# NilanEkanayake/TiTok-Video

Measured on AMD Instinct MI355X. Metric: video clips/sec encode+decode (whole node), higher is better.
Workload: dtype bf16

## Files before the change

include/titok_hip.h:

```cpp
#ifndef TITOK_HIP_H
#define TITOK_HIP_H

#include <stdint.h>

#ifdef __cplusplus
extern "C" {
#endif

#define TTV_OK 0
#define TTV_ERR_INVALID 1
#define TTV_ERR_LAUNCH 2
#define TTV_ERR_UNSUPPORTED 3

#define TTV_BF16 0
#define TTV_F32 1

#define TTV_ENCODER 0
#define TTV_DECODER 1

#define TTV_MAX_FSQ 8
#define TTV_MAX_TOKEN 64
#define TTV_MAX_CLIPS_PER_LAUNCH 64

const char* ttv_error_string(void);
int ttv_version(void);

typedef struct ttv_fsq_params {
  int32_t n;
  int32_t levels[TTV_MAX_FSQ];
  int32_t basis[TTV_MAX_FSQ];
  float half_l[TTV_MAX_FSQ];
  float offset[TTV_MAX_FSQ];
  float shift[TTV_MAX_FSQ];
  float half_width[TTV_MAX_FSQ];
} ttv_fsq_params;

int ttv_fsq_forward(const ttv_fsq_params* p, const void* z, int z_dtype, int rows, void* codes, int codes_dtype,
                    int32_t* indices, float* bounded, void* stream);
int ttv_fsq_indices_to_codes(const ttv_fsq_params* p, const int32_t* indices, int rows, void* codes, int codes_dtype,
                             void* stream);

int ttv_vq_codebook_norms(const void* codebook, int dtype, int ld, int N, int C, float* cnorm, void* stream);
int64_t ttv_vq_workspace_bytes(int rows);
int ttv_vq_l2_argmin(const void* z, int dtype, int ldz, const void* codebook, int ldc, const float* cnorm, int rows, int N, int C,
                     int32_t* indices, float* best_dist, void* workspace, int64_t workspace_bytes, void* stream);
int ttv_vq_lookup(const void* codebook, int dtype, int ldc, const int32_t* indices, int rows, int C, void* codes, int ldo, void* stream);
int ttv_vq_lookup_backward(const void* dcodes, int dtype, int ld, const int32_t* indices, int rows, int C, float* dcodebook, int ldc, void* stream);

int64_t ttv_vq_train_workspace_bytes(int rows, int N);
int ttv_vq_commit_forward(const void* z, int dtype, int ldz, const void* codebook, int ldc, const int32_t* indices, int rows, int N, int C,
                          float* loss, void* workspace, int64_t workspace_bytes, void* stream);
int ttv_vq_commit_backward(const void* grad, int ldg, const void* z, int ldz, const void* e, int lde, int dtype, int rows, int C, double scale,
                           void* dz, int ldd, void* stream);
int ttv_vq_ema_stats(const void* z, int dtype, int ldz, const int32_t* indices, int rows, int N, int C, const float* cluster_size,
                     float dead_threshold, uint64_t seed, const int64_t* ema_step, int rank, int world_size, float* stats, void* workspace,
                     int64_t workspace_bytes, void* stream);
int ttv_vq_ema_update(const float* stats, float* cluster_size, float* embed_avg, float* codebook, void* codebook_copy, int copy_dtype,
                      float* cnorm, int64_t* ema_step, int N, int C, float decay, float one_minus_decay, float eps, float dead_threshold,
                      void* workspace, int64_t workspace_bytes, void* stream);

int ttv_quant_rows_fp8(const void* in, int dtype, int ld_in, const float* gain, float eps, void* out, int ld_out, float* scales, int rows,
                       int width, void* stream);
int ttv_linear_fp8(const void* xq, int ldx, const float* x_scale, const void* wq, int ldw, const float* w_scale, void* y, int ldy, int M, int N,
                   int K, int epilogue, const float* rope_cs, int d_model, int gqa_dim, void* stream);

int ttv_split3_pack(const float* w, int ldw, void* out, int ldo, int rows, int K, void* stream);
int ttv_linear_split3(const float* x, int ldx, const void* w_image, int ldw, const float* bias, float* y, int ldy, int M, int N, int K, void* stream);

int64_t ttv_mx_scale_bytes_per_row(int width);
int ttv_quant_mx_fp8(const void* in, int dtype, int ld_in, void* out, int ld_out, void* mx, float* row_scales, int rows, int width, void* stream);
int ttv_linear_fp8_mx(const void* xq, int ldx, const void* x_mx, const float* x_row_scale, const void* wq, int ldw, const void* w_mx,
                      const float* w_row_scale, void* y, int ldy, int M, int N, int K, int epilogue, const float* rope_cs, int d_model,
                      int gqa_dim, const void* resid, int ldr, float alpha, void* stream);


int ttv_rmsnorm(const void* in, int in_dtype, int ld_in, const int32_t* src_rows, void* out, int out_dtype, int ld_out,
                const int32_t* dst_rows, const float* gain, int rows, int width, float eps, void* stream);

int ttv_rope_apply(void* x, int dtype, int ld, int rows, int heads, const float* rope_cs, void* stream);

int ttv_linear(const void* x, int ldx, const void* w, int ldw, const void* bias, const float* add_scalar, void* y, int ldy,
               int M, int N, int K, int dtype, void* stream);

int ttv_linear_qkv_rope(const void* x, int ldx, const void* w, int ldw, void* y, int ldy, int M, int d_model, int gqa_dim,
                        const float* rope_cs, int dtype, void* stream);
int ttv_linear_geglu(const void* x, int ldx, const void* w, int ldw, void* y, int ldy, int M, int I, int K, int dtype,
                     void* stream);
int ttv_linear_residual(const void* x, int ldx, const void* w, int ldw, const void* resid, int ldr, float alpha, void* y,
                        int ldy, int y_f32, int M, int N, int K, int dtype, void* stream);

int ttv_linear_residual_norm(const void* x, int ldx, const void* w, int ldw, const void* resid, int ldr, float alpha,
                             const float* gain, float eps, void* y, int ldy, int M, int N, int K, int dtype, void* stream);

int64_t ttv_mlp_pack_bytes(int inner, int next_qkv_rows);
int ttv_mlp_pack(const void* w12_folded, const void* w3, const void* out_proj, const void* next_qkv_folded, int next_qkv_rows, int inner,
                 int width, int dtype, void* mlp_packed, void* stream);
int ttv_mlp_fused(const void* x, int ldx, const void* mlp_packed, int inner, void* y, int ldy, const float* post_gain, float alpha,
                  float eps, int M, int width, int dtype, void* stream);
typedef struct ttv_next_qkv {
  void* qkv; int32_t ld;
  const float* rope_cs;
  int32_t rows;
  int32_t rope_q_end, rope_k_begin, rope_k_end;
} ttv_next_qkv;
int ttv_layer_tail_fused(const void* ao, int ldao, const float* attn_post_gain, float attn_alpha, const void* x, int ldx,
                         const void* mlp_packed, int inner, void* y, int ldy, const float* ffd_post_gain, float ffd_alpha, float eps,
                         int M, int width, int dtype, const ttv_next_qkv* next, void* stream);

int ttv_fill_const_rows(void* x, int dtype, int ld, const int32_t* rows_map, int rows, int width, const float* mask_token,
                        const float* gain, float eps, void* stream);
int ttv_decoder_embed(const void* codes, int token_size, const void* w, const void* bias, const float* mask_token, const float* gain,
                      void* x, int dtype, int ld, const int32_t* rows_map, int rows, int width, float eps, void* stream);

#define TTV_ATTN_GATE 1
#define TTV_ATTN_PAIRED 2
#define TTV_ATTN_QSCALED 4
#define TTV_ATTN_ALLFULL 8
#define TTV_ATTN_PIPE 16
#define TTV_ATTN_SPLIT3 32
#define TTV_ATTN_SPLIT_OUT 64
#define TTV_ATTN_SPLIT_IN 128
int ttv_attention(const void* qkvg, int ld, void* out, int ldo, const int32_t* cu_seqlens, const int32_t* qblocks,
                  int n_qblocks, int q_heads, int kv_heads, int head_dim, int flags, int dtype, void* stream);
int ttv_attention64(const void* qkvg, int ld, void* out, int ldo, const int32_t* cu_seqlens, const int32_t* items, int n_items,
                    int q_heads, int kv_heads, int head_dim, int flags, int dtype, void* stream);

int ttv_rmsnorm_mx(const void* in, int in_dtype, int ld_in, void* out, int out_dtype, int ld_out, const float* gain, int rows, int width,
                   float eps, float* next_rstd, void* mx_q, void* mx_s, void* stream);
int ttv_attention_mxout(const void* qkvg, int ld, void* out_q, void* out_mx, int ld_mx, const int32_t* cu_seqlens, const int32_t* qblocks,
                        int n_qblocks, int q_heads, int kv_heads, void* stream);
int ttv_linear_fp8_mx_geglu_q(const void* xq, int ldx, const void* x_mx, const float* x_row_scale, const void* wq, int ldw, const void* w_mx,
                              const float* w_row_scale, void* hq, void* hq_mx, int M, int N, int K, void* stream);

int ttv_row_rstd(const void* x, int dtype, int ldx, float* rstd, int rows, int width, float eps, void* stream);
int ttv_linear_rowscale(const void* x, int ldx, const void* w, int ldw, const float* row_scale, int epilogue, const float* rope_cs, int d_model,
                        int gqa_dim, void* y, int ldy, int M, int N, int K, int dtype, void* stream);

int ttv_patch_gather(const void* const* clips, const int32_t* clip_desc, int clip0, int n_clips, int patch_t, int patch_h,
                     int patch_w, int channels, void* patches, int ld, int dtype, int max_patches_per_clip, void* stream);
int ttv_patch_embed_norm(const void* const* clips, const int32_t* clip_desc, const int32_t* patch_rows, const int32_t* row_seq, int n_clips,
                         int patch_t, int patch_h, int patch_w, int channels, const void* w, int ldw, const void* bias,
                         const float* mask_token, const float* gain, float eps, void* x, int ldx, int rows, int width, int dtype,
                         void* stream);
int ttv_patch_scatter(const void* patches, int ld, const int32_t* clip_desc, int clip0, int n_clips, int patch_t, int patch_h,
                      int patch_w, int channels, void* const* clips, int dtype, int max_patches_per_clip, void* stream);

typedef struct ttv_tower_dims {
  int32_t kind;
  int32_t dtype;
  int32_t width;
  int32_t layers;
  int32_t q_heads, kv_heads, head_dim;
  int32_t inner;
  int32_t patch_t, patch_h, patch_w;
  int32_t pix_channels;
  int32_t token_size;
  float eps;
  float alpha;
} ttv_tower_dims;

typedef struct ttv_layer_weights {
  const float* pre_ln;
  const void* to_qkv;
  const void* out_proj;
  const float* ffd_norm;
  const void* w12;
  const void* w3;
  const float* attn_post_ln;
  const float* ffd_post_ln;
  const void* to_qkv_pn;
  const void* w12_pn;
  const void* mlp_pack;
  int32_t mlp_pack_qkv_rows;
  int32_t qkv_q_prescaled;
  const void* to_qkv_qs;
  const void* to_qkv_f8; const float* to_qkv_f8_scale;
  const void* w12_f8; const float* w12_f8_scale;
  const void* to_qkv_mx; const void* w12_mx;
  const void* out_proj_f8; const float* out_proj_f8_scale; const void* out_proj_mx;
  const void* w3_f8; const float* w3_f8_scale; const void* w3_mx;
} ttv_layer_weights;

typedef struct ttv_tower_weights {
  const void* proj_in_w;
  const void* proj_in_b;
  const float* mask_token;
  const float* ln_pre_t;
  const float* ln_pre_p;
  const float* ln_post;
  const void* proj_out_w;
  const void* proj_out_b;
  const ttv_layer_weights* layers;
  const void* proj_out_pn;
  int32_t f32_split3;
} ttv_tower_weights;

typedef struct ttv_batch {
  int32_t n_clips;
  int32_t total_rows;
  int32_t sum_tokens;
  int32_t sum_patches;
  int32_t max_patches_per_clip;
  int32_t n_qblocks;
  const int32_t* cu_seqlens;
  const int32_t* latent_rows;
  const int32_t* patch_rows;
  const int32_t* clip_desc;
  const int32_t* qblocks;
  const float* rope_cs;
  const int32_t* blocks64;
  const int32_t* row_seq;
  int32_t n_blocks64;
  int32_t qblocks_paired;
  int32_t qblocks_all_full;
  const int32_t* items64;
  int32_t n_items64;
  const int32_t* rope_ids;
  const float* rope_base;
  const int32_t* qblocks_latent;
  int32_t n_qblocks_latent;
  const int32_t* qblocks_patch;
  int32_t n_qblocks_patch;
  int32_t tokens_per_clip;
} ttv_batch;

int ttv_rope_table_build(const float* base_cos, const float* base_sin, int n_ids, int n_freqs, const int32_t* clip_desc,
                         const int32_t* cu_seqlens, const int32_t* row_seq, float* rope_cs, int total_rows, void* stream);

typedef struct ttv_plan_sizes {
  int32_t n_clips, total_rows, sum_tokens, sum_patches, max_patches_per_clip, max_seqlen, n_rope_ids, n_blocks64;
  int64_t host_words;
  int64_t off_cu_seqlens, off_clip_desc, off_blocks64;
  int64_t dev_words;
  int64_t off_latent_rows, off_patch_rows, off_row_seq, off_rope_ids;
} ttv_plan_sizes;

int ttv_plan_rows_sizes(const int32_t* pixel_dims, const int32_t* token_counts, int n_clips, const int32_t* patch, ttv_plan_sizes* sizes);
int ttv_plan_rows_fill(const int32_t* pixel_dims, const int32_t* token_counts, int n_clips, const int32_t* patch, int bwd_xcd,
                       int32_t* host_segment, int64_t host_words);

int ttv_plan_rows_build(const ttv_plan_sizes* sizes, const int32_t* host_segment, int32_t* dev_segment, const float* base_cos,
                        const float* base_sin, int n_freqs, float* rope_cs, const float* rope_base, ttv_batch* batch, void* stream);

typedef struct ttv_plan_attn {
  int32_t n_qblocks, qblocks_all_full, n_qblocks_latent, n_qblocks_patch, n_qblocks_l0;
  int32_t tokens_per_clip;
  int64_t words;
  int64_t off_qblocks, off_qblocks_latent, off_qblocks_patch, off_qblocks_l0;
} ttv_plan_attn;

int ttv_plan_attn_sizes(const int32_t* cu_seqlens, const int32_t* token_counts, int n_clips, int q_heads, int kv_heads, int split,
                        int tail_div, ttv_plan_attn* sizes);
int ttv_plan_attn_fill(const int32_t* cu_seqlens, const int32_t* token_counts, int n_clips, int q_heads, int kv_heads, int split,
                       int tail_div, int32_t* host_tables, int64_t host_words);
int ttv_plan_attn_set(const ttv_plan_attn* sizes, const int32_t* host_tables, int32_t* dev_tables, ttv_batch* batch, void* stream);

int ttv_rope_base_table(int head_dim, int nd, int n_ids, double theta, float* base_cos, float* base_sin);

int64_t ttv_tower_workspace_bytes(const ttv_tower_dims* dims, const ttv_batch* batch);

// ... 123 lines not shown
int ttv_l1_loss(void* const* recon, void* const* target, void* const* grad, const int32_t* sizes, int n_clips, int dtype, float* loss,
                void* stream);

int ttv_clip_from_u8(const void* frames_thwc, int T, int H, int W, void* clip_cthw, int dtype, void* stream);

int ttv_clip_resample_u8(void* const* frames_thwc, void* const* clips_cthw, const int32_t* geom, int n_clips, int dtype, void* stream);

int ttv_recon_panels_u8(void* const* target, void* const* recon, const int32_t* dims, int n_clips, int dtype, void* const* panels,
                        void* stream);

int ttv_sq_err_accumulate(void* const* recon, void* const* target, const int32_t* sizes, int n_clips, int dtype, int clamp, double* acc,
                          void* stream);

int64_t ttv_ssim_workspace_bytes(const int32_t* dims, int n_clips);
int ttv_ssim_accumulate(void* const* recon, void* const* target, const int32_t* dims, int n_clips, int dtype, int clamp, double* acc,
                        void* workspace, int64_t workspace_bytes, void* stream);

typedef struct {
  const void* w[13];
  const void* wd[13];
  const float* b[13];
  const float* lin[5];
} ttv_lpips_weights;

int64_t ttv_lpips_tape_bytes(int n, int H, int W, int dtype);
int64_t ttv_lpips_workspace_bytes(int n, int H, int W, int dtype);

int ttv_lpips_forward(const ttv_lpips_weights* w, const void* recon, const void* target, int n, int H, int W, int dtype, float* lpips,
                      float* gram, void* tape, void* workspace, int64_t workspace_bytes, void* stream);

int ttv_lpips_backward(const ttv_lpips_weights* w, const void* tape, int n, int H, int W, int dtype, const float* glpips,
                       const float* ggram, void* drecon, void* workspace, int64_t workspace_bytes, void* stream);

int64_t ttv_lpips_eval_workspace_bytes(int frames, int H, int W, int dtype);
int ttv_lpips_eval_accumulate(const ttv_lpips_weights* w, void* const* recon_clips, void* const* target_clips, const int32_t* frames,
                              int n_clips, int H, int W, int dtype, int clamp_recon, float* per_frame, double* acc, void* workspace,
                              int64_t workspace_bytes, void* stream);

int ttv_lpips_crops_forward(void* const* recon_clips, void* const* target_clips, const int32_t* clip_dims, int n_clips, const int32_t* crops,
                            int n_crops, int size, void* recon_crops, void* target_crops, int dtype, void* stream);
int ttv_lpips_crops_backward(void* const* recon_clips, void* const* grad_clips, const int32_t* clip_dims, int n_clips, const int32_t* crops,
                             int n_crops, int size, const void* g, int dtype, void* stream);

int ttv_gp_noise_add(const void* table, int n_clips, const int32_t* chunks, int n_chunks, int generate, uint64_t seed, uint64_t draw,
                     float gp_noise, int dtype, void* stream);

#define TTV_DISC_HEAD_GENERATOR 0
#define TTV_DISC_HEAD_DISCRIMINATOR 1
int ttv_disc_head(const void* per_token_a, const void* per_token_b, int mode, int groups, int n_clips, int tokens_per_clip, int dtype,
                  float gp_scale, float centering_weight, float* terms, float* grad, void* stream);

int64_t ttv_lpips_conv_workspace_bytes(int N, int H, int W, int Cin, int Cout, int dtype);
int ttv_lpips_conv3x3(const void* x, int N, int H, int W, int Cin, int Cout, const void* w, const float* bias, int mode, const void* h,
                      void* y, int dtype, void* workspace, int64_t workspace_bytes, void* stream);
int ttv_lpips_maxpool(const void* x, int N, int H, int W, int C, void* y, int dtype, void* stream);
int ttv_lpips_maxpool_backward(const void* dy, const float* add, const void* h, int N, int H, int W, int C, void* dx, int dtype,
                               void* stream);

#define TTV_I3D_CONVS 58
#define TTV_I3D_FEATURES 400
typedef struct {
  const float* w[TTV_I3D_CONVS];
  const float* scale[TTV_I3D_CONVS];
  const float* shift[TTV_I3D_CONVS];
} ttv_i3d_weights;

int64_t ttv_i3d_workspace_bytes(int n);

int ttv_fvd_preprocess(void* const* clips, const int32_t* dims, int n_clips, int dtype, int clamp, float* out, void* stream);

int ttv_i3d_features(const ttv_i3d_weights* w, const float* x, int n, float* feats, void* workspace, int64_t workspace_bytes,
                     void* stream);

int ttv_i3d_conv3d(const float* x, int N, int T, int H, int W, int Cin, int k, int stride, const float* w, const float* scale,
                   const float* shift, int Cout, int relu, float* y, int ldc, int c_off, void* stream);
int ttv_i3d_maxpool3d(const float* x, int N, int T, int H, int W, int C, int kt, int kh, int kw, int st, int sh, int sw, float* y,
                      void* stream);

#define TTV_VJEPA_WIDTH 1024
#define TTV_VJEPA_TOKENS 1568
#define TTV_VJEPA_PATCH_K 1536
typedef struct ttv_vjepa_layer {
  const float* norm1_w; const float* norm1_b;
  const void* qkv_w; const void* qkv_b;
  const void* proj_w; const void* proj_b;
  const float* norm2_w; const float* norm2_b;
  const void* fc1_w; const void* fc1_b;
  const void* fc2_w; const void* fc2_b;
} ttv_vjepa_layer;
typedef struct ttv_vjepa_weights {
  int32_t width, heads, depth;
  const void* patch_w; const void* patch_b; const float* pos_embed;
  const ttv_vjepa_layer* layers;
  const float* norm_w; const float* norm_b;
  const float* query_tokens; const void* pool_q;
  const float* pool_norm1_w; const float* pool_norm1_b;
  const void* pool_kv_w; const void* pool_kv_b;
  const void* pool_proj_w; const void* pool_proj_b;
  const float* pool_norm2_w; const float* pool_norm2_b;
  const void* pool_fc1_w; const void* pool_fc1_b;
  const void* pool_fc2_w; const void* pool_fc2_b;
} ttv_vjepa_weights;

int ttv_jedi_preprocess(void* const* clips, const int32_t* dims, int n_clips, int dtype, void* out, void* stream);
int64_t ttv_vjepa_workspace_bytes(int n);
int ttv_vjepa_features(const ttv_vjepa_weights* w, const void* x, int n, float* feats, int finetuned, void* workspace,
                       int64_t workspace_bytes, void* stream);

#define TTV_VJEPA_EPI_STORE 0
#define TTV_VJEPA_EPI_GELU 1
#define TTV_VJEPA_EPI_RESID 2
int ttv_vjepa_layernorm(const float* x, int ldx, int rows, int width, const float* w1, const float* b1, float eps1, const float* w2,
                        const float* b2, float eps2, float* y32, int ld32, void* y16, int ld16, void* stream);
int ttv_vjepa_linear(const void* x, int ldx, const void* w, int ldw, const void* bias, int M, int N, int K, int epilogue,
                     const float* resid, int ldr, int resid_rows, void* y, int ldy, void* stream);
int ttv_vjepa_pool_attention(const void* q, const void* kv, int n, int rows, void* out, void* stream);

#define TTV_KC_ATTENTION 1
#define TTV_KC_GEMM_QKV 2
#define TTV_KC_GEMM_GEGLU 3
#define TTV_KC_GEMM_RESID 4
#define TTV_KC_GEMM_STORE 5
#define TTV_KC_RMSNORM 6
#define TTV_KC_PATCH 7
#define TTV_KC_ROWS 8
int ttv_prof_begin(int kernel_class, int max_records);
enum {
  TTV_DBG_NO_STORES = 1,
  TTV_DBG_K256_NO_PANEL_DMA = 2,
  TTV_DBG_MLP_NO_WEIGHT_DMA = 2,
  TTV_DBG_K256_NO_TILE_RELOAD = 4,
  TTV_DBG_MLP_NO_GEGLU = 4,
  TTV_DBG_K256_NO_EPILOGUE_MATH = 8,
  TTV_DBG_MLP_TILES8 = 8,
  TTV_DBG_MLP_NO_P2 = 16,
  TTV_DBG_MLP_PAIRS_ONLY = 32,
  TTV_DBG_MLP_TILES4 = 64,
  TTV_DBG_GEMM_TILE160 = 128,
  TTV_DBG_GEMM_TILE128 = 256,
  TTV_DBG_GEMM_T256 = 512,
  TTV_DBG_MLP_TILES9 = 512,
  TTV_DBG_GEMM_NO_T256 = 1024,
  TTV_DBG_MX_UNFUSED_QUANT = 2048,
  TTV_DBG_SPLIT3_NO_IMAGES = 4096,
  TTV_DBG_SPLIT3_NO_DMA = 8192,
  TTV_DBG_K256_GENERAL = 16384,
  TTV_DBG_QKV256_OFF = 32768,
  TTV_DBG_QKV256_WS = 131072,
  TTV_DBG_ENC_ALL_ROWS = 524288,
  TTV_DBG_ATTN_NO_SWP = 1048576,
  TTV_DBG_DEC_ALL_BLOCKS = 2097152,
  TTV_DBG_DEC_L0_NO_CONST = 4194304,
  TTV_DBG_ENC_LAST_QKV_ALL = 8388608,
  TTV_DBG_PATCH_EMBED_UNFUSED = 16777216
};
int ttv_debug_set(int flags);
int ttv_debug_stamps(void* device_buffer);
int ttv_prof_end(double* total_ms, int* count);

#ifdef __cplusplus
}
#endif
#endif
```

titok_video_amd/_lib.py:

```python
from __future__ import annotations

import ctypes as C
import os
import threading

import torch

from . import switches

TTV_BF16, TTV_F32 = 0, 1
TTV_ENCODER, TTV_DECODER = 0, 1
TTV_MAX_FSQ = 8
TTV_MAX_TOKEN = 64
TTV_MAX_CLIPS_PER_LAUNCH = 64
TTV_DISC_HEAD_GENERATOR, TTV_DISC_HEAD_DISCRIMINATOR = 0, 1
TTV_TAPE_STORED, TTV_TAPE_RECOMPUTE = 0, 1

DBG_NO_STORES = 1
DBG_K256_NO_PANEL_DMA = 2
DBG_MLP_NO_WEIGHT_DMA = 2
DBG_K256_NO_TILE_RELOAD = 4
DBG_MLP_NO_GEGLU = 4
DBG_K256_NO_EPILOGUE_MATH = 8
DBG_MLP_TILES8 = 8
DBG_MLP_NO_P2 = 16
DBG_MLP_PAIRS_ONLY = 32
DBG_MLP_TILES4 = 64
DBG_GEMM_TILE160 = 128
DBG_GEMM_TILE128 = 256
DBG_GEMM_T256 = 512
DBG_MLP_TILES9 = 512
DBG_GEMM_NO_T256 = 1024
DBG_MX_UNFUSED_QUANT = 2048
DBG_SPLIT3_NO_IMAGES = 4096
DBG_SPLIT3_NO_DMA = 8192
DBG_K256_GENERAL = 16384
DBG_QKV256_OFF = 32768
DBG_QKV256_WS = 131072
DBG_ENC_ALL_ROWS = 524288
DBG_ATTN_NO_SWP = 1048576
DBG_DEC_ALL_BLOCKS = 2097152
DBG_DEC_L0_NO_CONST = 4194304
DBG_ENC_LAST_QKV_ALL = 8388608
DBG_PATCH_EMBED_UNFUSED = 16777216

_HERE = os.path.dirname(os.path.abspath(__file__))
LIB_PATH = switches.text("TTV_LIB_PATH") or os.path.join(_HERE, "libtitok_hip.so")

i32, i64, f32, vp = C.c_int32, C.c_int64, C.c_float, C.c_void_p


class FsqParams(C.Structure):
    _fields_ = [("n", i32), ("levels", i32 * TTV_MAX_FSQ), ("basis", i32 * TTV_MAX_FSQ),
                ("half_l", f32 * TTV_MAX_FSQ), ("offset", f32 * TTV_MAX_FSQ), ("shift", f32 * TTV_MAX_FSQ),
                ("half_width", f32 * TTV_MAX_FSQ)]


class TowerDims(C.Structure):
    _fields_ = [("kind", i32), ("dtype", i32), ("width", i32), ("layers", i32), ("q_heads", i32), ("kv_heads", i32),
                ("head_dim", i32), ("inner", i32), ("patch_t", i32), ("patch_h", i32), ("patch_w", i32),
                ("pix_channels", i32), ("token_size", i32), ("eps", f32), ("alpha", f32)]


class NextQkv(C.Structure):
    _fields_ = [("qkv", vp), ("ld", i32), ("rope_cs", vp), ("rows", i32), ("rope_q_end", i32), ("rope_k_begin", i32), ("rope_k_end", i32)]


class LayerWeights(C.Structure):
    _fields_ = [("pre_ln", vp), ("to_qkv", vp), ("out_proj", vp), ("ffd_norm", vp), ("w12", vp), ("w3", vp),
                ("attn_post_ln", vp), ("ffd_post_ln", vp), ("to_qkv_pn", vp), ("w12_pn", vp), ("mlp_pack", vp), ("mlp_pack_qkv_rows", i32), ("qkv_q_prescaled", i32),
                ("to_qkv_qs", vp), ("to_qkv_f8", vp), ("to_qkv_f8_scale", vp), ("w12_f8", vp), ("w12_f8_scale", vp),
                ("to_qkv_mx", vp), ("w12_mx", vp), ("out_proj_f8", vp), ("out_proj_f8_scale", vp), ("out_proj_mx", vp),
                ("w3_f8", vp), ("w3_f8_scale", vp), ("w3_mx", vp)]


class TowerWeights(C.Structure):
    _fields_ = [("proj_in_w", vp), ("proj_in_b", vp), ("mask_token", vp), ("ln_pre_t", vp), ("ln_pre_p", vp),
                ("ln_post", vp), ("proj_out_w", vp), ("proj_out_b", vp), ("layers", C.POINTER(LayerWeights)), ("proj_out_pn", vp),
                ("f32_split3", i32)]


class Batch(C.Structure):
    _fields_ = [("n_clips", i32), ("total_rows", i32), ("sum_tokens", i32), ("sum_patches", i32),
                ("max_patches_per_clip", i32), ("n_qblocks", i32), ("cu_seqlens", vp), ("latent_rows", vp),
                ("patch_rows", vp), ("clip_desc", vp), ("qblocks", vp), ("rope_cs", vp), ("blocks64", vp), ("row_seq", vp),
                ("n_blocks64", i32), ("qblocks_paired", i32), ("qblocks_all_full", i32), ("items64", vp), ("n_items64", i32),
                ("rope_ids", vp), ("rope_base", vp), ("qblocks_latent", vp), ("n_qblocks_latent", i32), ("qblocks_patch", vp),
                ("n_qblocks_patch", i32), ("tokens_per_clip", i32)]


class PlanSizes(C.Structure):
    _fields_ = [("n_clips", i32), ("total_rows", i32), ("sum_tokens", i32), ("sum_patches", i32), ("max_patches_per_clip", i32),
                ("max_seqlen", i32), ("n_rope_ids", i32), ("n_blocks64", i32), ("host_words", i64), ("off_cu_seqlens", i64),
                ("off_clip_desc", i64), ("off_blocks64", i64), ("dev_words", i64), ("off_latent_rows", i64), ("off_patch_rows", i64),
                ("off_row_seq", i64), ("off_rope_ids", i64)]


class PlanAttn(C.Structure):
    _fields_ = [("n_qblocks", i32), ("qblocks_all_full", i32), ("n_qblocks_latent", i32), ("n_qblocks_patch", i32), ("n_qblocks_l0", i32),
                ("tokens_per_clip", i32), ("words", i64), ("off_qblocks", i64), ("off_qblocks_latent", i64), ("off_qblocks_patch", i64),
                ("off_qblocks_l0", i64)]


class DecL0Const(C.Structure):
    _fields_ = [("rows", vp), ("latent_rows", i32), ("patch_rows", i32), ("state", vp), ("qblocks", vp), ("n_qblocks", i32)]


class LayerWeightsT(C.Structure):
    _fields_ = [("to_qkv_t", vp), ("out_proj_t", vp), ("w12_t", vp), ("w3_t", vp)]


class TowerWeightsT(C.Structure):
    _fields_ = [("proj_in_t", vp), ("proj_out_t", vp), ("layers", C.POINTER(LayerWeightsT))]


class LayerGrads(C.Structure):
    _fields_ = [("pre_ln", vp), ("to_qkv", vp), ("out_proj", vp), ("ffd_norm", vp), ("w12", vp), ("w3", vp),
                ("attn_post_ln", vp), ("ffd_post_ln", vp)]


class TowerGrads(C.Structure):
    _fields_ = [("proj_in_w", vp), ("proj_in_b", vp), ("mask_token", vp), ("ln_pre_t", vp), ("ln_pre_p", vp), ("ln_post", vp),
                ("proj_out_w", vp), ("proj_out_b", vp), ("layers", C.POINTER(LayerGrads)), ("layer_done_events", C.POINTER(vp))]


TTV_OPT_SCHEDULE_NONE, TTV_OPT_SCHEDULE_COSINE = 0, 1
TTV_OPT_SKIP_NONFINITE = 1


class OptState(C.Structure):
    _fields_ = [("updates", i64), ("skipped", i64), ("schedule_index", i64), ("skip_now", i32), ("lr", f32), ("bc1", f32),
                ("bc2_sqrt", f32), ("clip_coef", f32), ("norm", f32)]


class OptSchedule(C.Structure):
    _fields_ = [("kind", i32), ("reserved", i32), ("warmup_steps", i64), ("training_steps", i64), ("base_lr", C.c_double),
                ("end_lr", C.c_double), ("num_cycles", C.c_double), ("initial_lr", C.c_double), ("first", i64), ("stride", i64)]


class LpipsWeights(C.Structure):
    _fields_ = [("w", vp * 13), ("wd", vp * 13), ("b", vp * 13), ("lin", vp * 5)]


TTV_I3D_CONVS = 58
TTV_I3D_FEATURES = 400


class I3dWeights(C.Structure):
    _fields_ = [("w", vp * TTV_I3D_CONVS), ("scale", vp * TTV_I3D_CONVS), ("shift", vp * TTV_I3D_CONVS)]


TTV_VJEPA_WIDTH = 1024
TTV_VJEPA_TOKENS = 1568
TTV_VJEPA_PATCH_K = 1536
TTV_VJEPA_EPI_STORE, TTV_VJEPA_EPI_GELU, TTV_VJEPA_EPI_RESID = 0, 1, 2


class VjepaLayer(C.Structure):
    _fields_ = [("norm1_w", vp), ("norm1_b", vp), ("qkv_w", vp), ("qkv_b", vp), ("proj_w", vp), ("proj_b", vp), ("norm2_w", vp),
                ("norm2_b", vp), ("fc1_w", vp), ("fc1_b", vp), ("fc2_w", vp), ("fc2_b", vp)]


class VjepaWeights(C.Structure):
    _fields_ = [("width", i32), ("heads", i32), ("depth", i32), ("patch_w", vp), ("patch_b", vp), ("pos_embed", vp),
                ("layers", C.POINTER(VjepaLayer)), ("norm_w", vp), ("norm_b", vp), ("query_tokens", vp), ("pool_q", vp),
                ("pool_norm1_w", vp), ("pool_norm1_b", vp), ("pool_kv_w", vp), ("pool_kv_b", vp), ("pool_proj_w", vp),
                ("pool_proj_b", vp), ("pool_norm2_w", vp), ("pool_norm2_b", vp), ("pool_fc1_w", vp), ("pool_fc1_b", vp),
                ("pool_fc2_w", vp), ("pool_fc2_b", vp)]


_lib = None
_lock = threading.Lock()

SYMBOLS = {
    "ttv_error_string": (C.c_char_p, []),
    "ttv_version": (C.c_int, []),
    "ttv_fsq_forward": (C.c_int, [C.POINTER(FsqParams), vp, C.c_int, C.c_int, vp, C.c_int, vp, vp, vp]),
    "ttv_fsq_indices_to_codes": (C.c_int, [C.POINTER(FsqParams), vp, C.c_int, vp, C.c_int, vp]),
    "ttv_vq_codebook_norms": (C.c_int, [vp, C.c_int, C.c_int, C.c_int, C.c_int, vp, vp]),
    "ttv_vq_workspace_bytes": (C.c_int64, [C.c_int]),
    "ttv_vq_l2_argmin": (C.c_int, [vp, C.c_int, C.c_int, vp, C.c_int, vp, C.c_int, C.c_int, C.c_int, vp, vp, vp, C.c_int64, vp]),
    "ttv_vq_lookup": (C.c_int, [vp, C.c_int, C.c_int, vp, C.c_int, C.c_int, vp, C.c_int, vp]),
    "ttv_vq_lookup_backward": (C.c_int, [vp, C.c_int, C.c_int, vp, C.c_int, C.c_int, vp, C.c_int, vp]),
    "ttv_vq_train_workspace_bytes": (C.c_int64, [C.c_int, C.c_int]),
    "ttv_vq_commit_forward": (C.c_int, [vp, C.c_int, C.c_int, vp, C.c_int, vp, C.c_int, C.c_int, C.c_int, vp, vp, C.c_int64, vp]),
    "ttv_vq_commit_backward": (C.c_int, [vp, C.c_int, vp, C.c_int, vp, C.c_int, C.c_int, C.c_int, C.c_int, C.c_double, vp, C.c_int, vp]),
    "ttv_vq_ema_stats": (C.c_int, [vp, C.c_int, C.c_int, vp, C.c_int, C.c_int, C.c_int, vp, f32, C.c_uint64, vp, C.c_int, C.c_int, vp, vp, C.c_int64, vp]),
    "ttv_vq_ema_update": (C.c_int, [vp, vp, vp, vp, vp, C.c_int, vp, vp, C.c_int, C.c_int, f32, f32, f32, f32, vp, C.c_int64, vp]),
    "ttv_quant_rows_fp8": (C.c_int, [vp, C.c_int, C.c_int, vp, f32, vp, C.c_int, vp, C.c_int, C.c_int, vp]),
    "ttv_linear_fp8": (C.c_int, [vp, C.c_int, vp, vp, C.c_int, vp, vp, C.c_int, C.c_int, C.c_int, C.c_int, C.c_int, vp, C.c_int, C.c_int, vp]),
    "ttv_split3_pack": (C.c_int, [vp, C.c_int, vp, C.c_int, C.c_int, C.c_int, vp]),
    "ttv_linear_split3": (C.c_int, [vp, C.c_int, vp, C.c_int, vp, vp, C.c_int, C.c_int, C.c_int, C.c_int, vp]),
    "ttv_mx_scale_bytes_per_row": (C.c_int64, [C.c_int]),
    "ttv_quant_mx_fp8": (C.c_int, [vp, C.c_int, C.c_int, vp, C.c_int, vp, vp, C.c_int, C.c_int, vp]),
    "ttv_linear_fp8_mx": (C.c_int, [vp, C.c_int, vp, vp, vp, C.c_int, vp, vp, vp, C.c_int, C.c_int, C.c_int, C.c_int, C.c_int, vp, C.c_int, C.c_int,
                                    vp, C.c_int, f32, vp]),
    "ttv_rmsnorm": (C.c_int, [vp, C.c_int, C.c_int, vp, vp, C.c_int, C.c_int, vp, vp, C.c_int, C.c_int, f32, vp]),
    "ttv_rope_apply": (C.c_int, [vp, C.c_int, C.c_int, C.c_int, C.c_int, vp, vp]),
    "ttv_linear": (C.c_int, [vp, C.c_int, vp, C.c_int, vp, vp, vp, C.c_int, C.c_int, C.c_int, C.c_int, C.c_int, vp]),
    "ttv_linear_qkv_rope": (C.c_int, [vp, C.c_int, vp, C.c_int, vp, C.c_int, C.c_int, C.c_int, C.c_int, vp, C.c_int, vp]),
    "ttv_linear_geglu": (C.c_int, [vp, C.c_int, vp, C.c_int, vp, C.c_int, C.c_int, C.c_int, C.c_int, C.c_int, vp]),
    "ttv_linear_residual": (C.c_int, [vp, C.c_int, vp, C.c_int, vp, C.c_int, f32, vp, C.c_int, C.c_int, C.c_int, C.c_int,
                                      C.c_int, C.c_int, vp]),
    "ttv_linear_residual_norm": (C.c_int, [vp, C.c_int, vp, C.c_int, vp, C.c_int, f32, vp, f32, vp, C.c_int, C.c_int, C.c_int,
                                           C.c_int, C.c_int, vp]),
    "ttv_mlp_pack_bytes": (C.c_int64, [C.c_int, C.c_int]),
    "ttv_mlp_pack": (C.c_int, [vp, vp, vp, vp, C.c_int, C.c_int, C.c_int, C.c_int, vp, vp]),
    "ttv_layer_tail_fused": (C.c_int, [vp, C.c_int, vp, f32, vp, C.c_int, vp, C.c_int, vp, C.c_int, vp, f32, f32, C.c_int, C.c_int,
                                       C.c_int, vp, vp]),
    "ttv_mlp_fused": (C.c_int, [vp, C.c_int, vp, C.c_int, vp, C.c_int, vp, f32, f32, C.c_int, C.c_int, C.c_int, vp]),
    "ttv_fill_const_rows": (C.c_int, [vp, C.c_int, C.c_int, vp, C.c_int, C.c_int, vp, vp, f32, vp]),
    "ttv_decoder_embed": (C.c_int, [vp, C.c_int, vp, vp, vp, vp, vp, C.c_int, C.c_int, vp, C.c_int, C.c_int, f32, vp]),
    "ttv_attention": (C.c_int, [vp, C.c_int, vp, C.c_int, vp, vp, C.c_int, C.c_int, C.c_int, C.c_int, C.c_int, C.c_int, vp]),
    "ttv_attention64": (C.c_int, [vp, C.c_int, vp, C.c_int, vp, vp, C.c_int, C.c_int, C.c_int, C.c_int, C.c_int, C.c_int, vp]),
    "ttv_rmsnorm_mx": (C.c_int, [vp, C.c_int, C.c_int, vp, C.c_int, C.c_int, vp, C.c_int, C.c_int, f32, vp, vp, vp, vp]),
    "ttv_attention_mxout": (C.c_int, [vp, C.c_int, vp, vp, C.c_int, vp, vp, C.c_int, C.c_int, C.c_int, vp]),
    "ttv_linear_fp8_mx_geglu_q": (C.c_int, [vp, C.c_int, vp, vp, vp, C.c_int, vp, vp, vp, vp, C.c_int, C.c_int, C.c_int, vp]),
    "ttv_row_rstd": (C.c_int, [vp, C.c_int, C.c_int, vp, C.c_int, C.c_int, f32, vp]),
    "ttv_linear_rowscale": (C.c_int, [vp, C.c_int, vp, C.c_int, vp, C.c_int, vp, C.c_int, C.c_int, vp, C.c_int, C.c_int, C.c_int, C.c_int, C.c_int, vp]),
    "ttv_patch_gather": (C.c_int, [C.POINTER(vp), vp, C.c_int, C.c_int, C.c_int, C.c_int, C.c_int, C.c_int, vp, C.c_int,
                                   C.c_int, C.c_int, vp]),
    "ttv_patch_embed_norm": (C.c_int, [C.POINTER(vp), vp, vp, vp, C.c_int, C.c_int, C.c_int, C.c_int, C.c_int, vp, C.c_int, vp, vp, vp, f32,
                                       vp, C.c_int, C.c_int, C.c_int, C.c_int, vp]),
    "ttv_patch_scatter": (C.c_int, [vp, C.c_int, vp, C.c_int, C.c_int, C.c_int, C.c_int, C.c_int, C.c_int, C.POINTER(vp),
                                    C.c_int, C.c_int, vp]),
    "ttv_tower_workspace_bytes": (i64, [C.POINTER(TowerDims), C.POINTER(Batch)]),
    "ttv_encoder_forward": (C.c_int, [C.POINTER(TowerDims), C.POINTER(TowerWeights), C.POINTER(Batch), C.POINTER(vp),
                                      C.POINTER(FsqParams), vp, vp, vp, vp, vp, i64, vp]),
    "ttv_decoder_forward": (C.c_int, [C.POINTER(TowerDims), C.POINTER(TowerWeights), C.POINTER(Batch), vp, C.POINTER(vp),
                                      vp, i64, vp]),
    "ttv_dec_l0_const_bytes": (i64, [C.POINTER(TowerDims), C.c_int]),
    "ttv_dec_l0_const_build": (C.c_int, [C.POINTER(TowerDims), C.POINTER(TowerWeights), vp, vp, vp, vp, C.c_int, vp, i64, C.POINTER(i64), C.POINTER(i64), vp]),
    "ttv_decoder_forward_const": (C.c_int, [C.POINTER(TowerDims), C.POINTER(TowerWeights), C.POINTER(Batch), vp, C.POINTER(vp),
                                            vp, i64, C.POINTER(DecL0Const), vp]),
    "ttv_tower_tape_bytes": (i64, [C.POINTER(TowerDims), C.POINTER(Batch)]),
    "ttv_tower_bwd_workspace_bytes": (i64, [C.POINTER(TowerDims), C.POINTER(Batch)]),
    "ttv_encoder_forward_train": (C.c_int, [C.POINTER(TowerDims), C.POINTER(TowerWeights), C.POINTER(Batch), C.POINTER(vp), vp, vp,
                                            i64, vp]),
    "ttv_encoder_backward": (C.c_int, [C.POINTER(TowerDims), C.POINTER(TowerWeights), C.POINTER(TowerWeightsT), C.POINTER(Batch), vp,
                                       vp, C.POINTER(TowerGrads), C.POINTER(vp), vp, i64, vp]),
    "ttv_decoder_forward_train": (C.c_int, [C.POINTER(TowerDims), C.POINTER(TowerWeights), C.POINTER(Batch), vp, C.POINTER(vp), vp,
                                            i64, vp, i64, vp]),
    "ttv_decoder_backward": (C.c_int, [C.POINTER(TowerDims), C.POINTER(TowerWeights), C.POINTER(TowerWeightsT), C.POINTER(Batch), vp,
                                       C.POINTER(vp), vp, C.POINTER(TowerGrads), vp, vp, i64, vp]),
    "ttv_tower_tape_bytes_ex": (i64, [C.POINTER(TowerDims), C.POINTER(Batch), C.c_int]),
    "ttv_tower_bwd_workspace_bytes_ex": (i64, [C.POINTER(TowerDims), C.POINTER(Batch), C.c_int]),
    "ttv_encoder_forward_train_ex": (C.c_int, [C.POINTER(TowerDims), C.POINTER(TowerWeights), C.POINTER(Batch), C.POINTER(vp), vp, vp,
                                               i64, vp, C.c_int]),
    "ttv_encoder_backward_ex": (C.c_int, [C.POINTER(TowerDims), C.POINTER(TowerWeights), C.POINTER(TowerWeightsT), C.POINTER(Batch), vp,
                                          vp, C.POINTER(TowerGrads), C.POINTER(vp), vp, i64, vp, C.c_int]),
    "ttv_decoder_forward_train_ex": (C.c_int, [C.POINTER(TowerDims), C.POINTER(TowerWeights), C.POINTER(Batch), vp, C.POINTER(vp), vp,
                                               i64, vp, i64, vp, C.c_int]),
    "ttv_decoder_backward_ex": (C.c_int, [C.POINTER(TowerDims), C.POINTER(TowerWeights), C.POINTER(TowerWeightsT), C.POINTER(Batch), vp,
                                          C.POINTER(vp), vp, C.POINTER(TowerGrads), vp, vp, i64, vp, C.c_int]),
    "ttv_fsq_backward": (C.c_int, [C.POINTER(FsqParams), vp, vp, C.c_int, vp, C.c_int, vp]),
    "ttv_rmsnorm_backward_chain": (C.c_int, [vp, C.c_int, vp, C.c_int, vp, vp, vp, C.c_int, vp, C.c_int, vp, vp, C.c_float, vp, C.c_int,
                                              C.c_int, C.c_int, C.c_float, C.c_int, vp]),
    "ttv_opt_grad_sumsq": (C.c_int, [vp, vp, C.c_int, C.c_int, vp, vp]),
    "ttv_opt_adamw_step": (C.c_int, [vp, vp, C.c_int, C.c_int, vp, C.c_int] + [C.c_float] * 10 + [vp, vp]),
    "ttv_opt_prepare": (C.c_int, [vp, OptSchedule, C.c_double, C.c_double, C.c_double, C.c_float, vp, C.c_int, C.c_int, vp, vp]),
    "ttv_opt_adamw_step_dev": (C.c_int, [vp, vp, C.c_int, C.c_int, vp] + [C.c_float] * 6 + [vp]),
    "ttv_opt_param_norms": (C.c_int, [vp, vp, C.c_int, C.c_int, vp, vp, vp]),
    "ttv_opt_ema_update": (C.c_int, [vp, vp, C.c_int, C.c_int, C.c_float, vp]),
    "ttv_opt_ema_exchange": (C.c_int, [vp, vp, C.c_int, C.c_int, C.c_int, vp]),
    "ttv_linear_wgrad_workspace_bytes": (C.c_int64, [C.c_int, C.c_int, C.c_int]),
    "ttv_linear_wgrad": (C.c_int, [vp, C.c_int, vp, C.c_int, vp, C.c_int, C.c_int, C.c_int, C.c_int, C.c_int, vp, C.c_int64, vp]),
    "ttv_rmsnorm_backward": (C.c_int, [vp, C.c_int, vp, C.c_int, vp, vp, C.c_int, vp, C.c_int, C.c_int, f32, C.c_int, vp]),
    "ttv_attention_backward": (C.c_int, [vp, C.c_int, vp, C.c_int, vp, C.c_int, vp, vp, vp, vp, C.c_int, vp, vp, C.c_int, vp, C.c_int,
                                         C.c_int, C.c_int, C.c_int, vp, vp]),
    "ttv_attention_lse": (C.c_int, [vp, C.c_int, vp, C.c_int, vp, vp, C.c_int, C.c_int, C.c_int, C.c_int, C.c_int, C.c_int, vp, vp]),
    "ttv_codebook_histogram": (C.c_int, [vp, C.c_int, vp, C.c_int, vp]),
    "ttv_rope_table_build": (C.c_int, [vp, vp, C.c_int, C.c_int, vp, vp, vp, vp, C.c_int, vp]),
    "ttv_plan_rows_sizes": (C.c_int, [vp, vp, C.c_int, vp, C.POINTER(PlanSizes)]),
    "ttv_plan_rows_fill": (C.c_int, [vp, vp, C.c_int, vp, C.c_int, vp, i64]),
    "ttv_plan_rows_build": (C.c_int, [C.POINTER(PlanSizes), vp, vp, vp, vp, C.c_int, vp, vp, C.POINTER(Batch), vp]),
    "ttv_plan_attn_sizes": (C.c_int, [vp, vp, C.c_int, C.c_int, C.c_int, C.c_int, C.c_int, C.POINTER(PlanAttn)]),
    "ttv_plan_attn_fill": (C.c_int, [vp, vp, C.c_int, C.c_int, C.c_int, C.c_int, C.c_int, vp, i64]),
    "ttv_plan_attn_set": (C.c_int, [C.POINTER(PlanAttn), vp, vp, C.POINTER(Batch), vp]),
    "ttv_rope_base_table": (C.c_int, [C.c_int, C.c_int, C.c_int, C.c_double, vp, vp]),
    "ttv_l1_loss": (C.c_int, [vp, vp, vp, vp, C.c_int, C.c_int, vp, vp]),
    "ttv_clip_from_u8": (C.c_int, [vp, C.c_int, C.c_int, C.c_int, vp, C.c_int, vp]),
    "ttv_clip_resample_u8": (C.c_int, [vp, vp, vp, C.c_int, C.c_int, vp]),
    "ttv_recon_panels_u8": (C.c_int, [vp, vp, vp, C.c_int, C.c_int, vp, vp]),
    "ttv_sq_err_accumulate": (C.c_int, [vp, vp, vp, C.c_int, C.c_int, C.c_int, vp, vp]),
    "ttv_ssim_workspace_bytes": (C.c_int64, [vp, C.c_int]),
    "ttv_ssim_accumulate": (C.c_int, [vp, vp, vp, C.c_int, C.c_int, C.c_int, vp, vp, C.c_int64, vp]),
    "ttv_lpips_tape_bytes": (C.c_int64, [C.c_int, C.c_int, C.c_int, C.c_int]),
    "ttv_lpips_workspace_bytes": (C.c_int64, [C.c_int, C.c_int, C.c_int, C.c_int]),
    "ttv_lpips_forward": (C.c_int, [C.POINTER(LpipsWeights), vp, vp, C.c_int, C.c_int, C.c_int, C.c_int, vp, vp, vp, vp, C.c_int64, vp]),
    "ttv_lpips_backward": (C.c_int, [C.POINTER(LpipsWeights), vp, C.c_int, C.c_int, C.c_int, C.c_int, vp, vp, vp, vp, C.c_int64, vp]),
    "ttv_lpips_eval_workspace_bytes": (C.c_int64, [C.c_int, C.c_int, C.c_int, C.c_int]),
    "ttv_lpips_eval_accumulate": (C.c_int, [C.POINTER(LpipsWeights), vp, vp, vp, C.c_int, C.c_int, C.c_int, C.c_int, C.c_int, vp, vp, vp,
                                            C.c_int64, vp]),
    "ttv_lpips_conv_workspace_bytes": (C.c_int64, [C.c_int] * 6),
    "ttv_lpips_conv3x3": (C.c_int, [vp, C.c_int, C.c_int, C.c_int, C.c_int, C.c_int, vp, vp, C.c_int, vp, vp, C.c_int, vp, C.c_int64, vp]),
    "ttv_lpips_maxpool": (C.c_int, [vp, C.c_int, C.c_int, C.c_int, C.c_int, vp, C.c_int, vp]),
    "ttv_lpips_maxpool_backward": (C.c_int, [vp, vp, vp, C.c_int, C.c_int, C.c_int, C.c_int, vp, C.c_int, vp]),
    "ttv_lpips_crops_forward": (C.c_int, [vp, vp, vp, C.c_int, vp, C.c_int, C.c_int, vp, vp, C.c_int, vp]),
    "ttv_lpips_crops_backward": (C.c_int, [vp, vp, vp, C.c_int, vp, C.c_int, C.c_int, vp, C.c_int, vp]),
    "ttv_gp_noise_add": (C.c_int, [vp, C.c_int, vp, C.c_int, C.c_int, C.c_uint64, C.c_uint64, f32, C.c_int, vp]),
    "ttv_disc_head": (C.c_int, [vp, vp, C.c_int, C.c_int, C.c_int, C.c_int, C.c_int, f32, f32, vp, vp, vp]),
    "ttv_i3d_workspace_bytes": (C.c_int64, [C.c_int]),
    "ttv_fvd_preprocess": (C.c_int, [vp, vp, C.c_int, C.c_int, C.c_int, vp, vp]),
    "ttv_i3d_features": (C.c_int, [C.POINTER(I3dWeights), vp, C.c_int, vp, vp, C.c_int64, vp]),
    "ttv_i3d_conv3d": (C.c_int, [vp] + [C.c_int] * 7 + [vp, vp, vp, C.c_int, C.c_int, vp, C.c_int, C.c_int, vp]),
    "ttv_i3d_maxpool3d": (C.c_int, [vp] + [C.c_int] * 11 + [vp, vp]),
    "ttv_jedi_preprocess": (C.c_int, [vp, vp, C.c_int, C.c_int, vp, vp]),
    "ttv_vjepa_workspace_bytes": (C.c_int64, [C.c_int]),
    "ttv_vjepa_features": (C.c_int, [C.POINTER(VjepaWeights), vp, C.c_int, vp, C.c_int, vp, C.c_int64, vp]),
    "ttv_vjepa_layernorm": (C.c_int, [vp, C.c_int, C.c_int, C.c_int, vp, vp, C.c_float, vp, vp, C.c_float, vp, C.c_int, vp, C.c_int, vp]),
    "ttv_vjepa_linear": (C.c_int, [vp, C.c_int, vp, C.c_int, vp, C.c_int, C.c_int, C.c_int, C.c_int, vp, C.c_int, C.c_int, vp, C.c_int, vp]),
    "ttv_vjepa_pool_attention": (C.c_int, [vp, vp, C.c_int, C.c_int, vp, vp]),
    "ttv_debug_set": (C.c_int, [C.c_int]),
    "ttv_debug_stamps": (C.c_int, [vp]),
    "ttv_prof_begin": (C.c_int, [C.c_int, C.c_int]),
    "ttv_prof_end": (C.c_int, [C.POINTER(C.c_double), C.POINTER(C.c_int)]),
}

KERNEL_CLASSES = {"attention": 1, "gemm_qkv": 2, "gemm_geglu": 3, "gemm_resid": 4, "gemm_store": 5, "rmsnorm": 6,
                  "patch": 7, "rows": 8}


def lib():
    global _lib
    if _lib is None:
        with _lock:
            if _lib is None:
                if not os.path.exists(LIB_PATH):
                    raise RuntimeError(
                        f"titok_video_amd: {LIB_PATH} is missing - build it with `python -c 'import __graft_entry__ as g; "
                        "g.build()'` (or titok_video_amd/csrc/build.sh). There is no non-HIP fallback.")
                handle = C.CDLL(LIB_PATH)
                for name, (res, args) in SYMBOLS.items():
                    fn = getattr(handle, name)
                    fn.restype, fn.argtypes = res, args
                _lib = handle
    return _lib


def check(rc: int, what: str) -> None:
    if rc != 0:
        msg = lib().ttv_error_string().decode("utf-8", "replace")
        raise RuntimeError(f"{what} failed (code {rc}): {msg}")


def dtype_code(dt: torch.dtype) -> int:
    if dt == torch.bfloat16:
        return TTV_BF16
    if dt == torch.float32:
        return TTV_F32
    raise TypeError(f"titok_video_amd supports bfloat16 and float32 activations, got {dt}")


def require_gpu(t: torch.Tensor, what: str) -> None:
    if not t.is_cuda:
        raise RuntimeError(f"{what}: tensor is on {t.device}; titok_video_amd runs on MI355X (HIP) only, there is no CPU path")


def stream_ptr(device) -> int:
    return torch.cuda.current_stream(device).cuda_stream


# ... 10 lines not shown
```

titok_video_amd/csrc/ttv_api.hip:

```cpp
#include <stdarg.h>
#include <stdio.h>
#include <stdlib.h>
#include <string.h>

#include "ttv_common.h"
#include "ttv_kernels.h"

static thread_local char g_err[512] = "";

void ttv_set_error(const char* fmt, ...) {
  va_list ap;
  va_start(ap, fmt);
  vsnprintf(g_err, sizeof(g_err), fmt, ap);
  va_end(ap);
}

int g_ttv_prof_class = 0;
bool ttv_sw_enc_latent_last() { static const bool v = ttv_env_flag("TTV_ENC_LATENT_LAST", true); return v; }
bool ttv_enc_latent_rows_only(const ttv_tower_dims* d, const ttv_batch* b) {
  return ttv_sw_enc_latent_last() && !(g_ttv_debug & TTV_DBG_ENC_ALL_ROWS) && d->kind == TTV_ENCODER && b->latent_rows && b->sum_tokens > 0 &&
         b->sum_tokens < b->total_rows;
}
bool ttv_sw_keel_f32sum() { static const bool v = ttv_env_flag("TTV_KEEL_F32SUM", false); return v; }
bool ttv_sw_fused_patch() { static const bool v = ttv_env_flag("TTV_FUSED_PATCH", true); return v; }
bool ttv_sw_attn_pipe() { static const bool v = ttv_env_flag("TTV_ATTN_PIPE", false); return v; }
static bool sw_dec_l0_const() { static const bool v = ttv_env_flag("TTV_DEC_L0_CONST", true); return v; }
static bool sw_enc_last_qkv_skip() { static const bool v = ttv_env_flag("TTV_ENC_LAST_QKV_SKIP", true); return v; }
float ttv_sw_attn_thr() { static const float v = ttv_env_float("TTV_ATTN_THR", 8.0f); return v; }
thread_local int g_ttv_debug = 0;
long long* g_ttv_stamps = nullptr;
static hipEvent_t* g_prof_start = nullptr;
static hipEvent_t* g_prof_stop = nullptr;
static int g_prof_cap = 0, g_prof_n = 0;

TtvProfScope::TtvProfScope(int cls, hipStream_t stream) : slot(-1), s(stream) {
  if (g_ttv_prof_class != 0 && cls == g_ttv_prof_class && g_prof_n < g_prof_cap) {
    slot = g_prof_n++;
    (void)hipEventRecord(g_prof_start[slot], s);
  }
}
TtvProfScope::~TtvProfScope() {
  if (slot >= 0) (void)hipEventRecord(g_prof_stop[slot], s);
}

struct TowerWs {
  char *x, *xn, *qkv, *ao, *h, *pa, *pb;
  char *xl, *aol;
  char *f8, *f8mx;
  float* y32;
  float* rstd;
  int64_t total;
};

static TowerWs carve(const ttv_tower_dims* d, const ttv_batch* b, char* base) {
  const int64_t e = dtype_bytes(d->dtype);
  const int64_t L = b->total_rows, P = b->sum_patches;
  const int64_t g = (int64_t)d->kv_heads * d->head_dim;
  const int64_t pd = patch_dim(d);
  int64_t off = 0;
  TowerWs w;
  auto take = [&](int64_t bytes) { char* p = base ? base + off : nullptr; off += align256(bytes); return p; };
  w.x = take(L * d->width * e);
  w.xn = take(L * d->width * e);
  w.qkv = take(L * (2 * d->width + 2 * g) * e);
  w.ao = take(L * d->width * e);
  w.y32 = (float*)take(L * d->width * 4);
  w.h = take(L * d->inner * e);
  w.pa = take(P * pd * e);
  w.pb = take(P * d->width * e);
  w.rstd = (float*)take(L * 4);
  w.xl = take((int64_t)b->sum_tokens * d->width * e);
  w.aol = take((int64_t)b->sum_tokens * d->width * e);
  w.f8 = w.f8mx = nullptr;
  if (d->dtype == TTV_BF16 && d->width != 256 && d->width % 128 == 0) {
    const int64_t wide = d->width > d->inner ? d->width : d->inner;
    w.f8 = take(L * wide);
    w.f8mx = take(L * (wide / 128 + 4) * 4);
  }
  w.total = off;
  return w;
}

static int check_dims(const ttv_tower_dims* d, const ttv_batch* b) {
  TTV_CHECK_ARG(d && b, "null dims/batch");
  TTV_CHECK_ARG(d->dtype == TTV_BF16 || d->dtype == TTV_F32, "bad dtype %d", d->dtype);
  TTV_CHECK_ARG(d->head_dim == 64 && d->width == d->q_heads * 64, "width must be q_heads*64");
  TTV_CHECK_ARG(d->width % 64 == 0 && d->width <= 1024, "width %d unsupported", d->width);
  TTV_CHECK_ARG(d->inner % 32 == 0, "GEGLU inner dim must be a multiple of 32");
  TTV_CHECK_ARG(d->token_size >= 1 && d->token_size <= TTV_MAX_TOKEN, "token_size out of range");
  TTV_CHECK_ARG(((int64_t)d->pix_channels * d->patch_t * d->patch_h * d->patch_w) % 8 == 0, "patch vector length must be a multiple of 8");
  TTV_CHECK_ARG(b->n_clips > 0 && b->total_rows == b->sum_tokens + b->sum_patches, "inconsistent batch");
  return TTV_OK;
}

struct LayerCtx {
  const ttv_tower_dims* d; const ttv_batch* b; const TowerWs& ws; hipStream_t s;
  int split3, s3img;
  bool gen_ok;
  int pair, all_full, pipe;
};

static int tower_attention(const LayerCtx& c, bool q_scaled, const int32_t* table, int n_table, int site) {
  const ttv_tower_dims* d = c.d;
  const int flags = TTV_ATTN_GATE | (q_scaled ? TTV_ATTN_QSCALED : 0) | (c.split3 ? TTV_ATTN_SPLIT3 : 0) |
                    (c.s3img ? (TTV_ATTN_SPLIT_OUT | TTV_ATTN_SPLIT_IN) : 0) | site;
  return ttvk_attention(c.ws.qkv, 2 * d->width + 2 * d->kv_heads * d->head_dim, c.ws.ao, d->width, c.b->cu_seqlens, table, n_table, d->q_heads,
                        d->kv_heads, d->head_dim, flags, d->dtype, c.s);
}

static int run_layer_mx(const LayerCtx& c, const ttv_layer_weights& lw, int i, bool& rstd_valid, bool& xq_valid) {
  const ttv_tower_dims* d = c.d;
  const ttv_batch* b = c.b;
  const TowerWs& ws = c.ws;
  hipStream_t s = c.s;
  const int L = b->total_rows, dm = d->width, g = d->kv_heads * d->head_dim, dt = d->dtype, nq = 2 * dm + 2 * g, I = d->inner;
  const float alpha = keel_alpha(d, i);
  static const bool fused_env = ttv_env_flag("TTV_MX_FUSED_QUANT", true);
  const bool fused_q = fused_env && !(g_ttv_debug & TTV_DBG_MX_UNFUSED_QUANT);
  if (!rstd_valid) TTV_TRY(ttvk_row_rstd(ws.x, dt, dm, ws.rstd, L, dm, d->eps, s));
  if (!xq_valid) TTV_TRY(ttvk_quant_mx_fp8(ws.x, dt, dm, ws.f8, dm, ws.f8mx, nullptr, L, dm, s));
  xq_valid = false;
  const GemmArgs a = gemm_rope_qk(gemm_args(dt, ws.f8, dm, lw.to_qkv_f8, dm, L, nq, dm, ws.qkv, nq), b->rope_cs, dm, g);
  TTV_TRY(ttvk_gemm_fp8(EPI_QKV_ROPE, a, ws.rstd, lw.to_qkv_f8_scale, s, ws.f8mx, lw.to_qkv_mx));
  const bool q_scaled = lw.qkv_q_prescaled != 0;
  if (fused_q && q_scaled && !c.pair && !c.pipe && d->head_dim == 64) {
    TTV_TRY(ttvk_attention_mxout(ws.qkv, nq, ws.f8, ws.f8mx, (int)ttvk_mx_scale_ld(dm), b->cu_seqlens, b->qblocks, b->n_qblocks, d->q_heads,
                                 d->kv_heads, s));
  } else {
    TTV_TRY(tower_attention(c, q_scaled, b->qblocks, b->n_qblocks, c.pair | (c.pipe ? c.all_full | c.pipe : 0)));
    TTV_TRY(ttvk_quant_mx_fp8(ws.ao, dt, dm, ws.f8, dm, ws.f8mx, nullptr, L, dm, s));
  }
  const GemmArgs o = gemm_resid(gemm_args(dt, ws.f8, dm, lw.out_proj_f8, dm, L, dm, dm, ws.x, dm), ws.x, dm, alpha);
  TTV_TRY(ttvk_gemm_fp8(EPI_RESID_T, o, nullptr, lw.out_proj_f8_scale, s, ws.f8mx, lw.out_proj_mx));
  if (i > 0) {
    TTV_TRY(ttvk_rmsnorm(ws.x, dt, dm, nullptr, ws.x, dt, dm, nullptr, lw.attn_post_ln, L, dm, d->eps, s, ws.rstd, fused_q ? ws.f8 : nullptr,
                         fused_q ? ws.f8mx : nullptr));
    if (!fused_q) TTV_TRY(ttvk_quant_mx_fp8(ws.x, dt, dm, ws.f8, dm, ws.f8mx, nullptr, L, dm, s));
  } else {
    TTV_TRY(ttvk_row_rstd(ws.x, dt, dm, ws.rstd, L, dm, d->eps, s));
    TTV_TRY(ttvk_quant_mx_fp8(ws.x, dt, dm, ws.f8, dm, ws.f8mx, nullptr, L, dm, s));
  }
  GemmArgs f = gemm_args(dt, ws.f8, dm, lw.w12_f8, dm, L, I, dm, ws.h, I);
  char* const hq = ws.h;
  char* const hq_mx = ws.xn;
  const bool h_fused = fused_q && (int64_t)ttvk_mx_scale_ld(I) <= (int64_t)dm * 2;
  if (h_fused) { f.yq = hq; f.yq_mx = hq_mx; }
  TTV_TRY(ttvk_gemm_fp8(EPI_GEGLU, f, ws.rstd, lw.w12_f8_scale, s, ws.f8mx, lw.w12_mx));
  if (!h_fused) TTV_TRY(ttvk_quant_mx_fp8(ws.h, dt, I, ws.f8, I, ws.f8mx, nullptr, L, I, s));
  const GemmArgs f3 = gemm_resid(gemm_args(dt, h_fused ? hq : ws.f8, I, lw.w3_f8, I, L, dm, I, ws.x, dm), ws.x, dm, alpha);
  TTV_TRY(ttvk_gemm_fp8(EPI_RESID_T, f3, nullptr, lw.w3_f8_scale, s, h_fused ? hq_mx : ws.f8mx, lw.w3_mx));
  rstd_valid = false;
  if (i > 0) {
    TTV_TRY(ttvk_rmsnorm(ws.x, dt, dm, nullptr, ws.x, dt, dm, nullptr, lw.ffd_post_ln, L, dm, d->eps, s, ws.rstd, fused_q ? ws.f8 : nullptr,
                         fused_q ? ws.f8mx : nullptr));
    rstd_valid = true;
    xq_valid = fused_q;
  }
  return TTV_OK;
}

static bool rows_f8(int dt, int dm, const void* img, const void* row_scale, const void* mx, const void* folded) {
  return dt == TTV_BF16 && img && row_scale && !mx && dm % 128 == 0 && !(dm == 256 && folded);
}

struct PreNormW { const float* gain; const void *w, *w_pn, *w_f8; const float* w_f8_scale; bool f8; };

static int prenorm_proj(const LayerCtx& c, GemmEpilogue epi, const char* x, int rows, const PreNormW& p, int N, char* y, int y_image,
                        bool rstd_valid, int tile_run = 0, int tile_period = 0, int panel_lo = 0) {
  const ttv_tower_dims* d = c.d;
  const TowerWs& ws = c.ws;
  const int dm = d->width, dt = d->dtype;
  GemmArgs a = gemm_args(dt, nullptr, dm, nullptr, dm, rows, N, dm, y, N);
  if (epi == EPI_QKV_ROPE) a = gemm_rope_qk(a, c.b->rope_cs, dm, d->kv_heads * d->head_dim);
  if (p.f8) {
    float* const f8_scales = reinterpret_cast<float*>(ws.xn + align256((int64_t)c.b->total_rows * dm));
    TTV_TRY(ttvk_quant_rows_fp8(x, dt, dm, p.gain, d->eps, ws.xn, dm, f8_scales, rows, dm, c.s));
    a.x = ws.xn; a.w = p.w_f8;
    return ttvk_gemm_fp8(epi, a, f8_scales, p.w_f8_scale, c.s);
  }
  const bool fold256 = dt == TTV_BF16 && dm == 256 && p.w_pn;
  const bool fold_gen = c.gen_ok && p.w_pn;
  const bool fold = fold256 || fold_gen;
  if (fold_gen && !rstd_valid) TTV_TRY(ttvk_row_rstd(x, dt, dm, ws.rstd, rows, dm, d->eps, c.s));
  if (!fold) TTV_TRY(ttvk_rmsnorm(x, dt, dm, nullptr, ws.xn, dt, dm, nullptr, p.gain, rows, dm, d->eps, c.s, nullptr, nullptr, nullptr, c.s3img));
  a.split3 = c.split3; a.x_image = c.s3img && !fold; a.y_image = y_image;
  a.prenorm = fold256; a.eps = d->eps;
  a.row_scale = fold_gen ? ws.rstd : nullptr;
  a.x = fold ? x : ws.xn; a.w = fold ? p.w_pn : p.w;
  if (epi == EPI_QKV_ROPE) { a.rope_ids = c.b->rope_ids; a.rope_base = c.b->rope_ids ? c.b->rope_base : nullptr; }
  a.tile_run = tile_run; a.tile_period = tile_period; a.panel_lo = panel_lo;
  return ttvk_gemm(epi, a, c.s);
}

static int keel_tail(const LayerCtx& c, GemmArgs o, int layer, const float* post_gain, bool want_rstd, bool& rstd_valid) {
  const ttv_tower_dims* d = c.d;
  const int dm = d->width, dt = d->dtype;
  char* const cx = (char*)o.y;
  o = gemm_resid(o, cx, dm, keel_alpha(d, layer));
  o.split3 = c.split3; o.x_image = c.s3img;
  if (layer == 0) return ttvk_gemm(EPI_RESID_T, o, c.s);
  if (ttvk_gemm_supports_resid_norm(dt, dm, o.K)) {
    o.norm_gain = post_gain; o.eps = d->eps;
    return ttvk_gemm(EPI_RESID_NORM, o, c.s);
  }
  float* const next_rstd = want_rstd ? c.ws.rstd : nullptr;
  if (dt == TTV_BF16 && !ttv_sw_keel_f32sum()) {
    TTV_TRY(ttvk_gemm(EPI_RESID_T, o, c.s));
    TTV_TRY(ttvk_rmsnorm(cx, dt, dm, nullptr, cx, dt, dm, nullptr, post_gain, o.M, dm, d->eps, c.s, next_rstd));
  } else {
    o.y = c.ws.y32;
    TTV_TRY(ttvk_gemm(EPI_RESID_F32, o, c.s));
    TTV_TRY(ttvk_rmsnorm(c.ws.y32, TTV_F32, dm, nullptr, cx, dt, dm, nullptr, post_gain, o.M, dm, d->eps, c.s, next_rstd));
  }
  rstd_valid = want_rstd;
  return TTV_OK;
}

static bool qkv_tile_list_ok(const LayerCtx& c, const ttv_layer_weights& lw, int K, int P) {
  const ttv_tower_dims* d = c.d;
  const ttv_batch* b = c.b;
  if (d->dtype != TTV_BF16 || d->width != 256 || d->head_dim != 64 || c.split3) return false;
  if (K <= 0 || P <= 0 || K % 128 || P % 128 || (int64_t)b->n_clips * K != b->sum_tokens || (int64_t)b->n_clips * P != b->sum_patches) return false;
  if (!lw.to_qkv_pn || !lw.qkv_q_prescaled) return false;
  return ttvk_gemm_qkv_tiles_supported(d->width, d->kv_heads * d->head_dim, d->width);
}

static bool dec_l0_const_ok(const LayerCtx& c, const ttv_tower_weights* w, const ttv_dec_l0_const* l0) {
  const ttv_tower_dims* d = c.d;
  const ttv_batch* b = c.b;
  if (!l0 || !l0->rows || !sw_dec_l0_const() || (g_ttv_debug & TTV_DBG_DEC_L0_NO_CONST)) return false;
  if (d->kind != TTV_DECODER || !qkv_tile_list_ok(c, w->layers[0], l0->latent_rows, l0->patch_rows)) return false;
  if (c.pair || c.pipe || !c.all_full || (b->items64 && b->n_items64 > 0)) return false;
  return ttvk_attention_takes_swp(TTV_ATTN_GATE | TTV_ATTN_QSCALED | TTV_ATTN_ALLFULL);
}

static bool enc_last_qkv_skip_ok(const LayerCtx& c, const ttv_layer_weights& lw) {
  const ttv_batch* b = c.b;
  if (!sw_enc_last_qkv_skip() || (g_ttv_debug & TTV_DBG_ENC_LAST_QKV_ALL) || c.d->kind != TTV_ENCODER) return false;
  return qkv_tile_list_ok(c, lw, b->tokens_per_clip, b->max_patches_per_clip);
}

static int run_layers(const ttv_tower_dims* d, const ttv_tower_weights* w, const ttv_batch* b, const TowerWs& ws, hipStream_t s,
                      const ttv_dec_l0_const* l0 = nullptr) {
  const int L = b->total_rows, dm = d->width, g = d->kv_heads * d->head_dim, dt = d->dtype;
  const int split3 = (dt == TTV_F32 && w->f32_split3) ? 1 : 0;
  const bool gen_ok = (dt == TTV_BF16 && dm != 256) || split3;
  static const bool s3img_env = ttv_env_flag("TTV_SPLIT3_IMAGES", true);
  const int s3img = (split3 && s3img_env && !(g_ttv_debug & TTV_DBG_SPLIT3_NO_IMAGES)) ? 1 : 0;
  const int nq = 2 * dm + 2 * g;
  const int64_t row_bytes = (int64_t)dm * dtype_bytes(dt);
  bool qkv_ready = false;
  bool rstd_valid = false;
  bool xq_valid = false;
  const bool lat_last = ttv_enc_latent_rows_only(d, b) && b->qblocks_latent && b->n_qblocks_latent > 0;
  static const bool pat_env = ttv_env_flag("TTV_DEC_PATCH_LAST", true);
  const bool pat_last = pat_env && !(g_ttv_debug & TTV_DBG_DEC_ALL_BLOCKS) && d->kind == TTV_DECODER && d->layers >= 2 && b->qblocks_patch &&
                        b->n_qblocks_patch > 0 && !split3 && !b->qblocks_paired;
  bool compacted = false;
  const LayerCtx ctx = {d, b, ws, s, split3, s3img, gen_ok, b->qblocks_paired ? TTV_ATTN_PAIRED : 0, b->qblocks_all_full ? TTV_ATTN_ALLFULL : 0,
                        ttv_sw_attn_pipe() ? TTV_ATTN_PIPE : 0};
  const bool l0_const = dec_l0_const_ok(ctx, w, l0);
  for (int i = 0; i < d->layers; ++i) {
    const ttv_layer_weights& lw = w->layers[i];
    const bool last = i == d->layers - 1;
    const bool l0c = l0_const && i == 0;
    if (dt == TTV_BF16 && dm != 256 && dm % 128 == 0 && d->inner % 128 == 0 && !ttv_sw_keel_f32sum() && lw.to_qkv_f8 && lw.to_qkv_mx && lw.w12_f8 &&
        lw.w12_mx && lw.out_proj_f8 && lw.out_proj_mx && lw.w3_f8 && lw.w3_mx &&
        !(lat_last && last)) {
      TTV_TRY(run_layer_mx(ctx, lw, i, rstd_valid, xq_valid));
      qkv_ready = false;
      continue;
    }
    xq_valid = false;
    const bool f8_qkv = rows_f8(dt, dm, lw.to_qkv_f8, lw.to_qkv_f8_scale, lw.to_qkv_mx, lw.to_qkv_pn);
    const bool f8_w12 = rows_f8(dt, dm, lw.w12_f8, lw.w12_f8_scale, lw.w12_mx, lw.w12_pn);
    if (!qkv_ready) {
      const void* w_plain = (dt == TTV_BF16 && lw.to_qkv_qs) ? lw.to_qkv_qs : lw.to_qkv;
      const PreNormW qw = {lw.pre_ln, w_plain, lw.to_qkv_pn, lw.to_qkv_f8, lw.to_qkv_f8_scale, f8_qkv};
      if (l0c) TTV_TRY(prenorm_proj(ctx, EPI_QKV_ROPE, ws.x, L, qw, nq, ws.qkv, 0, rstd_valid, l0->latent_rows / 128, (l0->latent_rows + l0->patch_rows) / 128));
      else if (lat_last && last && !f8_qkv && enc_last_qkv_skip_ok(ctx, lw))
        TTV_TRY(prenorm_proj(ctx, EPI_QKV_ROPE, ws.x, L, qw, nq, ws.qkv, 0, rstd_valid, b->tokens_per_clip / 128,
                             (b->tokens_per_clip + b->max_patches_per_clip) / 128, 2 * dm / 64));
      else TTV_TRY(prenorm_proj(ctx, EPI_QKV_ROPE, ws.x, L, qw, nq, ws.qkv, s3img ? 2 : 0, rstd_valid));
    }
    const bool q_scaled = dt == TTV_BF16 && (lw.to_qkv_pn ? lw.qkv_q_prescaled != 0 : lw.to_qkv_qs != nullptr);
    rstd_valid = false;
    qkv_ready = false;
    const bool lat_now = lat_last && last;
    if (lat_now)
      TTV_TRY(tower_attention(ctx, q_scaled, b->qblocks_latent, b->n_qblocks_latent, ctx.all_full));
    else if (l0c) {
      TtvProfScope prof(TTV_KC_ATTENTION, s);
      const bool own = l0->qblocks && l0->n_qblocks > 0;
      TTV_TRY(ttvk_attention_swp(ws.qkv, nq, ws.ao, dm, b->cu_seqlens, own ? l0->qblocks : b->qblocks, own ? l0->n_qblocks : b->n_qblocks, d->q_heads,
                                 d->kv_heads, 1, s, l0->rows, l0->latent_rows, l0->state));
    } else if (pat_last && last && dt == TTV_BF16 && !ctx.pipe)
      TTV_TRY(tower_attention(ctx, q_scaled, b->qblocks_patch, b->n_qblocks_patch, ctx.all_full));
    else if (q_scaled && b->items64 && b->n_items64 > 0 && d->head_dim == 64)
      TTV_TRY(ttvk_attention64(ws.qkv, nq, ws.ao, dm, b->cu_seqlens, b->items64, b->n_items64, d->q_heads, d->kv_heads,
                               TTV_ATTN_GATE | TTV_ATTN_QSCALED, s));
    else
      TTV_TRY(tower_attention(ctx, q_scaled, b->qblocks, b->n_qblocks, ctx.pair | ctx.all_full | ctx.pipe));
    char* cx = ws.x;
    char* cao = ws.ao;
    int Lc = L;
    if (lat_now) {
      TTV_TRY(gather_rows(ws.x, ws.xl, b->latent_rows, b->sum_tokens, row_bytes, s));
      TTV_TRY(gather_rows(ws.ao, ws.aol, b->latent_rows, b->sum_tokens, row_bytes, s));
      cx = ws.xl; cao = ws.aol; Lc = b->sum_tokens;
      compacted = true;
    }
    static const bool use_fused_mlp = ttv_env_flag("TTV_FUSED_MLP", true);
    static const bool use_fused_qkv = ttv_env_flag("TTV_FUSED_QKV", false);
    const float alpha = keel_alpha(d, i);
    if (use_fused_mlp && ttvk_mlp_fused_supported(dt, dm, d->inner) && lw.mlp_pack) {
      MlpNextQkv nx = {};
      const bool back = use_fused_qkv && !last && lw.mlp_pack_qkv_rows == nq && nq % 64 == 0 && dm % 64 == 0 && g % 64 == 0;
      if (back) { nx.qkv = ws.qkv; nx.ld = nq; nx.rope_cs = b->rope_cs; nx.rows = nq; nx.rope_q_end = dm; nx.rope_k_begin = 2 * dm; nx.rope_k_end = 2 * dm + g; }
      TTV_TRY(ttvk_mlp_fused(cao, dm, i == 0 ? nullptr : lw.attn_post_ln, alpha, cx, dm, lw.mlp_pack, d->inner, cx, dm, i == 0 ? nullptr : lw.ffd_post_ln,
                             alpha, d->eps, Lc, back ? &nx : nullptr, s));
      qkv_ready = back;
      continue;
    }
    TTV_TRY(keel_tail(ctx, gemm_args(dt, cao, dm, lw.out_proj, dm, Lc, dm, dm, cx, dm), i, lw.attn_post_ln, gen_ok && lw.w12_pn && !f8_w12, rstd_valid));
    const PreNormW fw = {lw.ffd_norm, lw.w12, lw.w12_pn, lw.w12_f8, lw.w12_f8_scale, f8_w12};
    TTV_TRY(prenorm_proj(ctx, EPI_GEGLU, cx, Lc, fw, d->inner, ws.h, s3img, rstd_valid));
    rstd_valid = false;
    const ttv_layer_weights* nl = last ? nullptr : &w->layers[i + 1];
    const bool next_rstd = gen_ok && nl && nl->to_qkv_pn && !rows_f8(dt, dm, nl->to_qkv_f8, nl->to_qkv_f8_scale, nl->to_qkv_mx, nl->to_qkv_pn);
    TTV_TRY(keel_tail(ctx, gemm_args(dt, ws.h, d->inner, lw.w3, d->inner, Lc, dm, d->inner, cx, dm), i, lw.ffd_post_ln, next_rstd, rstd_valid));
  }
  if (compacted)
    TTV_TRY(scatter_rows(ws.xl, ws.x, b->latent_rows, b->sum_tokens, row_bytes, s));
  return TTV_OK;
}

static bool fused_patch_ok(const ttv_tower_dims* d, const ttv_batch* b, int dt) {
  auto pow2 = [](int v) { return v > 0 && (v & (v - 1)) == 0; };
  return ttv_sw_fused_patch() && dt == TTV_BF16 && d->patch_w == 8 && pow2(d->patch_t) && pow2(d->patch_h) &&
         b->n_clips <= TTV_MAX_CLIPS_PER_LAUNCH && b->row_seq && patch_dim(d) % 64 == 0;
}

extern "C" {

const char* ttv_error_string(void) { return g_err; }
int ttv_version(void) { return 100; }

int ttv_fsq_forward(const ttv_fsq_params* p, const void* z, int z_dtype, int rows, void* codes, int codes_dtype, int32_t* indices,
                    float* bounded, void* stream) {
  TTV_CHECK_ARG(rows >= 0 && (rows == 0 || (z && codes && indices)), "fsq_forward: null buffer");
  return ttvk_fsq_forward(p, z, z_dtype, rows, codes, codes_dtype, indices, bounded, (hipStream_t)stream);
}

int ttv_fsq_indices_to_codes(const ttv_fsq_params* p, const int32_t* indices, int rows, void* codes, int codes_dtype, void* stream) {
  TTV_CHECK_ARG(rows >= 0 && (rows == 0 || (indices && codes)), "fsq_indices_to_codes: null buffer");
  return ttvk_fsq_indices_to_codes(p, indices, rows, codes, codes_dtype, (hipStream_t)stream);
}

int ttv_vq_codebook_norms(const void* codebook, int dtype, int ld, int N, int C, float* cnorm, void* stream) {
  TTV_CHECK_ARG(N == 0 || (codebook && cnorm), "vq_codebook_norms: null buffer");
  return ttvk_vq_norms(codebook, dtype, ld, N, C, cnorm, (hipStream_t)stream);
}

int64_t ttv_vq_workspace_bytes(int rows) { return ttvk_vq_workspace_bytes(rows); }

int ttv_vq_l2_argmin(const void* z, int dtype, int ldz, const void* codebook, int ldc, const float* cnorm, int rows, int N, int C,
                     int32_t* indices, float* best_dist, void* workspace, int64_t workspace_bytes, void* stream) {
  TTV_CHECK_ARG(rows == 0 || (z && codebook && cnorm && indices), "vq_l2_argmin: null buffer");
  TTV_CHECK_ARG(ldz >= C && ldc >= C, "vq_l2_argmin: leading dims smaller than the codebook dim");
  return ttvk_vq_l2_argmin(z, dtype, ldz, codebook, ldc, cnorm, rows, N, C, indices, best_dist, workspace, workspace_bytes, (hipStream_t)stream);
}

int ttv_vq_lookup(const void* codebook, int dtype, int ldc, const int32_t* indices, int rows, int C, void* codes, int ldo, void* stream) {
  TTV_CHECK_ARG(rows == 0 || (codebook && indices && codes), "vq_lookup: null buffer");
  return ttvk_vq_lookup(codebook, dtype, ldc, indices, rows, C, codes, ldo, (hipStream_t)stream);
}

int ttv_vq_lookup_backward(const void* dcodes, int dtype, int ld, const int32_t* indices, int rows, int C, float* dcodebook, int ldc, void* stream) {
  TTV_CHECK_ARG(rows == 0 || (dcodes && indices && dcodebook), "vq_lookup_backward: null buffer");
  TTV_CHECK_ARG(ld >= C && ldc >= C, "vq_lookup_backward: leading dims smaller than the codebook dim");
  return ttvk_vq_lookup_bwd(dcodes, dtype, ld, indices, rows, C, dcodebook, ldc, (hipStream_t)stream);
}

int64_t ttv_vq_train_workspace_bytes(int rows, int N) {
  if (rows < 1 || N < 1) { ttv_set_error("vq_train_workspace_bytes: %d rows, %d entries", rows, N); return -1; }
  return ttvk_vq_train_workspace_bytes(rows, N);
}

int ttv_vq_commit_forward(const void* z, int dtype, int ldz, const void* codebook, int ldc, const int32_t* indices, int rows, int N, int C,
                          float* loss, void* workspace, int64_t workspace_bytes, void* stream) {
  TTV_CHECK_ARG(z && codebook && indices && loss && workspace, "vq_commit_forward: null buffer");
  return ttvk_vq_commit_forward(z, dtype, ldz, codebook, ldc, indices, rows, N, C, loss, workspace, workspace_bytes, (hipStream_t)stream);
}

int ttv_vq_commit_backward(const void* grad, int ldg, const void* z, int ldz, const void* e, int lde, int dtype, int rows, int C, double scale,
                           void* dz, int ldd, void* stream) {
  TTV_CHECK_ARG(grad && z && e && dz, "vq_commit_backward: null buffer");
  return ttvk_vq_commit_backward(grad, ldg, z, ldz, e, lde, dtype, rows, C, scale, dz, ldd, (hipStream_t)stream);
}

int ttv_vq_ema_stats(const void* z, int dtype, int ldz, const int32_t* indices, int rows, int N, int C, const float* cluster_size,
                     float dead_threshold, uint64_t seed, const int64_t* ema_step, int rank, int world_size, float* stats, void* workspace,
                     int64_t workspace_bytes, void* stream) {
  TTV_CHECK_ARG(z && indices && stats && workspace, "vq_ema_stats: null buffer");
  return ttvk_vq_ema_stats(z, dtype, ldz, indices, rows, N, C, cluster_size, dead_threshold, seed, ema_step, rank, world_size, stats, workspace,
                           workspace_bytes, (hipStream_t)stream);
}

int ttv_vq_ema_update(const float* stats, float* cluster_size, float* embed_avg, float* codebook, void* codebook_copy, int copy_dtype,
                      float* cnorm, int64_t* ema_step, int N, int C, float decay, float one_minus_decay, float eps, float dead_threshold,
                      void* workspace, int64_t workspace_bytes, void* stream) {
  TTV_CHECK_ARG(stats && cluster_size && embed_avg && codebook && codebook_copy && cnorm && ema_step && workspace, "vq_ema_update: null buffer");
  return ttvk_vq_ema_update(stats, cluster_size, embed_avg, codebook, codebook_copy, copy_dtype, cnorm, ema_step, N, C, decay, one_minus_decay, eps,
                            dead_threshold, workspace, workspace_bytes, (hipStream_t)stream);
}

int ttv_quant_rows_fp8(const void* in, int dtype, int ld_in, const float* gain, float eps, void* out, int ld_out, float* scales, int rows,
                       int width, void* stream) {
  TTV_CHECK_ARG(rows == 0 || (in && out && scales), "quant_rows_fp8: null buffer");
  return ttvk_quant_rows_fp8(in, dtype, ld_in, gain, eps, out, ld_out, scales, rows, width, (hipStream_t)stream);
}

int ttv_split3_pack(const float* w, int ldw, void* out, int ldo, int rows, int K, void* stream) {
  TTV_CHECK_ARG(rows == 0 || (w && out), "split3_pack: null buffer");
  return ttvk_split3_pack(w, ldw, out, ldo, rows, K, (hipStream_t)stream);
}

int ttv_linear_split3(const float* x, int ldx, const void* w_image, int ldw, const float* bias, float* y, int ldy, int M, int N, int K, void* stream) {
  TTV_CHECK_ARG(M == 0 || (x && w_image && y), "linear_split3: null buffer");
  GemmArgs a = gemm_args(TTV_F32, x, ldx, w_image, ldw, M, N, K, y, ldy);
  a.split3 = 1; a.bias = bias;
  return ttvk_gemm(EPI_STORE, a, (hipStream_t)stream);
}

int64_t ttv_mx_scale_bytes_per_row(int width) { return ttvk_mx_scale_ld(width); }

int ttv_quant_mx_fp8(const void* in, int dtype, int ld_in, void* out, int ld_out, void* mx, float* row_scales, int rows, int width, void* stream) {
  TTV_CHECK_ARG(rows == 0 || (in && out && mx), "quant_mx_fp8: null buffer");
  TTV_CHECK_ARG(ld_in >= width && ld_out >= width, "quant_mx_fp8: leading dims smaller than the width");
  return ttvk_quant_mx_fp8(in, dtype, ld_in, out, ld_out, mx, row_scales, rows, width, (hipStream_t)stream);
}

int ttv_linear_fp8_mx(const void* xq, int ldx, const void* x_mx, const float* x_row_scale, const void* wq, int ldw, const void* w_mx,
                      const float* w_row_scale, void* y, int ldy, int M, int N, int K, int epilogue, const float* rope_cs, int d_model,
                      int gqa_dim, const void* resid, int ldr, float alpha, void* stream) {
  TTV_CHECK_ARG(M == 0 || (xq && wq && y && x_mx && w_mx), "linear_fp8_mx: null buffer");
  TTV_CHECK_ARG(epilogue >= 0 && epilogue <= 3, "linear_fp8_mx: epilogue 0 (store), 1 (qkv + rotary), 2 (GEGLU) or 3 (alpha * resid + acc)");
  GemmArgs a = gemm_args(TTV_BF16, xq, ldx, wq, ldw, M, N, K, y, ldy);
  if (epilogue == 1) {
    TTV_CHECK_ARG(rope_cs && N == 2 * d_model + 2 * gqa_dim, "linear_fp8_mx: qkv epilogue needs rope_cs and N = 2 d_model + 2 gqa_dim");
    a = gemm_rope_qk(a, rope_cs, d_model, gqa_dim);
  }
  if (epilogue == 3) a = gemm_resid(a, resid, ldr, alpha);
  return ttvk_gemm_fp8(epilogue == 0 ? EPI_STORE : epilogue == 1 ? EPI_QKV_ROPE : epilogue == 2 ? EPI_GEGLU : EPI_RESID_T, a, x_row_scale,
                       w_row_scale, (hipStream_t)stream, x_mx, w_mx);
}

int ttv_linear_fp8(const void* xq, int ldx, const float* x_scale, const void* wq, int ldw, const float* w_scale, void* y, int ldy, int M, int N,
                   int K, int epilogue, const float* rope_cs, int d_model, int gqa_dim, void* stream) {
  TTV_CHECK_ARG(M == 0 || (xq && wq && y), "linear_fp8: null buffer");
  TTV_CHECK_ARG(epilogue >= 0 && epilogue <= 2, "linear_fp8: epilogue 0 (store), 1 (qkv + rotary) or 2 (GEGLU)");
  GemmArgs a = gemm_args(TTV_BF16, xq, ldx, wq, ldw, M, N, K, y, ldy);
  if (epilogue == 1) {
    TTV_CHECK_ARG(rope_cs && N == 2 * d_model + 2 * gqa_dim, "linear_fp8: qkv epilogue needs rope_cs and N = 2 d_model + 2 gqa_dim");
    a = gemm_rope_qk(a, rope_cs, d_model, gqa_dim);
  }
  return ttvk_gemm_fp8(epilogue == 0 ? EPI_STORE : epilogue == 1 ? EPI_QKV_ROPE : EPI_GEGLU, a, x_scale, w_scale, (hipStream_t)stream);
}

int ttv_rmsnorm(const void* in, int in_dtype, int ld_in, const int32_t* src_rows, void* out, int out_dtype, int ld_out,
                const int32_t* dst_rows, const float* gain, int rows, int width, float eps, void* stream) {
  TTV_CHECK_ARG(rows >= 0 && (rows == 0 || (in && out && gain)), "rmsnorm: null buffer");
  return ttvk_rmsnorm(in, in_dtype, ld_in, src_rows, out, out_dtype, ld_out, dst_rows, gain, rows, width, eps, (hipStream_t)stream);
}

int ttv_rope_apply(void* x, int dtype, int ld, int rows, int heads, const float* rope_cs, void* stream) {
  TTV_CHECK_ARG(rows == 0 || (x && rope_cs), "rope_apply: null buffer");
  TTV_CHECK_ARG(ld % 4 == 0 && ld >= heads * 64, "rope_apply: bad leading dim");
  return ttvk_rope_apply(x, dtype, ld, rows, heads, rope_cs, (hipStream_t)stream);
}

int ttv_linear(const void* x, int ldx, const void* w, int ldw, const void* bias, const float* add_scalar, void* y, int ldy, int M,
               int N, int K, int dtype, void* stream) {
  TTV_CHECK_ARG(M == 0 || (x && w && y), "linear: null buffer");
  GemmArgs a = gemm_args(dtype, x, ldx, w, ldw, M, N, K, y, ldy);
  a.bias = bias; a.add_scalar = add_scalar;
  return ttvk_gemm(EPI_STORE, a, (hipStream_t)stream);
}

int ttv_linear_qkv_rope(const void* x, int ldx, const void* w, int ldw, void* y, int ldy, int M, int d_model, int gqa_dim,
                        const float* rope_cs, int dtype, void* stream) {
  TTV_CHECK_ARG(M == 0 || (x && w && y && rope_cs), "linear_qkv_rope: null buffer");
  const GemmArgs a = gemm_args(dtype, x, ldx, w, ldw, M, 2 * d_model + 2 * gqa_dim, d_model, y, ldy);
  return ttvk_gemm(EPI_QKV_ROPE, gemm_rope_qk(a, rope_cs, d_model, gqa_dim), (hipStream_t)stream);
}

int ttv_linear_geglu(const void* x, int ldx, const void* w, int ldw, void* y, int ldy, int M, int I, int K, int dtype, void* stream) {
  TTV_CHECK_ARG(M == 0 || (x && w && y), "linear_geglu: null buffer");
  return ttvk_gemm(EPI_GEGLU, gemm_args(dtype, x, ldx, w, ldw, M, I, K, y, ldy), (hipStream_t)stream);
}

int ttv_linear_residual(const void* x, int ldx, const void* w, int ldw, const void* resid, int ldr, float alpha, void* y, int ldy,
                        int y_f32, int M, int N, int K, int dtype, void* stream) {
  TTV_CHECK_ARG(M == 0 || (x && w && y && resid), "linear_residual: null buffer");
  const GemmArgs a = gemm_resid(gemm_args(dtype, x, ldx, w, ldw, M, N, K, y, ldy), resid, ldr, alpha);
  return ttvk_gemm(y_f32 ? EPI_RESID_F32 : EPI_RESID_T, a, (hipStream_t)stream);
}

int ttv_linear_residual_norm(const void* x, int ldx, const void* w, int ldw, const void* resid, int ldr, float alpha,
                             const float* gain, float eps, void* y, int ldy, int M, int N, int K, int dtype, void* stream) {
  TTV_CHECK_ARG(M == 0 || (x && w && y && resid && gain), "linear_residual_norm: null buffer");
  GemmArgs a = gemm_resid(gemm_args(dtype, x, ldx, w, ldw, M, N, K, y, ldy), resid, ldr, alpha);
  a.norm_gain = gain; a.eps = eps;
  if (!ttvk_gemm_supports_resid_norm(dtype, N, K)) {
    ttv_set_error("linear_residual_norm: only bf16 with N == 256 has a fused kernel");
    return TTV_ERR_UNSUPPORTED;
  }
  return ttvk_gemm(EPI_RESID_NORM, a, (hipStream_t)stream);
}

int64_t ttv_mlp_pack_bytes(int inner, int next_qkv_rows) { return ttvk_mlp_pack_bytes(inner, next_qkv_rows); }

int ttv_mlp_pack(const void* w12_folded, const void* w3, const void* out_proj, const void* next_qkv_folded, int next_qkv_rows, int inner,
                 int width, int dtype, void* packed, void* stream) {
  if (!ttvk_mlp_fused_supported(dtype, width, inner)) {
    ttv_set_error("mlp_pack: only bf16, width 256, inner %% 32 == 0");
    return TTV_ERR_UNSUPPORTED;
  }
  return ttvk_mlp_pack(w12_folded, w3, out_proj, next_qkv_folded, next_qkv_rows, inner, packed, (hipStream_t)stream);
}

int ttv_mlp_fused(const void* x, int ldx, const void* mlp_packed, int inner, void* y, int ldy, const float* post_gain, float alpha,
                  float eps, int M, int width, int dtype, void* stream) {
  if (!ttvk_mlp_fused_supported(dtype, width, inner)) {
    ttv_set_error("mlp_fused: only bf16, width 256, inner %% 32 == 0");
    return TTV_ERR_UNSUPPORTED;
  }
  return ttvk_mlp_fused(nullptr, 0, nullptr, 1.f, x, ldx, mlp_packed, inner, y, ldy, post_gain, alpha, eps, M, nullptr, (hipStream_t)stream);
}

int ttv_layer_tail_fused(const void* ao, int ldao, const float* attn_post_gain, float attn_alpha, const void* x, int ldx,
                         const void* mlp_packed, int inner, void* y, int ldy, const float* ffd_post_gain, float ffd_alpha, float eps,
                         int M, int width, int dtype, const ttv_next_qkv* next, void* stream) {
  if (!ttvk_mlp_fused_supported(dtype, width, inner)) {
    ttv_set_error("layer_tail_fused: only bf16, width 256, inner %% 32 == 0");
    return TTV_ERR_UNSUPPORTED;
  }
  TTV_CHECK_ARG(ao, "layer_tail_fused: null attention output");
  MlpNextQkv nx = {};
  if (next) { nx.qkv = next->qkv; nx.ld = next->ld; nx.rope_cs = next->rope_cs; nx.rows = next->rows; nx.rope_q_end = next->rope_q_end;
              nx.rope_k_begin = next->rope_k_begin; nx.rope_k_end = next->rope_k_end; }
  return ttvk_mlp_fused(ao, ldao, attn_post_gain, attn_alpha, x, ldx, mlp_packed, inner, y, ldy, ffd_post_gain, ffd_alpha, eps, M,
                        next ? &nx : nullptr, (hipStream_t)stream);
}

int ttv_fill_const_rows(void* x, int dtype, int ld, const int32_t* rows_map, int rows, int width, const float* mask_token,
                        const float* gain, float eps, void* stream) {
  TTV_CHECK_ARG(rows == 0 || (x && rows_map && mask_token && gain), "fill_const_rows: null buffer");
  return ttvk_fill_const_rows(x, dtype, ld, rows_map, rows, width, mask_token, gain, eps, (hipStream_t)stream);
}

int ttv_decoder_embed(const void* codes, int token_size, const void* w, const void* bias, const float* mask_token, const float* gain,
                      void* x, int dtype, int ld, const int32_t* rows_map, int rows, int width, float eps, void* stream) {
  TTV_CHECK_ARG(rows == 0 || (codes && w && bias && mask_token && gain && x && rows_map), "decoder_embed: null buffer");
  return ttvk_dec_embed(codes, token_size, w, bias, mask_token, gain, x, dtype, ld, rows_map, rows, width, eps, (hipStream_t)stream);
}

int ttv_attention(const void* qkvg, int ld, void* out, int ldo, const int32_t* cu_seqlens, const int32_t* qblocks, int n_qblocks,
                  int q_heads, int kv_heads, int head_dim, int flags, int dtype, void* stream) {
  TTV_CHECK_ARG(n_qblocks == 0 || (qkvg && out && cu_seqlens && qblocks), "attention: null buffer");
  return ttvk_attention(qkvg, ld, out, ldo, cu_seqlens, qblocks, n_qblocks, q_heads, kv_heads, head_dim, flags, dtype, (hipStream_t)stream);
}
int ttv_attention64(const void* qkvg, int ld, void* out, int ldo, const int32_t* cu_seqlens, const int32_t* items, int n_items, int q_heads,
                    int kv_heads, int head_dim, int flags, int dtype, void* stream) {
  TTV_CHECK_ARG(dtype == TTV_BF16 && head_dim == 64, "attention64: bf16, head_dim 64 only");
  return ttvk_attention64(qkvg, ld, out, ldo, cu_seqlens, items, n_items, q_heads, kv_heads, flags, (hipStream_t)stream);
}

int ttv_rmsnorm_mx(const void* in, int in_dtype, int ld_in, void* out, int out_dtype, int ld_out, const float* gain, int rows, int width,
                   float eps, float* next_rstd, void* mx_q, void* mx_s, void* stream) {
  TTV_CHECK_ARG(rows >= 0 && (rows == 0 || (in && out && gain)), "rmsnorm_mx: null buffer");
  TTV_CHECK_ARG(!mx_q == !mx_s, "rmsnorm_mx: the image needs both its element and its scale buffer");
  return ttvk_rmsnorm(in, in_dtype, ld_in, nullptr, out, out_dtype, ld_out, nullptr, gain, rows, width, eps, (hipStream_t)stream, next_rstd, mx_q, mx_s);
}

int ttv_attention_mxout(const void* qkvg, int ld, void* out_q, void* out_mx, int ld_mx, const int32_t* cu_seqlens, const int32_t* qblocks,
                        int n_qblocks, int q_heads, int kv_heads, void* stream) {
  TTV_CHECK_ARG(n_qblocks >= 0 && (n_qblocks == 0 || (qkvg && out_q && out_mx && cu_seqlens && qblocks)), "attention_mxout: null buffer");
  return ttvk_attention_mxout(qkvg, ld, out_q, out_mx, ld_mx, cu_seqlens, qblocks, n_qblocks, q_heads, kv_heads, (hipStream_t)stream);
}

int ttv_linear_fp8_mx_geglu_q(const void* xq, int ldx, const void* x_mx, const float* x_row_scale, const void* wq, int ldw, const void* w_mx,
                              const float* w_row_scale, void* hq, void* hq_mx, int M, int N, int K, void* stream) {
  TTV_CHECK_ARG(M == 0 || (xq && wq && x_mx && w_mx && hq && hq_mx), "linear_fp8_mx_geglu_q: null buffer");
  GemmArgs a = gemm_args(TTV_BF16, xq, ldx, wq, ldw, M, N, K, hq, N);
  a.yq = hq; a.yq_mx = hq_mx;
  return ttvk_gemm_fp8(EPI_GEGLU, a, x_row_scale, w_row_scale, (hipStream_t)stream, x_mx, w_mx);
}

int ttv_row_rstd(const void* x, int dtype, int ldx, float* rstd, int rows, int width, float eps, void* stream) {
  TTV_CHECK_ARG(rows >= 0 && (rows == 0 || (x && rstd)), "row_rstd: null buffer");
  TTV_CHECK_ARG(ldx >= width, "row_rstd: leading dim smaller than the width");
  return ttvk_row_rstd(x, dtype, ldx, rstd, rows, width, eps, (hipStream_t)stream);
}

int ttv_linear_rowscale(const void* x, int ldx, const void* w, int ldw, const float* row_scale, int epilogue, const float* rope_cs, int d_model,
                        int gqa_dim, void* y, int ldy, int M, int N, int K, int dtype, void* stream) {
  TTV_CHECK_ARG(M == 0 || (x && w && y), "linear_rowscale: null buffer");
  TTV_CHECK_ARG(epilogue >= 0 && epilogue <= 2, "linear_rowscale: epilogue 0 (store), 1 (qkv + rotary) or 2 (GEGLU)");
  GemmArgs a = gemm_args(dtype, x, ldx, w, ldw, M, N, K, y, ldy);
  if (epilogue == 1) {
    TTV_CHECK_ARG(rope_cs && N == 2 * d_model + 2 * gqa_dim && K == d_model, "linear_rowscale: qkv epilogue needs rope_cs, N = 2 d_model + 2 gqa_dim and K = d_model");
    a = gemm_rope_qk(a, rope_cs, d_model, gqa_dim);
  }
  a.row_scale = row_scale;
  return ttvk_gemm(epilogue == 0 ? EPI_STORE : epilogue == 1 ? EPI_QKV_ROPE : EPI_GEGLU, a, (hipStream_t)stream);
}

int ttv_patch_gather(const void* const* clips, const int32_t* clip_desc, int clip0, int n_clips, int patch_t, int patch_h, int patch_w,
                     int channels, void* patches, int ld, int dtype, int max_patches_per_clip, void* stream) {
  TTV_CHECK_ARG(n_clips == 0 || (clips && clip_desc && patches), "patch_gather: null buffer");
  return ttvk_patch_copy(false, (void* const*)clips, clip_desc, clip0, n_clips, patch_t, patch_h, patch_w, channels, patches, ld, dtype, max_patches_per_clip, (hipStream_t)stream);
}

int ttv_patch_embed_norm(const void* const* clips, const int32_t* clip_desc, const int32_t* patch_rows, const int32_t* row_seq, int n_clips,
                         int patch_t, int patch_h, int patch_w, int channels, const void* w, int ldw, const void* bias, const float* mask_token,
                         const float* gain, float eps, void* x, int ldx, int rows, int width, int dtype, void* stream) {
  TTV_CHECK_ARG(rows == 0 || (clips && clip_desc && patch_rows && row_seq && w && bias && mask_token && gain && x), "patch_embed_norm: null buffer");
  const int pd = channels * patch_t * patch_h * patch_w;
  if (!ttvk_patch_embed_norm_supported(dtype, width, pd, patch_w)) {
    ttv_set_error("patch_embed_norm: only bf16, width 256, patch_w 8 and a patch vector that is a multiple of 64");
    return TTV_ERR_UNSUPPORTED;
  }
  return ttvk_patch_embed_norm((void* const*)clips, 0, n_clips, clip_desc, patch_rows, row_seq, patch_t, patch_h, patch_w, pd, w, ldw, bias,
                               mask_token, gain, eps, x, ldx, rows, (hipStream_t)stream);
}

int ttv_patch_scatter(const void* patches, int ld, const int32_t* clip_desc, int clip0, int n_clips, int patch_t, int patch_h, int patch_w,
                      int channels, void* const* clips, int dtype, int max_patches_per_clip, void* stream) {
  TTV_CHECK_ARG(n_clips == 0 || (clips && clip_desc && patches), "patch_scatter: null buffer");
  return ttvk_patch_copy(true, clips, clip_desc, clip0, n_clips, patch_t, patch_h, patch_w, channels, (void*)patches, ld, dtype, max_patches_per_clip, (hipStream_t)stream);
}

int64_t ttv_tower_workspace_bytes(const ttv_tower_dims* dims, const ttv_batch* batch) {
  if (check_dims(dims, batch) != TTV_OK) return -1;
  return carve(dims, batch, nullptr).total;
}

int ttv_encoder_forward(const ttv_tower_dims* d, const ttv_tower_weights* w, const ttv_batch* b, const void* const* clips,
                        const ttv_fsq_params* fsq, float* z, void* codes, int32_t* indices, float* bounded, void* workspace,
                        int64_t workspace_bytes, void* stream) {
  TTV_TRY(check_dims(d, b));
  TTV_CHECK_ARG(d->kind == TTV_ENCODER, "encoder_forward: dims.kind is not TTV_ENCODER");
  TTV_CHECK_ARG(w && w->layers && clips && workspace, "encoder_forward: null argument");
  TTV_CHECK_ARG(fsq || z, "encoder_forward: neither fsq nor z requested");
  TTV_CHECK_ARG(!fsq || (codes && indices), "encoder_forward: fsq needs codes and indices buffers");
  hipStream_t s = (hipStream_t)stream;
  TowerWs ws = carve(d, b, (char*)workspace);
  TTV_CHECK_ARG(ws.total <= workspace_bytes, "encoder_forward: workspace too small (%lld < %lld)", (long long)workspace_bytes, (long long)ws.total);
  const int dm = d->width, dt = d->dtype, P = b->sum_patches, pd = patch_dim(d);

  static const bool embed_env = ttv_env_flag("TTV_PATCH_EMBED_FUSED", true);
  if (embed_env && !(g_ttv_debug & TTV_DBG_PATCH_EMBED_UNFUSED) && fused_patch_ok(d, b, dt) && w->proj_in_b && w->mask_token &&
      ttvk_patch_embed_norm_supported(dt, dm, pd, d->patch_w)) {
    TTV_TRY(ttvk_patch_embed_norm((void* const*)clips, 0, b->n_clips, b->clip_desc, b->patch_rows, b->row_seq, d->patch_t, d->patch_h, d->patch_w,
                                  pd, w->proj_in_w, pd, w->proj_in_b, w->mask_token, w->ln_pre_p, d->eps, ws.x, dm, P, s));
  } else {
    const bool gather = fused_patch_ok(d, b, dt) && pd != 256;
    if (!gather) TTV_TRY(patch_copy_all(false, (void* const*)clips, d, b, ws.pa, dt, s));
    GemmArgs a = gemm_args(dt, ws.pa, pd, w->proj_in_w, pd, P, dm, pd, ws.pb, dm);
    a.bias = w->proj_in_b; a.add_scalar = w->mask_token;
    a.split3 = (dt == TTV_F32 && w->f32_split3) ? 1 : 0;
    if (gather) {
      a.gather = 1; a.clips = (void* const*)clips; a.n_clips = b->n_clips; a.clip_desc = b->clip_desc; a.patch_rows = b->patch_rows;
      a.row_seq = b->row_seq; a.patch_t = d->patch_t; a.patch_h = d->patch_h; a.patch_w = d->patch_w;
    }
    TTV_TRY(ttvk_gemm(EPI_STORE, a, s));
    TTV_TRY(ttvk_rmsnorm(ws.pb, dt, dm, nullptr, ws.x, dt, dm, b->patch_rows, w->ln_pre_p, P, dm, d->eps, s));
  }
  TTV_TRY(ttvk_fill_const_rows(ws.x, dt, dm, b->latent_rows, b->sum_tokens, dm, w->mask_token, w->ln_pre_t, d->eps, s));

  TTV_TRY(run_layers(d, w, b, ws, s));

  TTV_TRY(ttvk_enc_tail(ws.x, dt, dm, b->latent_rows, b->sum_tokens, dm, w->ln_post, d->eps, w->proj_out_w, w->proj_out_b, d->token_size, fsq, z, codes, indices, bounded, s));
  return TTV_OK;
}

int64_t ttv_dec_l0_const_bytes(const ttv_tower_dims* d, int patch_rows) {
  if (!d || patch_rows <= 0 || d->dtype != TTV_BF16 || d->width != 256 || d->head_dim != 64 || d->kv_heads <= 0) {
    ttv_set_error("dec_l0_const_bytes: bf16 decoders of width 256 and head_dim 64 only");
    return -1;
  }
  if (patch_rows % 128) {
    ttv_set_error("dec_l0_const_bytes: patch_rows must be a multiple of 128");
    return -1;
  }
  const int64_t nq = 2 * (int64_t)d->width + 2 * (int64_t)d->kv_heads * d->head_dim;
  return align256(patch_rows * nq * 2) + align256(ttvk_attention_swp_state_floats(patch_rows, d->q_heads) * 4 + 4) + align256((int64_t)patch_rows * d->width * 2);
}

int ttv_dec_l0_const_build(const ttv_tower_dims* d, const ttv_tower_weights* w, const int32_t* iota, const float* rope_cs, const int32_t* rope_ids,
                           const float* rope_base, int patch_rows, void* block, int64_t block_bytes, int64_t* state_offset, int64_t* flag_offset,
                           void* stream) {
  TTV_CHECK_ARG(d && w && w->layers && iota && rope_cs && block && patch_rows > 0, "dec_l0_const_build: null argument");
  const int64_t need = ttv_dec_l0_const_bytes(d, patch_rows);
  if (need < 0) return TTV_ERR_UNSUPPORTED;
// ... 254 lines not shown
```

titok_video_amd/csrc/ttv_kernels.h:

```cpp
#pragma once
#include <hip/hip_runtime.h>
#include <stdint.h>

#include "../../include/titok_hip.h"

int ttvk_rmsnorm(const void* in, int in_dtype, int ld_in, const int* src_rows, void* out, int out_dtype, int ld_out,
                 const int* dst_rows, const float* gain, int rows, int d, float eps, hipStream_t s, float* next_rstd = nullptr,
                 void* mx_q = nullptr, void* mx_s = nullptr,
                 int split_image = 0);
int ttvk_row_rstd(const void* in, int dtype, int ld_in, float* rstd, int rows, int d, float eps, hipStream_t s);
int ttvk_copy_rows(const void* src, int64_t ld_src_bytes, const int* src_rows, void* dst, int64_t ld_dst_bytes, const int* dst_rows, int rows,
                   int row_bytes, hipStream_t s);
int ttvk_fill_const_rows(void* x, int dtype, int ld, const int* rows_map, int rows, int d, const float* mask_token,
                         const float* gain, float eps, hipStream_t s);
int ttvk_dec_embed(const void* codes, int C, const void* w, const void* bias, const float* mask_token, const float* gain,
                   void* x, int dtype, int ld, const int* rows_map, int rows, int d, float eps, hipStream_t s);
int ttvk_fsq_forward(const ttv_fsq_params* p, const void* z, int z_dtype, int rows, void* codes, int codes_dtype, int* indices,
                     float* bounded, hipStream_t s);
int ttvk_fsq_indices_to_codes(const ttv_fsq_params* p, const int* indices, int rows, void* codes, int codes_dtype, hipStream_t s);
int ttvk_enc_tail(const void* x, int dtype, int ld, const int* rows_map, int rows, int d, const float* gain, float eps,
                  const void* w, const void* bias, int C, const ttv_fsq_params* fsq, float* z_out, void* codes, int* indices,
                  float* bounded, hipStream_t s);
int ttvk_patch_copy(bool scatter, void* const* clips, const int* clip_desc, int clip0, int n_clips, int pt, int ph, int pw,
                    int C, void* patches, int ld, int dtype, int max_patches, hipStream_t s);
int ttvk_rope_apply(void* x, int dtype, int ld, int rows, int heads, const float* cs, hipStream_t s);
int ttvk_histogram(const int* idx, int n, int64_t* counts, int size, hipStream_t s);
int ttvk_quant_rows_fp8(const void* in, int in_dtype, int ld_in, const float* gain, float eps, void* out, int ld_out, float* scales, int rows,
                        int d, hipStream_t s);

int ttvk_split3_pack(const float* w, int ldw, void* out, int ldo, int rows, int K, hipStream_t s);
int64_t ttvk_mx_scale_ld(int d);
int ttvk_quant_mx_fp8(const void* in, int in_dtype, int ld_in, void* out, int ld_out, void* mx, float* row_scales, int rows, int d, hipStream_t s);

int ttvk_clip_from_u8(const void* frames, long long n_pix, void* clip, int dtype, hipStream_t s);

int ttvk_clip_resample_u8(void* const* src, void* const* dst, const int32_t* geom, int n_clips, int dtype, hipStream_t s);

enum GemmEpilogue {
  EPI_STORE = 0,
  EPI_QKV_ROPE,
  EPI_GEGLU,
  EPI_RESID_T,
  EPI_RESID_F32,
  EPI_RESID_NORM,
  EPI_STORE_PATCH,
  EPI_BIAS_PLAIN,
  EPI_BIAS_GELU,
  EPI_BIAS_RESID_F32R,
};

struct GemmArgs {
  const void* x; int ldx;
  const void* w; int ldw;
  int M, N, K;
  void* y; int ldy;
  const void* bias;
  const float* add_scalar;
  const void* resid; int ldr;
  float alpha;
  const float* rope_cs;
  const int* rope_ids; const float* rope_base;
  int rope_q_end, rope_k_begin, rope_k_end;
  int dtype;
  const float* norm_gain;
  float* sum_f32; int ld_sum;
  void* y2; int ldy2; const float* norm_gain2;
  void* yq; void* yq_mx;
  int split3;
  int x_image, y_image;
  int prenorm;
  const float* row_scale;
  const int* x_rows;
  float eps;
  int gather;
  void* const* clips;
  int n_clips;
  const int* clip_desc;
  const int* patch_rows;
  const int* row_seq;
  int patch_t, patch_h, patch_w;
  int resid_rows;
  int tile_run, tile_period;
  int panel_lo;
};
struct ClipPtrs { void* p[TTV_MAX_CLIPS_PER_LAUNCH]; };
int ttvk_gemm(GemmEpilogue epi, const GemmArgs& a, hipStream_t s);
int ttvk_gemm_fp8(GemmEpilogue epi, const GemmArgs& a, const float* x_scale, const float* w_scale, hipStream_t s, const void* x_mx = nullptr,
                  const void* w_mx = nullptr);
bool ttvk_gemm_supports_resid_norm(int dtype, int N, int K);
bool ttvk_gemm_qkv_tiles_supported(int d_model, int gqa_dim, int ldw);

bool ttvk_patch_embed_norm_supported(int dtype, int width, int patch_dim, int patch_w);
int ttvk_patch_embed_norm(void* const* clips, int clip0, int n_clips, const int* clip_desc, const int* patch_rows, const int* row_seq,
                          int patch_t, int patch_h, int patch_w, int patch_dim, const void* w, int ldw, const void* bias,
                          const float* mask_token, const float* gain, float eps, void* x, int ldx, int M, hipStream_t s);

int ttvk_attention(const void* qkvg, int ld, void* out, int ldo, const int* cu_seqlens, const int* qblocks, int n_qblocks,
                   int q_heads, int kv_heads, int head_dim, int flags, int dtype, hipStream_t s, float* lse_out = nullptr,
                   void* out_raw = nullptr);

bool ttvk_attention_takes_swp(int flags);
int ttvk_attention_swp(const void* qkvg, int ld, void* out, int ldo, const int* cu_seqlens, const int* qblocks, int n_qblocks,
                       int q_heads, int kv_heads, int gate_mul, hipStream_t s, const void* rows2 = nullptr, int kwin = 0,
                       const float* state = nullptr);
int64_t ttvk_attention_swp_state_floats(int n_rows, int q_heads);
int ttvk_attention_swp_dump(const void* rows, int ld, int n_rows, int q_heads, int kv_heads, float* state, hipStream_t s);
int ttvk_attention_mxout(const void* qkvg, int ld, void* out_q, void* out_mx, int ld_mx, const int* cu_seqlens, const int* qblocks,
                         int n_qblocks, int q_heads, int kv_heads, hipStream_t s);

int ttvk_attention64(const void* qkvg, int ld, void* out, int ldo, const int* cu_seqlens, const int* items, int n_items, int q_heads,
                     int kv_heads, int flags, hipStream_t s);

int ttvk_vq_norms(const void* cb, int dtype, int ld, int N, int C, float* cnorm, hipStream_t s);
int64_t ttvk_vq_workspace_bytes(int rows);
int ttvk_vq_l2_argmin(const void* z, int dtype, int ldz, const void* cb, int ldc, const float* cnorm, int rows, int N, int C, int* indices,
                      float* best_dist, void* workspace, int64_t workspace_bytes, hipStream_t s);
int ttvk_vq_lookup(const void* cb, int dtype, int ldc, const int* indices, int rows, int C, void* codes, int ldo, hipStream_t s);
int ttvk_vq_lookup_bwd(const void* dcodes, int dtype, int ld, const int* indices, int rows, int C, float* dcb, int ldc, hipStream_t s);

int64_t ttvk_vq_train_workspace_bytes(int rows, int N);
int ttvk_vq_commit_forward(const void* z, int dtype, int ldz, const void* cb, int ldc, const int* idx, int rows, int N, int C, float* loss,
                           void* workspace, int64_t workspace_bytes, hipStream_t s);
int ttvk_vq_commit_backward(const void* g, int ldg, const void* z, int ldz, const void* e, int lde, int dtype, int rows, int C, double scale,
                            void* dz, int ldd, hipStream_t s);
int ttvk_vq_ema_stats(const void* z, int dtype, int ldz, const int* idx, int rows, int N, int C, const float* cluster_size, float dead_threshold,
                      uint64_t seed, const int64_t* ema_step, int rank, int world_size, float* stats, void* workspace, int64_t workspace_bytes,
                      hipStream_t s);
int ttvk_vq_ema_update(const float* stats, float* cluster_size, float* embed_avg, float* codebook, void* copy, int copy_dtype, float* cnorm,
                       int64_t* ema_step, int N, int C, float decay, float one_minus_decay, float eps, float dead_threshold, void* workspace,
                       int64_t workspace_bytes, hipStream_t s);

bool ttvk_mlp_fused_supported(int dtype, int width, int inner);
struct MlpNextQkv {
  void* qkv; int ld;
  const float* rope_cs;
  int rows;
  int rope_q_end, rope_k_begin, rope_k_end;
};
int64_t ttvk_mlp_pack_bytes(int inner, int next_qkv_rows);
int ttvk_mlp_pack(const void* w12_folded, const void* w3, const void* wo, const void* next_qkv_folded, int next_qkv_rows, int inner,
                  void* packed, hipStream_t s);
int ttvk_mlp_fused(const void* ao, int ldao, const float* front_gain, float front_alpha, const void* x, int ldx, const void* packed,
                   int inner, void* y, int ldy, const float* post_gain, float alpha, float eps, int M, const MlpNextQkv* nq, hipStream_t s);

int ttvk_l1_loss(void* const* recon, void* const* target, void* const* grad, const int* sizes, int n_clips, int total_clips, int dtype,
                 float* loss, hipStream_t s);
int ttvk_sq_err(void* const* recon, void* const* target, const int* sizes, int n_clips, int dtype, int clamp, double* acc2, hipStream_t s);
int ttvk_rmsnorm_bwd_chain(const void* x, int ldx, const void* dy, int lddy, const float* gain1, float* dgain1, float* dx, int lddx,
                           const void* y, int y_dt, int ldy, const float* gain2, float* dgain2, float out_scale, void* cast_out, int ldc, int rows,
                           int d, float eps, int dt, hipStream_t s);
int ttvk_rmsnorm_bwd(const void* x, int x_dt, int ldx, const int* xr, const void* dy, int dy_dt, int lddy, const int* dyr,
                     const float* gain, void* dx, int dx_dt, int lddx, const int* dxr, int acc, float* dgain, int rows, int d, float eps,
                     hipStream_t s);
int ttvk_colsum(const void* a, int dt, int lda, const int* rows_map, int rows, int n, float* out, hipStream_t s);
int ttvk_sumall(const void* a, int dt, int lda, const int* rows_map, int rows, int n, const float* colw, float scale, float* out, hipStream_t s);
int ttvk_gate_fwd(const void* a, int lda, const void* gate, int ldg, void* ag, int ldo, int rows, int d, int dt, hipStream_t s);
int ttvk_gate_bwd(const void* dag, int ldd, const void* a, int lda, const void* gate, int ldg, void* da, int ldda, void* dgate, int lddg,
                  int rows, int d, int dt, float* delta, hipStream_t s);
int ttvk_geglu_fwd(const void* u, int ldu, void* h, int ldh, int rows, int I, int dt, hipStream_t s);
int ttvk_geglu_bwd(const void* u, int ldu, const void* dh, int lddh, void* du, int lddu, int rows, int I, int dt, hipStream_t s);
int ttvk_scale_cast(const float* a, float alpha, float* b, void* c, int dt, long n, hipStream_t s);
int ttvk_to_f32(const void* a, int dt, float* b, long n, int accumulate, hipStream_t s);
int ttvk_fsq_bwd(const ttv_fsq_params* fp, const float* z, const void* dcodes, int dt, float* dz, int rows, hipStream_t s);
#define TTV_WGRAD_BATCH 6
struct WgradBatch {
  int n = 0;
  int64_t used_bytes = 0;
  struct Entry { const float* part; float* dw; int splits, lddw, N, K, tiles_n, tiles; } e[TTV_WGRAD_BATCH];
};
int ttvk_wgrad(const void* dy, int lddy, const void* x, int ldx, float* dw, int lddw, int L, int N, int K, int dt, float* part,
               int64_t part_bytes, hipStream_t s, WgradBatch* batch = nullptr);
int ttvk_wgrad_flush(WgradBatch* batch, hipStream_t s);
int64_t ttvk_wgrad_ws_bytes(int L, int N, int K);
int ttvk_outer_small(const void* a, int a_dt, int lda, int C, const void* b, int b_dt, int ldb, const int* b_rows, float* dw, int lddw,
                     int transpose_out, int rows, int d, hipStream_t s);
int ttvk_expand_small(const void* a, int a_dt, int lda, int C, const void* w, int w_dt, int ldw, int w_cf, void* out, int o_dt, int ldo,
                      int rows, int d, hipStream_t s);
int ttvk_reduce_small(const void* a, int a_dt, int lda, const int* a_rows, const void* w, int w_dt, int ldw, int C, float* out, int ldo,
                      int rows, int d, hipStream_t s);
int ttvk_attention_bwd(const void* qkvg, int ld, const void* o, int ldo, const void* dout, int ldd, const float* lse, float* delta,
                       const int* cu, const int* blocks64, int n_blocks64, const int* row_seq, void* dqkvg, int ldg, float* dkv_scratch,
                       int total_rows, int hq, int hkv, int dt, const float* rope_cs, hipStream_t s, int delta_ready = 0, const int* qlim_desc = nullptr);
int ttvk_rope_apply_dir(void* x, int dtype, int ld, int rows, int heads, const float* cs, int conj, hipStream_t s);
int ttvk_dec_embed_ex(const void* codes, int C, const void* w, const void* bias, const float* mask_token, const float* gain, void* x,
                      int dtype, int ld, const int* rows_map, int rows, int d, float eps, void* hpre, hipStream_t s);
int ttvk_const_rows_bwd(const float* colsum, const float* mask_token, const float* gain, int dt, float eps, float* dgain, float* dmask,
                        int d, hipStream_t s);
int ttvk_rope_build(const float* base_cos, const float* base_sin, int n_ids, int F, const int* clip_desc, const int* cu, const int* row_seq,
                    float* out, int total_rows, hipStream_t s);

int64_t ttvk_ssim_workspace_bytes(const int32_t* dims, int n_clips);
int ttvk_ssim(void* const* recon, void* const* target, const int32_t* dims, int n_clips, int dtype, int clamp, double* acc2, void* workspace,
              int64_t workspace_bytes, hipStream_t s);

int ttvk_lpips_crops_forward(void* const* recon, void* const* target, const int32_t* clip_dims, int n_clips, const int32_t* crops, int n_crops,
                             int size, void* recon_crops, void* target_crops, int dtype, hipStream_t s);
int ttvk_lpips_crops_backward(void* const* recon, void* const* grad, const int32_t* clip_dims, int n_clips, const int32_t* crops, int n_crops,
                              int size, const void* g, int dtype, hipStream_t s);

int64_t ttvk_lpips_tape_bytes(int n, int H, int W, int dtype);
int64_t ttvk_lpips_workspace_bytes(int n, int H, int W, int dtype);
int ttvk_lpips_forward(const ttv_lpips_weights* w, const void* recon, const void* target, int n, int H, int W, int dtype, float* lpips,
                       float* gram, void* tape, void* ws, int64_t ws_bytes, hipStream_t s);
int ttvk_lpips_backward(const ttv_lpips_weights* w, const void* tape, int n, int H, int W, int dtype, const float* glpips, const float* ggram,
                        void* drecon, void* ws, int64_t ws_bytes, hipStream_t s);
int64_t ttvk_lpips_eval_workspace_bytes(int frames, int H, int W, int dtype);
int ttvk_lpips_eval_accumulate(const ttv_lpips_weights* w, void* const* recon, void* const* target, const int32_t* frames, int n_clips, int H,
                               int W, int dtype, int clamp_recon, float* per_frame, double* acc, void* ws, int64_t ws_bytes, hipStream_t s);
int64_t ttvk_lpips_conv_workspace_bytes(int N, int H, int W, int Cin, int Cout, int dtype);
int ttvk_lpips_conv3x3(const void* x, int N, int H, int W, int Cin, int Cout, const void* w, const float* bias, int mode, const void* h,
                       void* y, int dtype, void* ws, int64_t ws_bytes, hipStream_t s);
int ttvk_lpips_maxpool(const void* x, int N, int H, int W, int C, void* y, int dtype, hipStream_t s);
int ttvk_lpips_maxpool_backward(const void* dy, const float* add, const void* h, int N, int H, int W, int C, void* dx, int dtype, hipStream_t s);

int64_t ttvk_i3d_workspace_bytes(int n);
int ttvk_fvd_preprocess(void* const* clips, const int32_t* dims, int n_clips, int dtype, int clamp, float* out, hipStream_t s);
int ttvk_i3d_features(const ttv_i3d_weights* w, const float* x, int n, float* feats, void* ws, int64_t ws_bytes, hipStream_t s);
int ttvk_i3d_conv3d(const float* x, int N, int T, int H, int W, int Cin, int k, int stride, const float* w, const float* scale,
                    const float* shift, int Cout, int relu, float* y, int ldc, int c_off, hipStream_t s);
int ttvk_i3d_maxpool3d(const float* x, int N, int T, int H, int W, int C, int kt, int kh, int kw, int st, int sh, int sw, float* y,
                       hipStream_t s);

int ttvk_jedi_preprocess(void* const* clips, const int32_t* dims, int n_clips, int dtype, void* out, hipStream_t s);
int64_t ttvk_vjepa_workspace_bytes(int n);
int ttvk_vjepa_features(const ttv_vjepa_weights* w, const void* x, int n, float* feats, int finetuned, void* ws, int64_t ws_bytes,
                        hipStream_t s);
int ttvk_vjepa_layernorm(const float* x, int ldx, int rows, int width, const float* w1, const float* b1, float eps1, const float* w2,
                         const float* b2, float eps2, float* y32, int ld32, void* y16, int ld16, hipStream_t s);
int ttvk_vjepa_linear(const void* x, int ldx, const void* w, int ldw, const void* bias, int M, int N, int K, int epilogue,
                      const float* resid, int ldr, int resid_rows, void* y, int ldy, hipStream_t s);
int ttvk_vjepa_pool_attention(const void* q, const void* kv, int n, int rows, void* out, hipStream_t s);

#define TTV_TRY(expr)                \
  do {                               \
    const int rc__ = (expr);         \
    if (rc__ != TTV_OK) return rc__; \
  } while (0)

static inline int64_t align256(int64_t v) { return (v + 255) & ~(int64_t)255; }
static inline int dtype_bytes(int dt) { return dt == TTV_BF16 ? 2 : 4; }
static inline int patch_dim(const ttv_tower_dims* d) { return d->pix_channels * d->patch_t * d->patch_h * d->patch_w; }
static inline float keel_alpha(const ttv_tower_dims* d, int layer) { return layer == 0 ? 1.f : d->alpha; }

static inline GemmArgs gemm_args(int dtype, const void* x, int ldx, const void* w, int ldw, int M, int N, int K, void* y, int ldy) {
  GemmArgs a = {};
  a.dtype = dtype; a.x = x; a.ldx = ldx; a.w = w; a.ldw = ldw; a.M = M; a.N = N; a.K = K; a.y = y; a.ldy = ldy;
  return a;
}
static inline GemmArgs gemm_rope_qk(GemmArgs a, const float* rope_cs, int d_model, int gqa_dim) {
  a.rope_cs = rope_cs; a.rope_q_end = d_model; a.rope_k_begin = 2 * d_model; a.rope_k_end = 2 * d_model + gqa_dim;
  return a;
}
static inline GemmArgs gemm_resid(GemmArgs a, const void* resid, int ldr, float alpha) {
  a.resid = resid; a.ldr = ldr; a.alpha = alpha;
  return a;
}

static inline int gather_rows(const void* src, void* dst, const int* index, int n_rows, int64_t row_bytes, hipStream_t s) {
  return ttvk_copy_rows(src, row_bytes, index, dst, row_bytes, nullptr, n_rows, (int)row_bytes, s);
}
static inline int scatter_rows(const void* src, void* dst, const int* index, int n_rows, int64_t row_bytes, hipStream_t s) {
  return ttvk_copy_rows(src, row_bytes, nullptr, dst, row_bytes, index, n_rows, (int)row_bytes, s);
}

template <typename F> static inline int for_clip_groups(int n_clips, F f) {
  for (int c0 = 0; c0 < n_clips; c0 += TTV_MAX_CLIPS_PER_LAUNCH) {
    const int n = n_clips - c0 < TTV_MAX_CLIPS_PER_LAUNCH ? n_clips - c0 : TTV_MAX_CLIPS_PER_LAUNCH;
    TTV_TRY(f(c0, n));
  }
  return TTV_OK;
}
static inline int patch_copy_all(bool scatter, void* const* clips, const ttv_tower_dims* d, const ttv_batch* b, void* buf, int dtype, hipStream_t s) {
  return for_clip_groups(b->n_clips, [&](int c0, int n) {
    return ttvk_patch_copy(scatter, clips + c0, b->clip_desc, c0, n, d->patch_t, d->patch_h, d->patch_w, d->pix_channels, buf, patch_dim(d), dtype,
                           b->max_patches_per_clip, s);
  });
}
```

titok_video_amd/csrc/ttv_mlp.hip:

```cpp
#include "ttv_common.h"
#include "ttv_kernels.h"

#define MLP_W12_CHUNKS 2048
#define MLP_W3_CHUNKS 1024
#define MLP_PANEL_CHUNKS (MLP_W12_CHUNKS + MLP_W3_CHUNKS)
#define MLP_WO_CHUNKS (4 * MLP_W12_CHUNKS)

struct MlpDev {
  const bf16_t* x; int ldx;
  const uint4* pack;
  const bf16_t* ao; int ldao;
  const float* front_gain;
  float front_alpha;
  bf16_t* qkv; int ldq;
  const float* rope_cs;
  int nqp, rope_q_end, rope_k_begin, rope_k_end;
  int I;
  bf16_t* y; int ldy;
  const float* post_gain;
  float alpha, eps;
  int M, n_tiles, debug;
  long long* stamps;
};

__global__ void k_mlp_pack(const bf16_t* __restrict__ w12f, const bf16_t* __restrict__ w3, const bf16_t* __restrict__ wo,
                           const bf16_t* __restrict__ wq, int nq_rows, int I, uint4* __restrict__ out) {
  const int np = I / 32;
  const int nqp = (nq_rows + 63) / 64;
  const int o = blockIdx.x * blockDim.x + threadIdx.x;
  if (o >= np * MLP_PANEL_CHUNKS + MLP_WO_CHUNKS + nqp * MLP_W12_CHUNKS) return;
  if (o >= np * MLP_PANEL_CHUNKS + MLP_WO_CHUNKS) {
    const int c = o - np * MLP_PANEL_CHUNKS - MLP_WO_CHUNKS, qp = c / MLP_W12_CHUNKS, cc = c - qp * MLP_W12_CHUNKS;
    const int r = cc >> 5, cp = cc & 31;
    const int ch = (cp & 16) | ((cp & 15) ^ (r & 15));
    int srow = qp * 64 + r;
    srow = srow < nq_rows ? srow : nq_rows - 1;
    const bf16_t* src = wq + (size_t)srow * 256 + (ch >> 2) * 32 + (ch & 3) * 4;
    const uint2 lo = *reinterpret_cast<const uint2*>(src), hi = *reinterpret_cast<const uint2*>(src + 16);
    out[o] = make_uint4(lo.x, lo.y, hi.x, hi.y);
    return;
  }
  if (o >= np * MLP_PANEL_CHUNKS) {
    const int c = o - np * MLP_PANEL_CHUNKS, wp = c / MLP_W12_CHUNKS, cc = c - wp * MLP_W12_CHUNKS;
    const int r = cc >> 5, cp = cc & 31;
    const int ch = (cp & 16) | ((cp & 15) ^ (r & 15));
    out[o] = wo ? *reinterpret_cast<const uint4*>(wo + (size_t)(wp * 64 + r) * 256 + ch * 8) : make_uint4(0, 0, 0, 0);
    return;
  }
  const int pn = o / MLP_PANEL_CHUNKS, c = o - pn * MLP_PANEL_CHUNKS;
  if (c < MLP_W12_CHUNKS) {
    const int r = c >> 5, cp = c & 31;
    const int ch = (cp & 16) | ((cp & 15) ^ (r & 15));
    const int srow = r < 32 ? pn * 32 + r : I + pn * 32 + (r - 32);
    const bf16_t* src = w12f + (size_t)srow * 256 + (ch >> 2) * 32 + (ch & 3) * 4;
    const uint2 lo = *reinterpret_cast<const uint2*>(src), hi = *reinterpret_cast<const uint2*>(src + 16);
    out[o] = make_uint4(lo.x, lo.y, hi.x, hi.y);
  } else {
    const int c3 = c - MLP_W12_CHUNKS, kq = c3 >> 8, row = c3 & 255;
    bf16x8 v;
#pragma unroll
    for (int j = 0; j < 8; ++j) v[j] = w3[(size_t)row * I + pn * 32 + (j < 4 ? 4 * kq + j : 16 + 4 * kq + (j - 4))];
    out[o] = __builtin_bit_cast(uint4, v);
  }
}

typedef uint32_t u32x2_t __attribute__((ext_vector_type(2)));
typedef uint32_t u32x4_t __attribute__((ext_vector_type(4)));
__device__ __forceinline__ f32x4 cvt4(bf16x4 b) { return (f32x4){(float)b[0], (float)b[1], (float)b[2], (float)b[3]}; }
#define MLP_LD12(img_, t_, s8_)                                                                                    \
  __builtin_bit_cast(bf16x8, (img_)[((t_) * 16 + l15) * 32 + ((((s8_) * 4 + kq) & 16) | ((((s8_) * 4 + kq) & 15) ^ l15))])
#define MLP_GLDS_4(src_, dst_)                                                                                     \
  do {                                                                                                             \
    unsigned keep__;                                                                                               \
    asm volatile("s_mov_b32 %0, m0\n\t"                                                                            \
                 "s_mov_b32 m0, %6\n\ts_nop 0\n\tglobal_load_lds_dwordx4 %1, %5\n\t"                               \
                 "s_add_u32 m0, %6, 0x2000\n\ts_nop 0\n\tglobal_load_lds_dwordx4 %2, %5\n\t"                       \
                 "s_add_u32 m0, %6, 0x4000\n\ts_nop 0\n\tglobal_load_lds_dwordx4 %3, %5\n\t"                       \
                 "s_add_u32 m0, %6, 0x6000\n\ts_nop 0\n\tglobal_load_lds_dwordx4 %4, %5\n\t"                       \
                 "s_mov_b32 m0, %0"                                                                                \
                 : "=&s"(keep__)                                                                                   \
                 : "v"(lane16), "v"(lane16 + 8192u), "v"(lane16 + 16384u), "v"(lane16 + 24576u), "s"(src_), "s"(dst_) \
                 : "memory", "scc");                                                                               \
  } while (0)
#define MLP_GLDS_2(src_, dst_)                                                                                     \
  do {                                                                                                             \
    unsigned keep__;                                                                                               \
    asm volatile("s_mov_b32 %0, m0\n\t"                                                                            \
                 "s_mov_b32 m0, %4\n\ts_nop 0\n\tglobal_load_lds_dwordx4 %1, %3\n\t"                               \
                 "s_add_u32 m0, %4, 0x2000\n\ts_nop 0\n\tglobal_load_lds_dwordx4 %2, %3\n\t"                       \
                 "s_mov_b32 m0, %0"                                                                                \
                 : "=&s"(keep__)                                                                                   \
                 : "v"(lane16), "v"(lane16 + 8192u), "s"(src_), "s"(dst_)                                          \
                 : "memory", "scc");                                                                               \
  } while (0)
#ifdef MLP_STAMPS
#define MLP_STAMP()                                                                                                \
  do {                                                                                                             \
    if (p.stamps && blockIdx.x == 0 && (wave & 3) == 0 && lane == 0 && n_stamp < 64)                               \
      p.stamps[(wave >> 2) * 64 + n_stamp++] = (long long)__builtin_readcyclecounter();                            \
  } while (0)
#else
#define MLP_STAMP() do { (void)n_stamp; } while (0)
#endif

template <int TPB, int T1, int T2, bool GELU_FIRST, bool KEEL, bool FRONT, bool BACK>
__device__ __forceinline__ void mlp_wave(const MlpDev& p, uint4* l12, uint4* l3, uint4* hb, const float* gl, int tile, int wave, int lane,
                                         int P1F, int P2F, int& n_stamp) {
  constexpr int T1A = T1 > 0 ? T1 : 1, T2A = T2 > 0 ? T2 : 1;
  const int l15 = lane & 15, kq = lane >> 4;
  const int np = p.I / 32;
  const uint32_t lane16 = lane * 16;
  const uint32_t lds_l12 = (uint32_t)(uintptr_t)(__attribute__((address_space(3))) void*)l12;
  const uint32_t lds_l3 = (uint32_t)(uintptr_t)(__attribute__((address_space(3))) void*)l3;
#define GLDS_W12(pn_, buf_)                                                                                        \
  do {                                                                                                             \
    const uint4* src__ = p.pack + ((size_t)(pn_) * MLP_PANEL_CHUNKS + wave * 64);                                  \
    const uint32_t dst__ = lds_l12 + ((buf_) * MLP_W12_CHUNKS + wave * 64) * 16;                                   \
    MLP_GLDS_4(src__, dst__);                                                                                      \
  } while (0)
#define GLDS_W3(pn_, buf_)                                                                                         \
  do {                                                                                                             \
    const uint4* src__ = p.pack + ((size_t)(pn_) * MLP_PANEL_CHUNKS + MLP_W12_CHUNKS + wave * 64);                 \
    const uint32_t dst__ = lds_l3 + ((buf_) * MLP_W3_CHUNKS + wave * 64) * 16;                                     \
    MLP_GLDS_2(src__, dst__);                                                                                      \
  } while (0)

  const int tok0 = tile * (16 * TPB) + l15;
  typedef __attribute__((address_space(1))) char gchar;
  typedef __attribute__((address_space(1))) const char gcchar;
  gcchar* const gx = (gcchar*)p.x;
  gcchar* const gao = (gcchar*)p.ao;
  gchar* const gy = (gchar*)p.y;

  MLP_STAMP();
  __syncthreads();

  bf16x8 bfr[T1A][8];
  float rstd[T1A];
  if (FRONT) {
#define GLDS_WO(wp_, buf_)                                                                                         \
  do {                                                                                                             \
    const uint4* src__ = p.pack + ((size_t)np * MLP_PANEL_CHUNKS + (wp_) * MLP_W12_CHUNKS + wave * 64);            \
    const uint32_t dst__ = lds_l12 + ((buf_) * MLP_W12_CHUNKS + wave * 64) * 16;                                   \
    MLP_GLDS_4(src__, dst__);                                                                                      \
  } while (0)
    GLDS_WO(0, 0);
    bf16x8 abf[T1A][8];
#pragma unroll
    for (int j = 0; j < T1; ++j) {
      const int t = tok0 + 16 * (P1F + j);
      const int tc = t < p.M ? t : p.M - 1;
      const uint32_t aoff = ((uint32_t)tc * (uint32_t)p.ldao + kq * 8) * 2u;
#pragma unroll
      for (int s8 = 0; s8 < 8; ++s8) abf[j][s8] = *(const __attribute__((address_space(1))) bf16x8*)(gao + aoff + s8 * 64);
    }
    f32x4 facc[16][T1A];
    __builtin_amdgcn_s_waitcnt(0x0F70);
    __syncthreads();
#pragma unroll
    for (int wp = 0; wp < 4; ++wp) {
      if (wp + 1 < 4) GLDS_WO(wp + 1, (wp + 1) & 1);
      const uint4* img = l12 + (wp & 1) * MLP_W12_CHUNKS;
      bf16x8 a[2][4];
      if constexpr (T1 > 0) {
#pragma unroll
      for (int i = 0; i < 4; ++i) a[0][i] = MLP_LD12(img, i, 0);
#pragma unroll
      for (int s8 = 0; s8 < 8; ++s8) {
        if (s8 + 1 < 8) {
#pragma unroll
          for (int i = 0; i < 4; ++i) a[(s8 + 1) & 1][i] = MLP_LD12(img, i, s8 + 1);
        }
#pragma unroll
        for (int i = 0; i < 4; ++i)
#pragma unroll
          for (int j = 0; j < T1; ++j)
            facc[4 * wp + i][j] = __builtin_amdgcn_mfma_f32_16x16x32_bf16(a[s8 & 1][i], abf[j][s8],
                                                                           s8 ? facc[4 * wp + i][j] : (f32x4){0.f, 0.f, 0.f, 0.f}, 0, 0, 0);
        if (s8 + 1 < 8) __builtin_amdgcn_sched_group_barrier(0x100, 4, 0);
        __builtin_amdgcn_sched_group_barrier(0x008, 4 * T1A, 0);
        __builtin_amdgcn_sched_barrier(0);
      }
      }
      __builtin_amdgcn_s_waitcnt(0x0F70);
      __syncthreads();
    }
#undef GLDS_WO
    GLDS_W12(0, 0);
#pragma unroll
    for (int j = 0; j < T1; ++j) {
      const int t = tok0 + 16 * (P1F + j);
      const int tc = t < p.M ? t : p.M - 1;
      const uint32_t roff = ((uint32_t)tc * (uint32_t)p.ldx + kq * 4) * 2u;
      float ss = 0.f;
#pragma unroll
      for (int m = 0; m < 16; ++m) {
        facc[m][j] += p.front_alpha * cvt4(*(const __attribute__((address_space(1))) bf16x4*)(gx + roff + m * 32));
#pragma unroll
        for (int e = 0; e < 4; ++e) ss = fmaf(facc[m][j][e], facc[m][j][e], ss);
      }
      float scale = 1.0f;
      if (p.front_gain) {
        ss = quad16_sum(ss);
        scale = 1.0f / sqrtf(ss * (1.0f / 256.0f) + p.eps);
      }
      float ss2 = 0.f;
#pragma unroll
      for (int s8 = 0; s8 < 8; ++s8) {
        bf16x4 q[2];
#pragma unroll
        for (int u = 0; u < 2; ++u) {
          const int m = 2 * s8 + u;
          f32x4 v = facc[m][j];
          if (p.front_gain) {
            const f32x4 g = *reinterpret_cast<const f32x4*>(gl + 256 + m * 16 + kq * 4);
#pragma unroll
            for (int e = 0; e < 4; ++e) v[e] = v[e] * scale * g[e];
          }
          q[u] = (bf16x4){(bf16_t)v[0], (bf16_t)v[1], (bf16_t)v[2], (bf16_t)v[3]};
#pragma unroll
          for (int e = 0; e < 4; ++e) {
            const float r = (float)q[u][e];
            ss2 = fmaf(r, r, ss2);
          }
        }
        bfr[j][s8] = (bf16x8){q[0][0], q[0][1], q[0][2], q[0][3], q[1][0], q[1][1], q[1][2], q[1][3]};
      }
      ss2 = quad16_sum(ss2);
      rstd[j] = 1.0f / sqrtf(ss2 * (1.0f / 256.0f) + p.eps);
    }
  } else {
    GLDS_W12(0, 0);
#pragma unroll
    for (int j = 0; j < T1; ++j) {
      const int t = tok0 + 16 * (P1F + j);
      const int tc = t < p.M ? t : p.M - 1;
      const uint32_t xoff = ((uint32_t)tc * (uint32_t)p.ldx + kq * 4) * 2u;
#pragma unroll
      for (int s8 = 0; s8 < 8; ++s8) {
        const u32x2_t lo = *(const __attribute__((address_space(1))) u32x2_t*)(gx + xoff + s8 * 64);
        const u32x2_t hi = *(const __attribute__((address_space(1))) u32x2_t*)(gx + xoff + (s8 * 64 + 32));
        bfr[j][s8] = __builtin_bit_cast(bf16x8, (u32x4_t){lo.x, lo.y, hi.x, hi.y});
      }
    }
#pragma unroll
    for (int j = 0; j < T1; ++j) {
      float ss = 0.f;
#pragma unroll
      for (int s8 = 0; s8 < 8; ++s8)
#pragma unroll
        for (int e = 0; e < 8; ++e) {
          const float v = (float)bfr[j][s8][e];
          ss = fmaf(v, v, ss);
        }
      ss = quad16_sum(ss);
      rstd[j] = 1.0f / sqrtf(ss * (1.0f / 256.0f) + p.eps);
    }
  }
  f32x4 out[16][T2A];
#pragma unroll
  for (int m = 0; m < 16; ++m)
#pragma unroll
    for (int j = 0; j < T2; ++j) out[m][j] = (f32x4){0.f, 0.f, 0.f, 0.f};

  __builtin_amdgcn_s_waitcnt(0x0F70);
  __syncthreads();
  MLP_STAMP();

  for (int it = 0; it <= np; ++it) {
    if (it + 1 < np && !(p.debug & TTV_DBG_MLP_NO_WEIGHT_DMA)) GLDS_W12(it + 1, (it + 1) & 1);
    if (it < np && (!(p.debug & TTV_DBG_MLP_NO_WEIGHT_DMA) || it == 0)) GLDS_W3(it, it & 1);

    f32x4 acc1[4][T1A];
    if (T1 > 0 && it < np) {
      const uint4* img = l12 + (it & 1) * MLP_W12_CHUNKS;
      bf16x8 a[2][4];
#pragma unroll
      for (int i = 0; i < 4; ++i) a[0][i] = MLP_LD12(img, i, 0);
#pragma unroll
      for (int s8 = 0; s8 < 8; ++s8) {
// ... 103 lines not shown
  bf16x8 xq[T2A][8];
  float rstdq[T2A];
#pragma unroll
  for (int j = 0; j < T2; ++j) {
    const int t = tok0 + 16 * (P2F + j);
    const bool tv = t < p.M;
    const int tc = tv ? t : p.M - 1;
    const uint32_t roff = ((uint32_t)tc * (uint32_t)p.ldx + kq * 4) * 2u;
    float ss = 0.f;
#pragma unroll
    for (int s8 = 0; s8 < 8; ++s8) {
      f32x4 rv0, rv1;
      if (FRONT) {
        const bf16x8 rb = __builtin_bit_cast(bf16x8, xres[((P2F + j) * 8 + s8) * 64 + lane]);
        rv0 = (f32x4){(float)rb[0], (float)rb[1], (float)rb[2], (float)rb[3]};
        rv1 = (f32x4){(float)rb[4], (float)rb[5], (float)rb[6], (float)rb[7]};
      } else {
        rv0 = cvt4(*(const __attribute__((address_space(1))) bf16x4*)(gx + roff + (2 * s8) * 32));
        rv1 = cvt4(*(const __attribute__((address_space(1))) bf16x4*)(gx + roff + (2 * s8 + 1) * 32));
      }
      out[2 * s8][j] += p.alpha * rv0;
      out[2 * s8 + 1][j] += p.alpha * rv1;
#pragma unroll
      for (int e = 0; e < 4; ++e) {
        ss = fmaf(out[2 * s8][j][e], out[2 * s8][j][e], ss);
        ss = fmaf(out[2 * s8 + 1][j][e], out[2 * s8 + 1][j][e], ss);
      }
    }
    float scale = 1.0f;
    if (KEEL) {
      ss = quad16_sum(ss);
      scale = 1.0f / sqrtf(ss * (1.0f / 256.0f) + p.eps);
    }
    const bool odd = kq & 1;
    const uint32_t yoff = ((uint32_t)tc * (uint32_t)p.ldy + (odd ? 16 + kq * 4 - 4 : kq * 4)) * 2u;
    float ssq = 0.f;
#pragma unroll
    for (int ip = 0; ip < 8; ++ip) {
      const int i0 = 2 * ip, i1 = 2 * ip + 1;
      f32x4 y0 = out[i0][j], y1 = out[i1][j];
      if (KEEL) {
        const f32x4 g0 = *reinterpret_cast<const f32x4*>(gl + i0 * 16 + kq * 4);
        const f32x4 g1 = *reinterpret_cast<const f32x4*>(gl + i1 * 16 + kq * 4);
#pragma unroll
        for (int e = 0; e < 4; ++e) { y0[e] = y0[e] * scale * g0[e]; y1[e] = y1[e] * scale * g1[e]; }
      }
      const bf16x4 q0 = {(bf16_t)y0[0], (bf16_t)y0[1], (bf16_t)y0[2], (bf16_t)y0[3]};
      const bf16x4 q1 = {(bf16_t)y1[0], (bf16_t)y1[1], (bf16_t)y1[2], (bf16_t)y1[3]};
      const uint2 p0 = __builtin_bit_cast(uint2, q0), p1 = __builtin_bit_cast(uint2, q1);
      if (BACK) {
        xq[j][ip] = __builtin_bit_cast(bf16x8, make_uint4(p0.x, p0.y, p1.x, p1.y));
#pragma unroll
        for (int e = 0; e < 4; ++e) {
          const float r0 = (float)q0[e], r1 = (float)q1[e];
          ssq = fmaf(r0, r0, ssq);
          ssq = fmaf(r1, r1, ssq);
        }
      }
      const uint4 ov = xchg16_pair(p0, p1);
      if (tv && !(p.debug & TTV_DBG_NO_STORES)) *(__attribute__((address_space(1))) u32x4_t*)(gy + yoff + ip * 64) = (u32x4_t){ov.x, ov.y, ov.z, ov.w};
    }
    if (BACK) {
      ssq = quad16_sum(ssq);
      rstdq[j] = 1.0f / sqrtf(ssq * (1.0f / 256.0f) + p.eps);
    }
  }
  MLP_STAMP();

  if (BACK) {
#define GLDS_WQ(qp_, buf_)                                                                                         \
  do {                                                                                                             \
    const uint4* src__ = p.pack + ((size_t)np * MLP_PANEL_CHUNKS + MLP_WO_CHUNKS + (qp_) * MLP_W12_CHUNKS + wave * 64); \
    const uint32_t dst__ = lds_l12 + ((buf_) * MLP_W12_CHUNKS + wave * 64) * 16;                                   \
    MLP_GLDS_4(src__, dst__);                                                                                      \
  } while (0)
    __syncthreads();
    GLDS_WQ(0, 0);
    gchar* const gq = (gchar*)p.qkv;
    gcchar* const grope = (gcchar*)p.rope_cs;
    f32x2 rc[4][T2A], rs[4][T2A];
    uint32_t qoff[T2A];
    bool qv[T2A];
#pragma unroll
    for (int j = 0; j < T2; ++j) {
      const int t = tok0 + 16 * (P2F + j);
      qv[j] = t < p.M;
      const int tc = qv[j] ? t : p.M - 1;
      qoff[j] = ((uint32_t)tc * (uint32_t)p.ldq + kq * 4) * 2u;
      gcchar* cs = grope + ((uint32_t)tc * 64u + kq * 2) * 4u;
#pragma unroll
      for (int i = 0; i < 4; ++i) {
        rc[i][j] = *(const __attribute__((address_space(1))) f32x2*)(cs + i * 32);
        rs[i][j] = *(const __attribute__((address_space(1))) f32x2*)(cs + 128 + i * 32);
      }
    }
    __builtin_amdgcn_s_waitcnt(0x0F70);
    __syncthreads();
    for (int qp = 0; qp < p.nqp; ++qp) {
      if (qp + 1 < p.nqp) GLDS_WQ(qp + 1, (qp + 1) & 1);
      const uint4* img = l12 + (qp & 1) * MLP_W12_CHUNKS;
      f32x4 qa[4][T2A];
      bf16x8 a[2][4];
#pragma unroll
      for (int i = 0; i < 4; ++i) a[0][i] = MLP_LD12(img, i, 0);
#pragma unroll
      for (int s8 = 0; s8 < 8; ++s8) {
        if (s8 + 1 < 8) {
#pragma unroll
          for (int i = 0; i < 4; ++i) a[(s8 + 1) & 1][i] = MLP_LD12(img, i, s8 + 1);
        }
#pragma unroll
        for (int i = 0; i < 4; ++i)
#pragma unroll
          for (int j = 0; j < T2; ++j)
            qa[i][j] = __builtin_amdgcn_mfma_f32_16x16x32_bf16(a[s8 & 1][i], xq[j][s8], s8 ? qa[i][j] : (f32x4){0.f, 0.f, 0.f, 0.f}, 0, 0, 0);
        if (s8 + 1 < 8) __builtin_amdgcn_sched_group_barrier(0x100, 4, 0);
        __builtin_amdgcn_sched_group_barrier(0x008, 4 * T2A, 0);
        __builtin_amdgcn_sched_barrier(0);
      }
      __builtin_amdgcn_s_waitcnt(0x0F70);
      __syncthreads();
      const int f_first = qp * 64;
      const bool rot = f_first < p.rope_q_end || (f_first >= p.rope_k_begin && f_first < p.rope_k_end);
#pragma unroll
      for (int j = 0; j < T2; ++j) {
        const bool odd = kq & 1;
        gchar* const qrow = gq + (qoff[j] - (uint32_t)(kq * 4) * 2u) + (uint32_t)(f_first + (odd ? 16 + kq * 4 - 4 : kq * 4)) * 2u;
#pragma unroll
        for (int ip = 0; ip < 2; ++ip) {
          uint2 pk[2];
#pragma unroll
          for (int u = 0; u < 2; ++u) {
            const int i = 2 * ip + u;
            f32x4 v = qa[i][j] * rstdq[j];
            if (rot)
              v = (f32x4){v[0] * rc[i][j].x - v[1] * rs[i][j].x, v[0] * rs[i][j].x + v[1] * rc[i][j].x,
                          v[2] * rc[i][j].y - v[3] * rs[i][j].y, v[2] * rs[i][j].y + v[3] * rc[i][j].y};
            const bf16x4 q = {(bf16_t)v[0], (bf16_t)v[1], (bf16_t)v[2], (bf16_t)v[3]};
            pk[u] = __builtin_bit_cast(uint2, q);
          }
          const uint4 ox = xchg16_pair(pk[0], pk[1]);
          const u32x4_t ov = {ox.x, ox.y, ox.z, ox.w};
          if (qv[j]) *(__attribute__((address_space(1))) u32x4_t*)(qrow + ip * 64) = ov;
        }
      }
    }
#undef GLDS_WQ
    MLP_STAMP();
  }
#undef GLDS_W12
#undef GLDS_W3
}

template <int TILES, bool KEEL, bool FRONT, bool BACK>
__global__ __launch_bounds__(512, 1) void k_mlp256(MlpDev p) {
  extern __shared__ __attribute__((aligned(16))) uint4 smem[];
  uint4* const l12 = smem;
  uint4* const l3 = smem + 2 * MLP_W12_CHUNKS;
  uint4* const hb = l3 + 2 * MLP_W3_CHUNKS;
  float* const gl = reinterpret_cast<float*>(hb + 2 * TILES * 64);
  if (threadIdx.x < 256) {
    gl[threadIdx.x] = p.post_gain ? p.post_gain[threadIdx.x] : 1.0f;
    gl[256 + threadIdx.x] = (FRONT && p.front_gain) ? p.front_gain[threadIdx.x] : 1.0f;
  }
  const int lane = threadIdx.x & 63;
  const int wave = __builtin_amdgcn_readfirstlane(threadIdx.x >> 6);
  int n_stamp = 0;
  const int tile = blockIdx.x;
  if constexpr (TILES == 9) {
    if (wave < 4) mlp_wave<9, 2, 0, false, KEEL, FRONT, BACK>(p, l12, l3, hb, gl, tile, wave, lane, 2 * wave, 0, n_stamp);
    else if (wave < 6) mlp_wave<9, 0, 3, false, KEEL, FRONT, BACK>(p, l12, l3, hb, gl, tile, wave, lane, 0, 3 * (wave - 4), n_stamp);
    else if (wave == 6) mlp_wave<9, 1, 1, false, KEEL, FRONT, BACK>(p, l12, l3, hb, gl, tile, wave, lane, 8, 6, n_stamp);
    else mlp_wave<9, 0, 2, false, KEEL, FRONT, BACK>(p, l12, l3, hb, gl, tile, wave, lane, 0, 7, n_stamp);
  } else {
    constexpr int NT = TILES / 4;
    constexpr int TA = NT - NT / 2;
    const int g0 = (wave & 3) * NT;
    if (wave < 4) mlp_wave<TILES, TA, NT - TA, false, KEEL, FRONT, BACK>(p, l12, l3, hb, gl, tile, wave, lane, g0, g0 + TA, n_stamp);
    else mlp_wave<TILES, NT - TA, TA, false, KEEL, FRONT, BACK>(p, l12, l3, hb, gl, tile, wave, lane, g0 + TA, g0, n_stamp);
  }
}
#undef MLP_LD12
#undef MLP_GLDS_4
#undef MLP_GLDS_2
#undef MLP_STAMP

bool ttvk_mlp_fused_supported(int dtype, int width, int inner) { return dtype == TTV_BF16 && width == 256 && inner % 32 == 0 && inner > 0; }

int64_t ttvk_mlp_pack_bytes(int inner, int next_qkv_rows) {
  if (inner <= 0 || inner % 32 != 0 || next_qkv_rows < 0) return 0;
  return ((int64_t)(inner / 32) * MLP_PANEL_CHUNKS + MLP_WO_CHUNKS + (int64_t)((next_qkv_rows + 63) / 64) * MLP_W12_CHUNKS) * 16;
}

int ttvk_mlp_pack(const void* w12_folded, const void* w3, const void* wo, const void* next_qkv_folded, int next_qkv_rows, int inner,
                  void* packed, hipStream_t s) {
  TTV_CHECK_ARG(w12_folded && w3 && packed, "mlp_pack: null buffer");
  TTV_CHECK_ARG(inner > 0 && inner % 32 == 0, "mlp_pack: inner %% 32");
  TTV_CHECK_ARG((next_qkv_folded != nullptr) == (next_qkv_rows > 0), "mlp_pack: next_qkv weight and row count must come together");
  TTV_CHECK_ARG(((uintptr_t)w12_folded % 16 == 0) && ((uintptr_t)packed % 16 == 0) && ((uintptr_t)wo % 16 == 0) &&
                    ((uintptr_t)next_qkv_folded % 16 == 0), "mlp_pack: 16-byte alignment");
  const int total = inner / 32 * MLP_PANEL_CHUNKS + MLP_WO_CHUNKS + (next_qkv_rows + 63) / 64 * MLP_W12_CHUNKS;
  hipLaunchKernelGGL(k_mlp_pack, dim3(ttv_cdiv(total, 256)), dim3(256), 0, s, (const bf16_t*)w12_folded, (const bf16_t*)w3,
                     (const bf16_t*)wo, (const bf16_t*)next_qkv_folded, next_qkv_rows, inner, (uint4*)packed);
  TTV_CHECK_LAUNCH("mlp_pack");
  return TTV_OK;
}

int ttvk_mlp_fused(const void* ao, int ldao, const float* front_gain, float front_alpha, const void* x, int ldx, const void* packed,
                   int inner, void* y, int ldy, const float* post_gain, float alpha, float eps, int M, const MlpNextQkv* nq, hipStream_t s) {
  if (M == 0) return TTV_OK;
  TTV_CHECK_ARG(x && packed && y, "mlp_fused: null buffer");
  TTV_CHECK_ARG(inner % 32 == 0 && ldx % 8 == 0 && ldy % 8 == 0 && (!ao || ldao % 8 == 0), "mlp_fused: inner %% 32, leading dims %% 8");
  TTV_CHECK_ARG(((uintptr_t)x % 16 == 0) && ((uintptr_t)packed % 16 == 0) && ((uintptr_t)y % 16 == 0) && ((uintptr_t)ao % 16 == 0),
                "mlp_fused: 16-byte alignment");
  MlpDev d;
  d.x = (const bf16_t*)x; d.ldx = ldx; d.pack = (const uint4*)packed; d.I = inner;
  d.ao = (const bf16_t*)ao; d.ldao = ldao; d.front_gain = front_gain; d.front_alpha = front_alpha;
  d.y = (bf16_t*)y; d.ldy = ldy; d.post_gain = post_gain; d.alpha = alpha; d.eps = eps; d.M = M; d.debug = g_ttv_debug; d.stamps = g_ttv_stamps;
  d.qkv = nullptr; d.ldq = 0; d.rope_cs = nullptr; d.nqp = 0; d.rope_q_end = d.rope_k_begin = d.rope_k_end = 0;
  if (nq) {
    TTV_CHECK_ARG(nq->qkv && nq->rope_cs && nq->rows > 0 && nq->rows % 64 == 0 && nq->ld >= nq->rows && nq->ld % 4 == 0 &&
                      (uintptr_t)nq->qkv % 8 == 0, "mlp_fused: bad next-qkv arguments (rows %% 64, ld %% 4, 8-byte aligned)");
    TTV_CHECK_ARG(nq->rope_q_end % 64 == 0 && nq->rope_k_begin % 64 == 0 && nq->rope_k_end % 64 == 0, "mlp_fused: rotary ranges must be whole heads");
    d.qkv = (bf16_t*)nq->qkv; d.ldq = nq->ld; d.rope_cs = nq->rope_cs; d.nqp = nq->rows / 64;
    d.rope_q_end = nq->rope_q_end; d.rope_k_begin = nq->rope_k_begin; d.rope_k_end = nq->rope_k_end;
  }
  const int cus = 256;
  int tiles = 4;
  long best = -1;
  for (int c = 1; c <= 3; ++c) {
    const long cost = (long)ttv_cdiv(ttv_cdiv(M, 64 * c), cus) * (16 + 19 * c);
    if (best < 0 || cost < best) { best = cost; tiles = 4 * c; }
  }
  if (!nq && !(g_ttv_debug & TTV_DBG_MLP_PAIRS_ONLY)) {
    const long cost9 = (long)ttv_cdiv(ttv_cdiv(M, 144), cus) * (16 + 14 * 3);
    if (cost9 < best) { best = cost9; tiles = 9; }
  }
  if ((g_ttv_debug & TTV_DBG_MLP_TILES9) && !nq) tiles = 9;
  if (g_ttv_debug & TTV_DBG_MLP_TILES8) tiles = 8;
  if (g_ttv_debug & TTV_DBG_MLP_TILES4) tiles = 4;
  d.n_tiles = ttv_cdiv(M, 16 * tiles);
  const int grid = d.n_tiles;
  const size_t smem = (size_t)(2 * MLP_W12_CHUNKS + 2 * MLP_W3_CHUNKS + 2 * tiles * 64) * sizeof(uint4) + 2048;
  TtvProfScope prof(TTV_KC_GEMM_GEGLU, s);
#define LAUNCH_MLP(TILES_, KEEL_, FRONT_, BACK_)                                                                    \
  do {                                                                                                              \
    (void)hipFuncSetAttribute((const void*)k_mlp256<TILES_, KEEL_, FRONT_, BACK_>, hipFuncAttributeMaxDynamicSharedMemorySize, (int)smem); \
    hipLaunchKernelGGL((k_mlp256<TILES_, KEEL_, FRONT_, BACK_>), dim3(grid), dim3(512), smem, s, d);                \
  } while (0)
#define LAUNCH_MLP_F(TILES_, KEEL_)                                                                                 \
  do {                                                                                                              \
    if (ao && nq) LAUNCH_MLP(TILES_, KEEL_, true, true);                                                            \
    else if (ao) LAUNCH_MLP(TILES_, KEEL_, true, false);                                                            \
    else LAUNCH_MLP(TILES_, KEEL_, false, false);                                                                   \
  } while (0)
#define LAUNCH_MLP_9(KEEL_)                                                                                         \
  do {                                                                                                              \
    if (ao) LAUNCH_MLP(9, KEEL_, true, false);                                                                      \
    else LAUNCH_MLP(9, KEEL_, false, false);                                                                        \
  } while (0)
  TTV_CHECK_ARG(!nq || ao, "mlp_fused: the next-qkv part needs the out_proj front (ttv_layer_tail_fused)");
  if (post_gain) {
    if (tiles == 9) LAUNCH_MLP_9(true); else if (tiles == 12) LAUNCH_MLP_F(12, true); else if (tiles == 8) LAUNCH_MLP_F(8, true); else LAUNCH_MLP_F(4, true);
  } else {
    if (tiles == 9) LAUNCH_MLP_9(false); else if (tiles == 12) LAUNCH_MLP_F(12, false); else if (tiles == 8) LAUNCH_MLP_F(8, false); else LAUNCH_MLP_F(4, false);
  }
#undef LAUNCH_MLP_9
#undef LAUNCH_MLP_F
#undef LAUNCH_MLP
  TTV_CHECK_LAUNCH("mlp_fused");
  return TTV_OK;
}
```

titok_video_amd/csrc/ttv_patch_embed.hip:

```cpp
#include "ttv_common.h"
#include "ttv_kernels.h"

#define PE_TT 128
#define PE_F 256
#define PE_BK 64
#define PE_STAGES 3
#define PE_STAGE_U4 ((PE_F + PE_TT) * 8)

struct PatchEmbedDev {
  ClipPtrs clips;
  const int* clip_desc; const int* patch_rows; const int* row_seq;
  const bf16_t* w; const bf16_t* bias; const float* mask_token; const float* gain;
  bf16_t* x;
  int ldw, ldx, M, K, clip0, pt_shift, ph_shift;
  float eps;
};

__global__ __launch_bounds__(512, 1) void k_patch_embed256(PatchEmbedDev p) {
  __shared__ __attribute__((aligned(16))) uint4 lds[PE_STAGES][PE_STAGE_U4];
  const int tid = threadIdx.x, lane = tid & 63;
  const int wave = __builtin_amdgcn_readfirstlane(tid >> 6);
  const int wf = wave & 1, wt = wave >> 1;
  const int tbase = blockIdx.x * PE_TT;

  const int lr = lane >> 3, lp = lane & 7;
  uint32_t woff[4];
#pragma unroll
  for (int i = 0; i < 4; ++i) {
    const int row = wave * 32 + i * 8 + lr;
    woff[i] = ((uint32_t)row * (uint32_t)p.ldw + (uint32_t)((lp ^ ((row >> 1) & 7)) * 8)) * 2u;
  }
  const bf16_t* gbase[2];
  int gthw[2], ghw[2], gw_[2], gch[2];
#pragma unroll
  for (int i = 0; i < 2; ++i) {
    const int row = wave * 16 + i * 8 + lr;
    int t = tbase + row;
    t = t < p.M ? t : p.M - 1;
    const int ci = p.row_seq[p.patch_rows[t]];
    const int* ds = p.clip_desc + (size_t)ci * 8;
    const int Tn = ds[0], H = ds[1], W = ds[2], gh = ds[4], gw = ds[5], pl = t - ds[6];
    const int gwi = pl % gw, r = pl / gw, ghi = r % gh, gti = r / gh;
    gthw[i] = Tn * H * W; ghw[i] = H * W; gw_[i] = W;
    gch[i] = lp ^ ((row >> 1) & 7);
    gbase[i] = reinterpret_cast<const bf16_t*>(p.clips.p[ci - p.clip0]) + ((size_t)((gti << p.pt_shift) * H + (ghi << p.ph_shift)) * W + gwi * 8);
  }
  const uint32_t lds0 = (uint32_t)(uintptr_t)(__attribute__((address_space(3))) void*)&lds[0][0];
  constexpr uint32_t STAGEB = PE_STAGE_U4 * 16;
#define PE_DMA_W(voff_, base_, dst_)                                                                             \
  do {                                                                                                           \
    unsigned keep__;                                                                                             \
    asm volatile("s_mov_b32 %0, m0\n\ts_mov_b32 m0, %3\n\ts_nop 0\n\tglobal_load_lds_dwordx4 %1, %2\n\ts_mov_b32 m0, %0" \
                 : "=&s"(keep__) : "v"(voff_), "s"(base_), "s"(dst_) : "memory");                                 \
  } while (0)
#define PE_DMA_X(ptr_, dst_)                                                                                     \
  do {                                                                                                           \
    unsigned keep__;                                                                                             \
    asm volatile("s_mov_b32 %0, m0\n\ts_mov_b32 m0, %2\n\ts_nop 0\n\tglobal_load_lds_dwordx4 %1, off\n\ts_mov_b32 m0, %0" \
                 : "=&s"(keep__) : "v"(ptr_), "s"(dst_) : "memory");                                              \
  } while (0)
#define PE_STAGE(kt_, st_)                                                                                       \
  do {                                                                                                           \
    const bf16_t* wb__ = p.w + (size_t)(kt_) * PE_BK;                                                            \
    const uint32_t dw__ = lds0 + (st_) * STAGEB + wave * 4096;                                                   \
    const uint32_t dx__ = lds0 + (st_) * STAGEB + PE_F * 128 + wave * 2048;                                      \
    _Pragma("unroll") for (int i__ = 0; i__ < 4; ++i__) PE_DMA_W(woff[i__], wb__, dw__ + i__ * 1024);            \
    _Pragma("unroll") for (int i__ = 0; i__ < 2; ++i__) {                                                        \
      const int sg__ = (kt_) * 8 + gch[i__];                                                                     \
      const int c__ = sg__ >> (p.pt_shift + p.ph_shift), ipt__ = (sg__ >> p.ph_shift) & ((1 << p.pt_shift) - 1); \
      const int iph__ = sg__ & ((1 << p.ph_shift) - 1);                                                          \
      const bf16_t* src__ = gbase[i__] + ((size_t)c__ * gthw[i__] + (size_t)ipt__ * ghw[i__] + (size_t)iph__ * gw_[i__]); \
      PE_DMA_X(src__, dx__ + i__ * 1024);                                                                        \
    }                                                                                                            \
  } while (0)

  f32x4 acc[8][2];
#pragma unroll
  for (int i = 0; i < 8; ++i)
#pragma unroll
    for (int j = 0; j < 2; ++j) acc[i][j] = (f32x4){0.f, 0.f, 0.f, 0.f};

  const int l15 = lane & 15, kq = lane >> 4;
  const int nk = p.K / PE_BK;
  const char* const ldsb = reinterpret_cast<const char*>(&lds[0][0]);
  const uint32_t fo0 = (uint32_t)(l15 * 128 + (((0 + kq) ^ ((l15 >> 1) & 7)) << 4));
  const uint32_t fo1 = (uint32_t)(l15 * 128 + (((4 + kq) ^ ((l15 >> 1) & 7)) << 4));
  const uint32_t a_base = (uint32_t)(wf * 128 * 128), b_base = (uint32_t)(PE_F * 128 + wt * 32 * 128);

  asm volatile("s_waitcnt vmcnt(0)" ::: "memory");
  PE_STAGE(0, 0);
  if (nk > 1) PE_STAGE(1, 1);
  int st = 0;
  for (int kt = 0; kt < nk; ++kt) {
    if (kt + 1 < nk) asm volatile("s_waitcnt vmcnt(6)" ::: "memory");
    else asm volatile("s_waitcnt vmcnt(0)" ::: "memory");
    __syncthreads();
    if (kt + 2 < nk) {
      const int st2 = st + 2 >= PE_STAGES ? st + 2 - PE_STAGES : st + 2;
      PE_STAGE(kt + 2, st2);
    }
    const char* const sb = ldsb + (size_t)st * STAGEB;
#pragma unroll
    for (int ks = 0; ks < 2; ++ks) {
      const uint32_t fo = ks ? fo1 : fo0;
      bf16x8 a[8], b[2];
#pragma unroll
      for (int i = 0; i < 8; ++i) a[i] = *reinterpret_cast<const bf16x8*>(sb + a_base + fo + i * 2048);
#pragma unroll
      for (int j = 0; j < 2; ++j) b[j] = *reinterpret_cast<const bf16x8*>(sb + b_base + fo + j * 2048);
#pragma unroll
      for (int i = 0; i < 8; ++i)
#pragma unroll
        for (int j = 0; j < 2; ++j) acc[i][j] = __builtin_amdgcn_mfma_f32_16x16x32_bf16(a[i], b[j], acc[i][j], 0, 0, 0);
    }
    st = st + 1 == PE_STAGES ? 0 : st + 1;
  }
#undef PE_STAGE
#undef PE_DMA_W
#undef PE_DMA_X

  const float sc = round_to<bf16_t>(p.mask_token[0]);
  float* const gx = reinterpret_cast<float*>(&lds[st][0]);
  float grp[8][2];
#pragma unroll
  for (int i = 0; i < 8; ++i) {
    const int f = wf * 128 + i * 16 + kq * 4;
    const f32x4 bv = Vec4<bf16_t>::load(p.bias + f);
#pragma unroll
    for (int j = 0; j < 2; ++j) {
      acc[i][j] += bv;
#pragma unroll
      for (int e = 0; e < 4; ++e)
        acc[i][j][e] = round_to<bf16_t>(round_to<bf16_t>(acc[i][j][e]) + sc);
      const f32x4 y = acc[i][j];
      grp[i][j] = fmaf(y[3], y[3], fmaf(y[2], y[2], fmaf(y[0], y[0], y[1] * y[1])));
      gx[(wf * PE_TT + wt * 32 + j * 16 + l15) * 33 + i * 4 + kq] = grp[i][j];
    }
  }
  __syncthreads();
#pragma unroll
  for (int j = 0; j < 2; ++j) {
    const int tl = wt * 32 + j * 16 + l15;
    const int t = tbase + tl;
    float s1[8];
#pragma unroll
    for (int i = 0; i < 8; ++i) s1[i] = grp[i][j] + gx[((wf ^ 1) * PE_TT + tl) * 33 + i * 4 + kq];
    const float t0 = s1[0] + s1[4], t1 = s1[1] + s1[5], t2 = s1[2] + s1[6], t3 = s1[3] + s1[7];
    float tot = (t0 + t2) + (t1 + t3);
    tot = pair32_sum(tot);
    {
      const unsigned u = __float_as_uint(tot);
      const auto a = __builtin_amdgcn_permlane16_swap(u, u, false, false);
      const unsigned a0 = a[0], a1 = a[1];
      tot = __uint_as_float(a0) + __uint_as_float(a1);
    }
    const float rstd = 1.0f / sqrtf(tot / 256.0f + p.eps);
    if (t < p.M) {
      bf16_t* const q = p.x + (size_t)p.patch_rows[t] * p.ldx;
#pragma unroll
      for (int i = 0; i < 8; ++i) {
        const int f = wf * 128 + i * 16 + kq * 4;
        const f32x4 g = *reinterpret_cast<const f32x4*>(p.gain + f);
        const f32x4 o = {acc[i][j][0] * rstd * g[0], acc[i][j][1] * rstd * g[1], acc[i][j][2] * rstd * g[2], acc[i][j][3] * rstd * g[3]};
        Vec4<bf16_t>::store(q + f, o);
      }
    }
  }
}

bool ttvk_patch_embed_norm_supported(int dtype, int width, int patch_dim, int patch_w) {
  return dtype == TTV_BF16 && width == PE_F && patch_dim % PE_BK == 0 && patch_dim >= PE_BK && patch_w == 8;
}

int ttvk_patch_embed_norm(void* const* clips, int clip0, int n_clips, const int* clip_desc, const int* patch_rows, const int* row_seq,
                          int patch_t, int patch_h, int patch_w, int patch_dim, const void* w, int ldw, const void* bias,
                          const float* mask_token, const float* gain, float eps, void* x, int ldx, int M, hipStream_t s) {
  if (M == 0) return TTV_OK;
  auto lg2 = [](int v) { int sh = 0; while ((1 << sh) < v) ++sh; return (1 << sh) == v ? sh : -1; };
  TTV_CHECK_ARG(patch_w == 8 && lg2(patch_t) >= 0 && lg2(patch_h) >= 0 && patch_dim % PE_BK == 0 && patch_dim >= PE_BK &&
                    patch_dim % (patch_t * patch_h * patch_w) == 0,
                "patch_embed_norm: patch_w == 8, power-of-two patch_t / patch_h and a patch vector that is a multiple of 64");
  TTV_CHECK_ARG(n_clips > 0 && n_clips <= TTV_MAX_CLIPS_PER_LAUNCH, "patch_embed_norm: 1 .. %d clips per call", TTV_MAX_CLIPS_PER_LAUNCH);
  TTV_CHECK_ARG(ldw >= patch_dim && ldw % 8 == 0 && ldx >= PE_F && ldx % 4 == 0 && (uint64_t)PE_F * (uint64_t)ldw * 2u < (1ull << 32),
                "patch_embed_norm: leading dims must hold a row and keep its alignment");
  TTV_CHECK_ARG((uintptr_t)w % 16 == 0 && (uintptr_t)x % 8 == 0 && (uintptr_t)bias % 8 == 0 && (uintptr_t)gain % 16 == 0,
                "patch_embed_norm: pointers must keep their vector alignment");
  PatchEmbedDev d;
  for (int i = 0; i < n_clips; ++i) {
    TTV_CHECK_ARG(clips[i] && (uintptr_t)clips[i] % 16 == 0, "patch_embed_norm: clip %d is null or not 16-byte aligned", i);
    d.clips.p[i] = clips[i];
  }
  for (int i = n_clips; i < TTV_MAX_CLIPS_PER_LAUNCH; ++i) d.clips.p[i] = nullptr;
  d.clip_desc = clip_desc; d.patch_rows = patch_rows; d.row_seq = row_seq;
  d.w = (const bf16_t*)w; d.bias = (const bf16_t*)bias; d.mask_token = mask_token; d.gain = gain; d.x = (bf16_t*)x;
  d.ldw = ldw; d.ldx = ldx; d.M = M; d.K = patch_dim; d.clip0 = clip0; d.pt_shift = lg2(patch_t); d.ph_shift = lg2(patch_h);
  d.eps = eps;
  TtvProfScope prof(TTV_KC_GEMM_STORE, s);
  hipLaunchKernelGGL(k_patch_embed256, dim3(ttv_cdiv(M, PE_TT)), dim3(512), 0, s, d);
  TTV_CHECK_LAUNCH("patch_embed256");
  return TTV_OK;
}
```

Measured before the change: 31100.

## Run last decoder MLP tail only on patch rows; stage patch-embed stores through LDS

In the decoder's last layer, the fused MLP tail now runs only over the patch-row runs of each clip and skips the latent-token rows whose outputs are never used. A row-run tile mapping and a tile-size choice are added for this. Separately, the patch-embed kernel writes its normalized output into LDS first and then stores full 16-byte rows to global memory, with row indices prefetched early. Optional cycle-counter stamps are added behind a compile flag. Risks: stricter alignment checks on x and ldx, and the row-run path only applies when the batch layout is regular.

```diff
diff --git a/include/titok_hip.h b/include/titok_hip.h
--- a/include/titok_hip.h
+++ b/include/titok_hip.h
@@ -106,6 +106,9 @@
 int ttv_layer_tail_fused(const void* ao, int ldao, const float* attn_post_gain, float attn_alpha, const void* x, int ldx,
                          const void* mlp_packed, int inner, void* y, int ldy, const float* ffd_post_gain, float ffd_alpha, float eps,
                          int M, int width, int dtype, const ttv_next_qkv* next, void* stream);
+int ttv_layer_tail_fused_rows(const void* ao, int ldao, const float* attn_post_gain, float attn_alpha, const void* x, int ldx,
+                              const void* mlp_packed, int inner, void* y, int ldy, const float* ffd_post_gain, float ffd_alpha, float eps,
+                              int M, int width, int dtype, int run_tokens, int period_tokens, int skip_tokens, void* stream);
 
 int ttv_fill_const_rows(void* x, int dtype, int ld, const int32_t* rows_map, int rows, int width, const float* mask_token,
                         const float* gain, float eps, void* stream);
@@ -535,7 +538,8 @@
   TTV_DBG_DEC_ALL_BLOCKS = 2097152,
   TTV_DBG_DEC_L0_NO_CONST = 4194304,
   TTV_DBG_ENC_LAST_QKV_ALL = 8388608,
-  TTV_DBG_PATCH_EMBED_UNFUSED = 16777216
+  TTV_DBG_PATCH_EMBED_UNFUSED = 16777216,
+  TTV_DBG_DEC_LAST_TAIL_ALL = 33554432
 };
 int ttv_debug_set(int flags);
 int ttv_debug_stamps(void* device_buffer);
diff --git a/titok_video_amd/_lib.py b/titok_video_amd/_lib.py
--- a/titok_video_amd/_lib.py
+++ b/titok_video_amd/_lib.py
@@ -43,6 +43,7 @@
 DBG_DEC_L0_NO_CONST = 4194304
 DBG_ENC_LAST_QKV_ALL = 8388608
 DBG_PATCH_EMBED_UNFUSED = 16777216
+DBG_DEC_LAST_TAIL_ALL = 33554432
 
 _HERE = os.path.dirname(os.path.abspath(__file__))
 LIB_PATH = switches.text("TTV_LIB_PATH") or os.path.join(_HERE, "libtitok_hip.so")
@@ -208,6 +209,8 @@
     "ttv_mlp_pack": (C.c_int, [vp, vp, vp, vp, C.c_int, C.c_int, C.c_int, C.c_int, vp, vp]),
     "ttv_layer_tail_fused": (C.c_int, [vp, C.c_int, vp, f32, vp, C.c_int, vp, C.c_int, vp, C.c_int, vp, f32, f32, C.c_int, C.c_int,
                                        C.c_int, vp, vp]),
+    "ttv_layer_tail_fused_rows": (C.c_int, [vp, C.c_int, vp, f32, vp, C.c_int, vp, C.c_int, vp, C.c_int, vp, f32, f32, C.c_int, C.c_int,
+                                            C.c_int, C.c_int, C.c_int, C.c_int, vp]),
     "ttv_mlp_fused": (C.c_int, [vp, C.c_int, vp, C.c_int, vp, C.c_int, vp, f32, f32, C.c_int, C.c_int, C.c_int, vp]),
     "ttv_fill_const_rows": (C.c_int, [vp, C.c_int, C.c_int, vp, C.c_int, C.c_int, vp, vp, f32, vp]),
     "ttv_decoder_embed": (C.c_int, [vp, C.c_int, vp, vp, vp, vp, vp, C.c_int, C.c_int, vp, C.c_int, C.c_int, f32, vp]),
diff --git a/titok_video_amd/csrc/ttv_api.hip b/titok_video_amd/csrc/ttv_api.hip
--- a/titok_video_amd/csrc/ttv_api.hip
+++ b/titok_video_amd/csrc/ttv_api.hip
@@ -26,6 +26,7 @@
 bool ttv_sw_attn_pipe() { static const bool v = ttv_env_flag("TTV_ATTN_PIPE", false); return v; }
 static bool sw_dec_l0_const() { static const bool v = ttv_env_flag("TTV_DEC_L0_CONST", true); return v; }
 static bool sw_enc_last_qkv_skip() { static const bool v = ttv_env_flag("TTV_ENC_LAST_QKV_SKIP", true); return v; }
+static bool sw_dec_last_tail_rows() { static const bool v = ttv_env_flag("TTV_DEC_LAST_TAIL_ROWS", true); return v; }
 float ttv_sw_attn_thr() { static const float v = ttv_env_float("TTV_ATTN_THR", 8.0f); return v; }
 thread_local int g_ttv_debug = 0;
 long long* g_ttv_stamps = nullptr;
@@ -238,6 +239,16 @@
   const ttv_batch* b = c.b;
   if (!sw_enc_last_qkv_skip() || (g_ttv_debug & TTV_DBG_ENC_LAST_QKV_ALL) || c.d->kind != TTV_ENCODER) return false;
   return qkv_tile_list_ok(c, lw, b->tokens_per_clip, b->max_patches_per_clip);
+}
+
+static bool tail_row_runs_ok(const LayerCtx& c, const ttv_layer_weights& lw) {
+  const ttv_tower_dims* d = c.d;
+  const ttv_batch* b = c.b;
+  const int K = b->tokens_per_clip, P = b->max_patches_per_clip;
+  if (!sw_dec_last_tail_rows() || (g_ttv_debug & TTV_DBG_DEC_LAST_TAIL_ALL) || d->kind != TTV_DECODER) return false;
+  if (d->dtype != TTV_BF16 || d->width != 256 || c.split3 || !lw.mlp_pack || !ttvk_mlp_fused_supported(d->dtype, d->width, d->inner)) return false;
+  if (K <= 0 || P <= 0 || K % 128 || P % 128 || (int64_t)b->n_clips * K != b->sum_tokens || (int64_t)b->n_clips * P != b->sum_patches) return false;
+  return (int64_t)b->n_clips * (K + P) == b->total_rows;
 }
 
 static int run_layers(const ttv_tower_dims* d, const ttv_tower_weights* w, const ttv_batch* b, const TowerWs& ws, hipStream_t s,
@@ -304,21 +315,23 @@
     char* cx = ws.x;
     char* cao = ws.ao;
     int Lc = L;
+    static const bool use_fused_mlp = ttv_env_flag("TTV_FUSED_MLP", true);
+    const bool use_runs = use_fused_mlp && pat_last && last && dt == TTV_BF16 && !ctx.pipe && tail_row_runs_ok(ctx, lw);
+    const MlpRowRuns runs = {b->max_patches_per_clip, b->tokens_per_clip + b->max_patches_per_clip, b->tokens_per_clip};
     if (lat_now) {
       TTV_TRY(gather_rows(ws.x, ws.xl, b->latent_rows, b->sum_tokens, row_bytes, s));
       TTV_TRY(gather_rows(ws.ao, ws.aol, b->latent_rows, b->sum_tokens, row_bytes, s));
       cx = ws.xl; cao = ws.aol; Lc = b->sum_tokens;
       compacted = true;
     }
-    static const bool use_fused_mlp = ttv_env_flag("TTV_FUSED_MLP", true);
     static const bool use_fused_qkv = ttv_env_flag("TTV_FUSED_QKV", false);
     const float alpha = keel_alpha(d, i);
     if (use_fused_mlp && ttvk_mlp_fused_supported(dt, dm, d->inner) && lw.mlp_pack) {
       MlpNextQkv nx = {};
-      const bool back = use_fused_qkv && !last && lw.mlp_pack_qkv_rows == nq && nq % 64 == 0 && dm % 64 == 0 && g % 64 == 0;
+      const bool back = use_fused_qkv && !last && !use_runs && lw.mlp_pack_qkv_rows == nq && nq % 64 == 0 && dm % 64 == 0 && g % 64 == 0;
       if (back) { nx.qkv = ws.qkv; nx.ld = nq; nx.rope_cs = b->rope_cs; nx.rows = nq; nx.rope_q_end = dm; nx.rope_k_begin = 2 * dm; nx.rope_k_end = 2 * dm + g; }
       TTV_TRY(ttvk_mlp_fused(cao, dm, i == 0 ? nullptr : lw.attn_post_ln, alpha, cx, dm, lw.mlp_pack, d->inner, cx, dm, i == 0 ? nullptr : lw.ffd_post_ln,
-                             alpha, d->eps, Lc, back ? &nx : nullptr, s));
+                             alpha, d->eps, Lc, back ? &nx : nullptr, s, use_runs ? &runs : nullptr));
       qkv_ready = back;
       continue;
     }
@@ -552,6 +565,19 @@
               nx.rope_k_begin = next->rope_k_begin; nx.rope_k_end = next->rope_k_end; }
   return ttvk_mlp_fused(ao, ldao, attn_post_gain, attn_alpha, x, ldx, mlp_packed, inner, y, ldy, ffd_post_gain, ffd_alpha, eps, M,
                         next ? &nx : nullptr, (hipStream_t)stream);
+}
+
+int ttv_layer_tail_fused_rows(const void* ao, int ldao, const float* attn_post_gain, float attn_alpha, const void* x, int ldx,
+                              const void* mlp_packed, int inner, void* y, int ldy, const float* ffd_post_gain, float ffd_alpha, float eps,
+                              int M, int width, int dtype, int run_tokens, int period_tokens, int skip_tokens, void* stream) {
+  if (!ttvk_mlp_fused_supported(dtype, width, inner)) {
+    ttv_set_error("layer_tail_fused_rows: only bf16, width 256, inner %% 32 == 0");
+    return TTV_ERR_UNSUPPORTED;
+  }
+  TTV_CHECK_ARG(ao, "layer_tail_fused_rows: null attention output");
+  const MlpRowRuns runs = {run_tokens, period_tokens, skip_tokens};
+  return ttvk_mlp_fused(ao, ldao, attn_post_gain, attn_alpha, x, ldx, mlp_packed, inner, y, ldy, ffd_post_gain, ffd_alpha, eps, M, nullptr,
+                        (hipStream_t)stream, &runs);
 }
 
 int ttv_fill_const_rows(void* x, int dtype, int ld, const int32_t* rows_map, int rows, int width, const float* mask_token,
diff --git a/titok_video_amd/csrc/ttv_kernels.h b/titok_video_amd/csrc/ttv_kernels.h
--- a/titok_video_amd/csrc/ttv_kernels.h
+++ b/titok_video_amd/csrc/ttv_kernels.h
@@ -140,8 +140,14 @@
 int64_t ttvk_mlp_pack_bytes(int inner, int next_qkv_rows);
 int ttvk_mlp_pack(const void* w12_folded, const void* w3, const void* wo, const void* next_qkv_folded, int next_qkv_rows, int inner,
                   void* packed, hipStream_t s);
+struct MlpRowRuns {
+  int run_tokens;
+  int period_tokens;
+  int skip_tokens;
+};
 int ttvk_mlp_fused(const void* ao, int ldao, const float* front_gain, float front_alpha, const void* x, int ldx, const void* packed,
-                   int inner, void* y, int ldy, const float* post_gain, float alpha, float eps, int M, const MlpNextQkv* nq, hipStream_t s);
+                   int inner, void* y, int ldy, const float* post_gain, float alpha, float eps, int M, const MlpNextQkv* nq, hipStream_t s,
+                   const MlpRowRuns* runs = nullptr);
 
 int ttvk_l1_loss(void* const* recon, void* const* target, void* const* grad, const int* sizes, int n_clips, int total_clips, int dtype,
                  float* loss, hipStream_t s);
diff --git a/titok_video_amd/csrc/ttv_mlp.hip b/titok_video_amd/csrc/ttv_mlp.hip
--- a/titok_video_amd/csrc/ttv_mlp.hip
+++ b/titok_video_amd/csrc/ttv_mlp.hip
@@ -21,6 +21,7 @@
   float alpha, eps;
   int M, n_tiles, debug;
   long long* stamps;
+  int run_bpr, run_period, run_skip;
 };
 
 __global__ void k_mlp_pack(const bf16_t* __restrict__ w12f, const bf16_t* __restrict__ w3, const bf16_t* __restrict__ wo,
@@ -103,7 +104,7 @@
 #define MLP_STAMP() do { (void)n_stamp; } while (0)
 #endif
 
-template <int TPB, int T1, int T2, bool GELU_FIRST, bool KEEL, bool FRONT, bool BACK>
+template <int TPB, int T1, int T2, bool GELU_FIRST, bool KEEL, bool FRONT, bool BACK, bool RUNS = false>
 __device__ __forceinline__ void mlp_wave(const MlpDev& p, uint4* l12, uint4* l3, uint4* hb, const float* gl, int tile, int wave, int lane,
                                          int P1F, int P2F, int& n_stamp) {
   constexpr int T1A = T1 > 0 ? T1 : 1, T2A = T2 > 0 ? T2 : 1;
@@ -125,7 +126,7 @@
     MLP_GLDS_2(src__, dst__);                                                                                      \
   } while (0)
 
-  const int tok0 = tile * (16 * TPB) + l15;
+  const int tok0 = RUNS ? (tile / p.run_bpr) * p.run_period + p.run_skip + (tile % p.run_bpr) * (16 * TPB) + l15 : tile * (16 * TPB) + l15;
   typedef __attribute__((address_space(1))) char gchar;
   typedef __attribute__((address_space(1))) const char gcchar;
   gcchar* const gx = (gcchar*)p.x;
@@ -535,7 +536,7 @@
 #undef GLDS_W3
 }
 
-template <int TILES, bool KEEL, bool FRONT, bool BACK>
+template <int TILES, bool KEEL, bool FRONT, bool BACK, bool RUNS = false>
 __global__ __launch_bounds__(512, 1) void k_mlp256(MlpDev p) {
   extern __shared__ __attribute__((aligned(16))) uint4 smem[];
   uint4* const l12 = smem;
@@ -559,8 +560,8 @@
     constexpr int NT = TILES / 4;
     constexpr int TA = NT - NT / 2;
     const int g0 = (wave & 3) * NT;
-    if (wave < 4) mlp_wave<TILES, TA, NT - TA, false, KEEL, FRONT, BACK>(p, l12, l3, hb, gl, tile, wave, lane, g0, g0 + TA, n_stamp);
-    else mlp_wave<TILES, NT - TA, TA, false, KEEL, FRONT, BACK>(p, l12, l3, hb, gl, tile, wave, lane, g0 + TA, g0, n_stamp);
+    if (wave < 4) mlp_wave<TILES, TA, NT - TA, false, KEEL, FRONT, BACK, RUNS>(p, l12, l3, hb, gl, tile, wave, lane, g0, g0 + TA, n_stamp);
+    else mlp_wave<TILES, NT - TA, TA, false, KEEL, FRONT, BACK, RUNS>(p, l12, l3, hb, gl, tile, wave, lane, g0 + TA, g0, n_stamp);
   }
 }
 #undef MLP_LD12
@@ -590,7 +591,8 @@
 }
 
 int ttvk_mlp_fused(const void* ao, int ldao, const float* front_gain, float front_alpha, const void* x, int ldx, const void* packed,
-                   int inner, void* y, int ldy, const float* post_gain, float alpha, float eps, int M, const MlpNextQkv* nq, hipStream_t s) {
+                   int inner, void* y, int ldy, const float* post_gain, float alpha, float eps, int M, const MlpNextQkv* nq, hipStream_t s,
+                   const MlpRowRuns* runs) {
   if (M == 0) return TTV_OK;
   TTV_CHECK_ARG(x && packed && y, "mlp_fused: null buffer");
   TTV_CHECK_ARG(inner % 32 == 0 && ldx % 8 == 0 && ldy % 8 == 0 && (!ao || ldao % 8 == 0), "mlp_fused: inner %% 32, leading dims %% 8");
@@ -601,6 +603,7 @@
   d.ao = (const bf16_t*)ao; d.ldao = ldao; d.front_gain = front_gain; d.front_alpha = front_alpha;
   d.y = (bf16_t*)y; d.ldy = ldy; d.post_gain = post_gain; d.alpha = alpha; d.eps = eps; d.M = M; d.debug = g_ttv_debug; d.stamps = g_ttv_stamps;
   d.qkv = nullptr; d.ldq = 0; d.rope_cs = nullptr; d.nqp = 0; d.rope_q_end = d.rope_k_begin = d.rope_k_end = 0;
+  d.run_bpr = 1; d.run_period = d.run_skip = 0;
   if (nq) {
     TTV_CHECK_ARG(nq->qkv && nq->rope_cs && nq->rows > 0 && nq->rows % 64 == 0 && nq->ld >= nq->rows && nq->ld % 4 == 0 &&
                       (uintptr_t)nq->qkv % 8 == 0, "mlp_fused: bad next-qkv arguments (rows %% 64, ld %% 4, 8-byte aligned)");
@@ -622,7 +625,27 @@
   if ((g_ttv_debug & TTV_DBG_MLP_TILES9) && !nq) tiles = 9;
   if (g_ttv_debug & TTV_DBG_MLP_TILES8) tiles = 8;
   if (g_ttv_debug & TTV_DBG_MLP_TILES4) tiles = 4;
-  d.n_tiles = ttv_cdiv(M, 16 * tiles);
+  if (runs) {
+    TTV_CHECK_ARG(ao && !nq, "mlp_fused: row runs need the out_proj front and exclude the next-qkv part");
+    TTV_CHECK_ARG(runs->run_tokens > 0 && runs->run_tokens % 64 == 0 && runs->skip_tokens >= 0 && runs->period_tokens > 0 &&
+                      runs->skip_tokens + runs->run_tokens <= runs->period_tokens && M % runs->period_tokens == 0,
+                  "mlp_fused: bad row runs (run %% 64, skip + run <= period, M %% period)");
+    const int n_runs = M / runs->period_tokens;
+    tiles = 0;
+    best = -1;
+    for (int c = 1; c <= 2; ++c) {
+      if (runs->run_tokens % (64 * c)) continue;
+      const long cost = (long)ttv_cdiv(n_runs * (runs->run_tokens / (64 * c)), cus) * (16 + 19 * c);
+      if (best < 0 || cost < best) { best = cost; tiles = 4 * c; }
+    }
+    if (g_ttv_debug & TTV_DBG_MLP_TILES8) tiles = 8;
+    if (g_ttv_debug & TTV_DBG_MLP_TILES4) tiles = 4;
+    TTV_CHECK_ARG(runs->run_tokens % (16 * tiles) == 0, "mlp_fused: the forced block size does not divide the row run");
+    d.run_bpr = runs->run_tokens / (16 * tiles); d.run_period = runs->period_tokens; d.run_skip = runs->skip_tokens;
+    d.n_tiles = n_runs * d.run_bpr;
+  } else {
+    d.n_tiles = ttv_cdiv(M, 16 * tiles);
+  }
   const int grid = d.n_tiles;
   const size_t smem = (size_t)(2 * MLP_W12_CHUNKS + 2 * MLP_W3_CHUNKS + 2 * tiles * 64) * sizeof(uint4) + 2048;
   TtvProfScope prof(TTV_KC_GEMM_GEGLU, s);
@@ -643,7 +666,16 @@
     else LAUNCH_MLP(9, KEEL_, false, false);                                                                        \
   } while (0)
   TTV_CHECK_ARG(!nq || ao, "mlp_fused: the next-qkv part needs the out_proj front (ttv_layer_tail_fused)");
-  if (post_gain) {
+  if (runs) {
+#define LAUNCH_MLP_R(TILES_, KEEL_)                                                                                 \
+  do {                                                                                                              \
+    (void)hipFuncSetAttribute((const void*)k_mlp256<TILES_, KEEL_, true, false, true>, hipFuncAttributeMaxDynamicSharedMemorySize, (int)smem); \
+    hipLaunchKernelGGL((k_mlp256<TILES_, KEEL_, true, false, true>), dim3(grid), dim3(512), smem, s, d);            \
+  } while (0)
+    if (post_gain) { if (tiles == 8) LAUNCH_MLP_R(8, true); else LAUNCH_MLP_R(4, true); }
+    else { if (tiles == 8) LAUNCH_MLP_R(8, false); else LAUNCH_MLP_R(4, false); }
+#undef LAUNCH_MLP_R
+  } else if (post_gain) {
     if (tiles == 9) LAUNCH_MLP_9(true); else if (tiles == 12) LAUNCH_MLP_F(12, true); else if (tiles == 8) LAUNCH_MLP_F(8, true); else LAUNCH_MLP_F(4, true);
   } else {
     if (tiles == 9) LAUNCH_MLP_9(false); else if (tiles == 12) LAUNCH_MLP_F(12, false); else if (tiles == 8) LAUNCH_MLP_F(8, false); else LAUNCH_MLP_F(4, false);
diff --git a/titok_video_amd/csrc/ttv_patch_embed.hip b/titok_video_amd/csrc/ttv_patch_embed.hip
--- a/titok_video_amd/csrc/ttv_patch_embed.hip
+++ b/titok_video_amd/csrc/ttv_patch_embed.hip
@@ -14,7 +14,17 @@
   bf16_t* x;
   int ldw, ldx, M, K, clip0, pt_shift, ph_shift;
   float eps;
+#ifdef PE_STAMPS
+  long long* stamps;
+#endif
 };
+
+#define PE_OROW 272
+#ifdef PE_STAMPS
+#define PE_STAMP(n_) ts[n_] = (long long)__builtin_readcyclecounter()
+#else
+#define PE_STAMP(n_) do { } while (0)
+#endif
 
 __global__ __launch_bounds__(512, 1) void k_patch_embed256(PatchEmbedDev p) {
   __shared__ __attribute__((aligned(16))) uint4 lds[PE_STAGES][PE_STAGE_U4];
@@ -22,6 +32,10 @@
   const int wave = __builtin_amdgcn_readfirstlane(tid >> 6);
   const int wf = wave & 1, wt = wave >> 1;
   const int tbase = blockIdx.x * PE_TT;
+#ifdef PE_STAMPS
+  long long ts[5] = {0, 0, 0, 0, 0};
+#endif
+  PE_STAMP(0);
 
   const int lr = lane >> 3, lp = lane & 7;
   uint32_t woff[4];
@@ -87,7 +101,14 @@
   const uint32_t fo1 = (uint32_t)(l15 * 128 + (((4 + kq) ^ ((l15 >> 1) & 7)) << 4));
   const uint32_t a_base = (uint32_t)(wf * 128 * 128), b_base = (uint32_t)(PE_F * 128 + wt * 32 * 128);
 
+  int orow[8];
+#pragma unroll
+  for (int r = 0; r < 8; ++r) {
+    const int t = tbase + wt * 32 + r * 4 + (lane >> 4);
+    orow[r] = p.patch_rows[t < p.M ? t : p.M - 1];
+  }
   asm volatile("s_waitcnt vmcnt(0)" ::: "memory");
+  PE_STAMP(1);
   PE_STAGE(0, 0);
   if (nk > 1) PE_STAGE(1, 1);
   int st = 0;
@@ -95,6 +116,7 @@
     if (kt + 1 < nk) asm volatile("s_waitcnt vmcnt(6)" ::: "memory");
     else asm volatile("s_waitcnt vmcnt(0)" ::: "memory");
     __syncthreads();
+    if (kt == 0) PE_STAMP(2);
     if (kt + 2 < nk) {
       const int st2 = st + 2 >= PE_STAGES ? st + 2 - PE_STAGES : st + 2;
       PE_STAGE(kt + 2, st2);
@@ -115,6 +137,7 @@
     }
     st = st + 1 == PE_STAGES ? 0 : st + 1;
   }
+  PE_STAMP(3);
 #undef PE_STAGE
 #undef PE_DMA_W
 #undef PE_DMA_X
@@ -138,10 +161,10 @@
     }
   }
   __syncthreads();
+  char* const tw = reinterpret_cast<char*>(&lds[(st + 1 + (wave >> 2)) % PE_STAGES][0]) + (wave & 3) * (32 * PE_OROW);
 #pragma unroll
   for (int j = 0; j < 2; ++j) {
     const int tl = wt * 32 + j * 16 + l15;
-    const int t = tbase + tl;
     float s1[8];
 #pragma unroll
     for (int i = 0; i < 8; ++i) s1[i] = grp[i][j] + gx[((wf ^ 1) * PE_TT + tl) * 33 + i * 4 + kq];
@@ -155,17 +178,29 @@
       tot = __uint_as_float(a0) + __uint_as_float(a1);
     }
     const float rstd = 1.0f / sqrtf(tot / 256.0f + p.eps);
-    if (t < p.M) {
-      bf16_t* const q = p.x + (size_t)p.patch_rows[t] * p.ldx;
-#pragma unroll
-      for (int i = 0; i < 8; ++i) {
-        const int f = wf * 128 + i * 16 + kq * 4;
-        const f32x4 g = *reinterpret_cast<const f32x4*>(p.gain + f);
-        const f32x4 o = {acc[i][j][0] * rstd * g[0], acc[i][j][1] * rstd * g[1], acc[i][j][2] * rstd * g[2], acc[i][j][3] * rstd * g[3]};
-        Vec4<bf16_t>::store(q + f, o);
-      }
-    }
-  }
+#pragma unroll
+    for (int i = 0; i < 8; ++i) {
+      const int f = wf * 128 + i * 16 + kq * 4;
+      const f32x4 g = *reinterpret_cast<const f32x4*>(p.gain + f);
+      const f32x4 o = {acc[i][j][0] * rstd * g[0], acc[i][j][1] * rstd * g[1], acc[i][j][2] * rstd * g[2], acc[i][j][3] * rstd * g[3]};
+      Vec4<bf16_t>::store(reinterpret_cast<bf16_t*>(tw + (j * 16 + l15) * PE_OROW + (i * 16 + kq * 4) * 2), o);
+    }
+  }
+  asm volatile("s_waitcnt lgkmcnt(0)" ::: "memory");
+#pragma unroll
+  for (int r = 0; r < 8; ++r) {
+    const int row = r * 4 + (lane >> 4);
+    const uint4 v = *reinterpret_cast<const uint4*>(tw + row * PE_OROW + (lane & 15) * 16);
+    if (tbase + wt * 32 + row < p.M)
+      *reinterpret_cast<uint4*>(p.x + (size_t)orow[r] * p.ldx + wf * 128 + (lane & 15) * 8) = v;
+  }
+  PE_STAMP(4);
+#ifdef PE_STAMPS
+  if (p.stamps && blockIdx.x == 0 && lane == 0) {
+#pragma unroll
+    for (int n = 0; n < 5; ++n) p.stamps[wave * 8 + n] = ts[n];
+  }
+#endif
 }
 
 bool ttvk_patch_embed_norm_supported(int dtype, int width, int patch_dim, int patch_w) {
@@ -181,9 +216,9 @@
                     patch_dim % (patch_t * patch_h * patch_w) == 0,
                 "patch_embed_norm: patch_w == 8, power-of-two patch_t / patch_h and a patch vector that is a multiple of 64");
   TTV_CHECK_ARG(n_clips > 0 && n_clips <= TTV_MAX_CLIPS_PER_LAUNCH, "patch_embed_norm: 1 .. %d clips per call", TTV_MAX_CLIPS_PER_LAUNCH);
-  TTV_CHECK_ARG(ldw >= patch_dim && ldw % 8 == 0 && ldx >= PE_F && ldx % 4 == 0 && (uint64_t)PE_F * (uint64_t)ldw * 2u < (1ull << 32),
+  TTV_CHECK_ARG(ldw >= patch_dim && ldw % 8 == 0 && ldx >= PE_F && ldx % 8 == 0 && (uint64_t)PE_F * (uint64_t)ldw * 2u < (1ull << 32),
                 "patch_embed_norm: leading dims must hold a row and keep its alignment");
-  TTV_CHECK_ARG((uintptr_t)w % 16 == 0 && (uintptr_t)x % 8 == 0 && (uintptr_t)bias % 8 == 0 && (uintptr_t)gain % 16 == 0,
+  TTV_CHECK_ARG((uintptr_t)w % 16 == 0 && (uintptr_t)x % 16 == 0 && (uintptr_t)bias % 8 == 0 && (uintptr_t)gain % 16 == 0,
                 "patch_embed_norm: pointers must keep their vector alignment");
   PatchEmbedDev d;
   for (int i = 0; i < n_clips; ++i) {
@@ -195,6 +230,9 @@
   d.w = (const bf16_t*)w; d.bias = (const bf16_t*)bias; d.mask_token = mask_token; d.gain = gain; d.x = (bf16_t*)x;
   d.ldw = ldw; d.ldx = ldx; d.M = M; d.K = patch_dim; d.clip0 = clip0; d.pt_shift = lg2(patch_t); d.ph_shift = lg2(patch_h);
   d.eps = eps;
+#ifdef PE_STAMPS
+  d.stamps = g_ttv_stamps;
+#endif
   TtvProfScope prof(TTV_KC_GEMM_STORE, s);
   hipLaunchKernelGGL(k_patch_embed256, dim3(ttv_cdiv(M, PE_TT)), dim3(512), 0, s, d);
   TTV_CHECK_LAUNCH("patch_embed256");
```

After: 31290 (median of 2 runs). No clear change (+0.6%).
